# 0xPARC/plonky2-aes

Hardware: AMD Instinct MI355X
Metric: proofs/sec (AES-GCM 1 KiB circuit) (higher is better)
Workload: dtype u64 (Goldilocks field)

## Files before the change

### bindings/plonky2-hip/src/ffi.rs

```rust
#![allow(non_camel_case_types, dead_code)]
use std::os::raw::{c_char, c_int, c_long, c_void};

#[repr(C)] pub struct P2Builder { _private: [u8; 0] }
#[repr(C)] pub struct P2Circuit { _private: [u8; 0] }
#[repr(C)] pub struct P2Assignment { pub targets: *const u64, pub values: *const u64, pub count: usize }
#[repr(C)] #[derive(Default, Clone, Copy)]
pub struct P2CircuitInfo {
    pub degree_bits: u32, pub num_wires: u32, pub num_routed_wires: u32, pub num_constants_cols: u32, pub num_zs_cols: u32,
    pub num_quotient_cols: u32, pub num_luts: u32, pub num_ops: u32, pub num_levels: u32, pub num_slots: u32,
    pub num_virtual_targets: u32, pub num_fri_rounds: u32, pub proof_bytes: u64, pub zero_knowledge: u32, pub num_gate_kinds: u32,
    pub num_public_inputs: u32, pub hasher: u32,
}
#[repr(C)] pub struct P2KernelTime { pub name: [c_char; 48], pub ms: f32, pub count: u32 }
#[repr(C)] #[derive(Default, Clone, Copy, Debug)]
pub struct P2WitnessFault { pub kind: i32, pub op_kind: i32, pub input_index: i64, pub target: u64, pub gate_row: u32, pub computed: u64, pub found: u64 }

pub const P2_OK: c_int = 0;
pub const P2_PROOF_OK: c_int = 0;
pub const P2_VALUE_UNSET: u64 = u64::MAX;
pub const P2_FAULT_KINDS: [&str; 6] = ["NONE", "INPUT_NOT_CANONICAL", "INPUT_CONFLICT", "LOOKUP_MISS", "GENERATOR_CONFLICT", "NOT_SET"];
pub const P2_HASHER_POSEIDON: c_int = 0;
pub const P2_HASHER_KECCAK: c_int = 1;
pub const P2_POINT_WORDS: usize = 10;
pub const P2_SCALAR_LIMBS: usize = 5;
// ... 52 lines not shown
    pub fn p2_gcm_inc32(a0: *mut P2Builder, block: *const u64, out: *mut u64);
    pub fn p2_gcm_gf_2_128_mul(a0: *mut P2Builder, xor_lut: usize, shift_lut: usize, bitref_lut: usize, x: *const u64, y: *const u64, out: *mut u64);
    pub fn p2_gcm_ghash(a0: *mut P2Builder, xor_lut: usize, shift_lut: usize, bitref_lut: usize, h: *const u64, x: *const u64, len: usize, out: *mut u64) -> c_int;
    pub fn p2_gcm_gf_2_128_mul_tables(a0: *mut P2Builder, xor_lut: usize, clmul_lo_lut: usize, clmul_hi_lut: usize, x: *const u64, y: *const u64, out: *mut u64) -> c_int;
    pub fn p2_gcm_ghash_tables(a0: *mut P2Builder, xor_lut: usize, clmul_lo_lut: usize, clmul_hi_lut: usize, h: *const u64, x: *const u64, len: usize, out: *mut u64, lanes: c_int) -> c_int;
    pub fn p2_builder_set_ghash_tables(a0: *mut P2Builder, lanes: c_int) -> c_int;
    pub fn p2_aes_gcm_build(a0: *mut P2Builder, nk: c_int, nr: c_int, L: usize, with_tag: c_int, key: *mut u64, nonce: *mut u64, pt: *mut u64, ct: *mut u64, tag: *mut u64) -> c_int;
    pub fn p2_aes_gcm_build_aad(a0: *mut P2Builder, nk: c_int, nr: c_int, L: usize, with_tag: c_int, aad_len: usize, key: *mut u64, nonce: *mut u64, pt: *mut u64, ct: *mut u64, tag: *mut u64, aad: *mut u64) -> c_int;
    pub fn p2_builder_hash_n_to_m_no_pad(a0: *mut P2Builder, inputs: *const u64, n: usize, outputs: *mut u64, m: usize) -> c_int;
    pub fn p2_builder_permute_swapped(a0: *mut P2Builder, inputs: *const u64, swap: u64, out: *mut u64) -> c_int;
    pub fn p2_builder_hash_or_noop(a0: *mut P2Builder, inputs: *const u64, n: usize, out: *mut u64) -> c_int;
    pub fn p2_builder_add_virtual_hash(a0: *mut P2Builder, out: *mut u64) -> c_int;
    pub fn p2_builder_add_virtual_cap(a0: *mut P2Builder, cap_height: c_int, out: *mut u64) -> c_int;
    pub fn p2_builder_connect_hashes(a0: *mut P2Builder, x: *const u64, y: *const u64) -> c_int;
    pub fn p2_builder_verify_merkle_proof_to_cap(a0: *mut P2Builder, leaf: *const u64, leaf_len: usize, index_bits: *const u64, n_bits: usize, cap: *const u64, cap_height: c_int, siblings: *const u64, n_siblings: usize) -> c_int;
    pub fn p2_builder_verify_merkle_proof(a0: *mut P2Builder, leaf: *const u64, leaf_len: usize, index_bits: *const u64, n_bits: usize, root: *const u64, siblings: *const u64, n_siblings: usize) -> c_int;
    pub fn p2_builder_merkle_update_to_cap(a0: *mut P2Builder, old_leaf: *const u64, new_leaf: *const u64, leaf_len: usize, index_bits: *const u64, n_bits: usize, old_cap: *const u64, cap_height: c_int, siblings: *const u64, n_siblings: usize, new_cap: *mut u64) -> c_int;
    pub fn p2_builder_merkle_update(a0: *mut P2Builder, old_leaf: *const u64, new_leaf: *const u64, leaf_len: usize, index_bits: *const u64, n_bits: usize, old_root: *const u64, siblings: *const u64, n_siblings: usize, new_root: *mut u64) -> c_int;
    pub fn p2_native_merkle_cap(leaves: *const u64, num_leaves: usize, leaf_len: usize, cap_height: c_int, cap: *mut u64) -> c_int;
    pub fn p2_native_merkle_prove(leaves: *const u64, num_leaves: usize, leaf_len: usize, cap_height: c_int, index: usize, siblings: *mut u64) -> c_int;
    pub fn p2_native_merkle_verify(leaf: *const u64, leaf_len: usize, index: usize, siblings: *const u64, depth: usize, cap: *const u64, cap_height: c_int, status: *mut c_int) -> c_int;
    pub fn p2_native_merkle_update(leaves: *mut u64, num_leaves: usize, leaf_len: usize, cap_height: c_int, indices: *const u64, new_leaves: *const u64, k: usize, siblings: *mut u64, root_after: *mut u64) -> c_int;
    pub fn p2_builder_merkle_map_lookup_to_cap(a0: *mut P2Builder, key_bits: *const u64, n_bits: usize, value: *const u64, value_len: usize, present: u64, cap: *const u64, cap_height: c_int, siblings: *const u64, n_siblings: usize) -> c_int;
    pub fn p2_builder_merkle_map_lookup(a0: *mut P2Builder, key_bits: *const u64, n_bits: usize, value: *const u64, value_len: usize, present: u64, root: *const u64, siblings: *const u64, n_siblings: usize) -> c_int;
    pub fn p2_builder_merkle_map_update_to_cap(a0: *mut P2Builder, key_bits: *const u64, n_bits: usize, old_present: u64, old_value: *const u64, new_present: u64, new_value: *const u64, value_len: usize, old_cap: *const u64, cap_height: c_int, siblings: *const u64, n_siblings: usize, new_cap: *mut u64) -> c_int;
    pub fn p2_builder_merkle_map_update(a0: *mut P2Builder, key_bits: *const u64, n_bits: usize, old_present: u64, old_value: *const u64, new_present: u64, new_value: *const u64, value_len: usize, old_root: *const u64, siblings: *const u64, n_siblings: usize, new_root: *mut u64) -> c_int;
    pub fn p2_builder_merkle_map_insert_to_cap(a0: *mut P2Builder, key_bits: *const u64, n_bits: usize, value: *const u64, value_len: usize, old_cap: *const u64, cap_height: c_int, siblings: *const u64, n_siblings: usize, new_cap: *mut u64) -> c_int;
    pub fn p2_builder_merkle_map_insert(a0: *mut P2Builder, key_bits: *const u64, n_bits: usize, value: *const u64, value_len: usize, old_root: *const u64, siblings: *const u64, n_siblings: usize, new_root: *mut u64) -> c_int;
    pub fn p2_builder_merkle_map_remove_to_cap(a0: *mut P2Builder, key_bits: *const u64, n_bits: usize, value: *const u64, value_len: usize, old_cap: *const u64, cap_height: c_int, siblings: *const u64, n_siblings: usize, new_cap: *mut u64) -> c_int;
    pub fn p2_builder_merkle_map_remove(a0: *mut P2Builder, key_bits: *const u64, n_bits: usize, value: *const u64, value_len: usize, old_root: *const u64, siblings: *const u64, n_siblings: usize, new_root: *mut u64) -> c_int;
    pub fn p2_native_merkle_map_cap(keys: *const u64, values: *const u64, n: usize, value_len: usize, key_bits: c_int, cap_height: c_int, cap: *mut u64) -> c_int;
    pub fn p2_native_merkle_map_get(keys: *const u64, values: *const u64, n: usize, value_len: usize, key_bits: c_int, cap_height: c_int, key: u64, present: *mut c_int, value: *mut u64, siblings: *mut u64) -> c_int;
    pub fn p2_native_merkle_map_verify(key: u64, key_bits: c_int, present: u64, value: *const u64, value_len: usize, siblings: *const u64, cap: *const u64, cap_height: c_int, status: *mut c_int) -> c_int;
    pub fn p2_poseidon_cipher_build(a0: *mut P2Builder, L: usize, ks: *mut u64, m: *mut u64, nonce: *mut u64, ct: *mut u64) -> c_int;
    pub fn p2_builder_poseidon_encrypt(a0: *mut P2Builder, ks: *const u64, nonce: *const u64, m: *const u64, L: usize, ct: *mut u64) -> c_int;
    pub fn p2_builder_poseidon_decrypt(a0: *mut P2Builder, ks: *const u64, nonce: *const u64, ct: *const u64, L: usize, m: *mut u64) -> c_int;
    pub fn p2_native_hash_n_to_m_no_pad(in: *const u64, n: usize, out: *mut u64, m: usize);
    pub fn p2_native_poseidon_encrypt(ks10: *const u64, msg: *const u64, n_msg: usize, nonce2: *const u64, ct: *mut u64);
    pub fn p2_native_poseidon_decrypt(ks10: *const u64, ct: *const u64, n_ct: usize, nonce2: *const u64, l: usize, msg: *mut u64) -> c_int;
    pub fn p2_ecgfp5_group_order(out: *mut u64);
    pub fn p2_ecgfp5_generator(out: *mut u64);
    pub fn p2_ecgfp5_mul(k: *const u64, p: *const u64, out: *mut u64);
    pub fn p2_ecgfp5_add(p: *const u64, q: *const u64, out: *mut u64);
    pub fn p2_ecgfp5_neg(p: *const u64, out: *mut u64);
    pub fn p2_ecgfp5_is_in_subgroup(p: *const u64) -> c_int;
    pub fn p2_ecgfp5_compress(p: *const u64, w: *mut u64);
    pub fn p2_ecgfp5_decompress(w: *const u64, out: *mut u64) -> c_int;
    pub fn p2_ecgfp5_random_scalar(out: *mut u64) -> c_int;
    pub fn p2_ecgfp5_random_point(out: *mut u64) -> c_int;
    pub fn p2_ecgfp5_encode_binary(limbs: *const u32, out: *mut u64) -> c_int;
    pub fn p2_ecgfp5_random_scalar_seeded(seed: u64, out: *mut u64);
    pub fn p2_ecgfp5_random_point_seeded(seed: u64, out: *mut u64);
    pub fn p2_ecgfp5_encode_binary_seeded(limbs: *const u32, seed: u64, out: *mut u64);
    pub fn p2_ecgfp5_decode_binary(p: *const u64, limbs: *mut u32);
    pub fn p2_elgamal_encrypt(pk: *const u64, nonce: *const u64, msg: *const u64, c0: *mut u64, c1: *mut u64) -> c_int;
    pub fn p2_elgamal_decrypt(sk: *const u64, c0: *const u64, c1: *const u64, msg: *mut u64) -> c_int;
    pub fn p2_hashed_elgamal_encrypt(pk: *const u64, nonce: *const u64, msg: *const u64, c0: *mut u64, ct: *mut u64) -> c_int;
    pub fn p2_hashed_elgamal_decrypt(sk: *const u64, c0: *const u64, ct: *const u64, msg: *mut u64) -> c_int;
    pub fn p2_builder_add_virtual_point_target(a0: *mut P2Builder, out: *mut u64);
    pub fn p2_builder_constant_point(a0: *mut P2Builder, p: *const u64, out: *mut u64);
    pub fn p2_builder_add_virtual_biguint320_target(a0: *mut P2Builder, bits: *mut u64);
    pub fn p2_builder_multiply_point(a0: *mut P2Builder, bits: *const u64, p: *const u64, out: *mut u64) -> c_int;
    pub fn p2_builder_add_point(a0: *mut P2Builder, p: *const u64, q: *const u64, out: *mut u64);
    pub fn p2_builder_set_ec_gate(a0: *mut P2Builder, on: c_int) -> c_int;
    pub fn p2_builder_ec_step(a0: *mut P2Builder, acc: *const u64, q: *const u64, bit: u64, hinted: c_int, mid: *mut u64, out: *mut u64) -> c_int;
    pub fn p2_builder_public_key(a0: *mut P2Builder, sk_bits: *const u64, pk: *mut u64) -> c_int;
    pub fn p2_builder_elgamal_encrypt(a0: *mut P2Builder, pk: *const u64, nonce_bits: *const u64, msg: *const u64, c0: *mut u64, c1: *mut u64) -> c_int;
    pub fn p2_builder_hashed_elgamal_encrypt(a0: *mut P2Builder, pk: *const u64, nonce_bits: *const u64, msg: *const u64, c0: *mut u64, ct: *mut u64) -> c_int;
    pub fn p2_ecgfp5_encode_binary_padded(limbs: *const u32, pad: *const u32, attempts: usize, out: *mut u64, used: *mut u32) -> c_int;
    pub fn p2_builder_neg_point(a0: *mut P2Builder, p: *const u64, out: *mut u64) -> c_int;
    pub fn p2_builder_elgamal_decrypt(a0: *mut P2Builder, sk_bits: *const u64, c0: *const u64, c1: *const u64, msg: *mut u64) -> c_int;
    pub fn p2_builder_hashed_elgamal_decrypt(a0: *mut P2Builder, sk_bits: *const u64, c0: *const u64, ct: *const u64, msg: *mut u64) -> c_int;
    pub fn p2_ecgfp5_scalar_muladd(a: *const u64, b: *const u64, c: *const u64, out: *mut u64);
    pub fn p2_schnorr_challenge(r: *const u64, pk: *const u64, msg: *const u64, msg_len: usize, e: *mut u64) -> c_int;
    pub fn p2_schnorr_sign(sk: *const u64, nonce: *const u64, msg: *const u64, msg_len: usize, sig: *mut u64, pk: *mut u64, status: *mut c_int) -> c_int;
    pub fn p2_schnorr_verify(pk: *const u64, msg: *const u64, msg_len: usize, sig: *const u64, status: *mut c_int) -> c_int;
    pub fn p2_builder_add_virtual_schnorr_signature(a0: *mut P2Builder, s_bits: *mut u64, e: *mut u64) -> c_int;
    pub fn p2_builder_verify_schnorr_signature(a0: *mut P2Builder, pk: *const u64, msg: *const u64, msg_len: usize, s_bits: *const u64, e: *const u64, r: *mut u64) -> c_int;
    pub fn p2_selftest_host(seed: u64, n_reductions: usize, n_permutations: usize) -> c_int;
    pub fn p2_selftest_device(seed: u64, threads: usize, device: c_int) -> c_int;
    pub fn p2_selftest_lazy_device(seed: u64, threads: usize, device: c_int) -> c_int;
    pub fn p2_selftest_ntt_device(seed: u64, threads: usize, device: c_int) -> c_int;
    pub fn p2_host_poseidon_known(states: *mut u64, n_perm: usize, kind: c_int, rows: u32, parts: c_int) -> c_int;
    pub fn p2_host_pcipher_hash_state(in: *const u64, last: c_int, out: *mut u64) -> c_int;
    pub fn p2_host_partial_rounds(states: *mut u64, count: usize) -> c_int;
    pub fn p2_host_merged_middle(states: *mut u64, count: usize) -> c_int;
    pub fn p2_host_ecstep_constraints(wires: *const u64, count: usize, out: *mut u64) -> c_int;
    pub fn p2_host_ecstep_constraints_ext(wires: *const u64, count: usize, out: *mut u64) -> c_int;
    pub fn p2_host_hash_leaves(data: *const u64, cols: usize, active_cols: usize, num_leaves: usize, digests: *mut u64) -> c_int;
    pub fn p2_native_gf_2_8_mul(a: u8, b: u8) -> u8;
    pub fn p2_native_aes_key_expansion(key: *const u8, nk: c_int, nr: c_int, out: *mut u8);
    pub fn p2_native_aes_encrypt_block(key: *const u8, nk: c_int, nr: c_int, in16: *const u8, out16: *mut u8);
    pub fn p2_native_gf_2_128_mul(x16: *const u8, y16: *const u8, out16: *mut u8);
    pub fn p2_native_ghash(h16: *const u8, x: *const u8, len: usize, out16: *mut u8);
    pub fn p2_native_gctr(key: *const u8, nk: c_int, nr: c_int, icb16: *const u8, x: *const u8, len: usize, y: *mut u8);
    pub fn p2_native_aes_gcm_encrypt_aad(key: *const u8, nk: c_int, nr: c_int, nonce12: *const u8, aad: *const u8, aad_len: usize, pt: *const u8, len: usize, ct: *mut u8, tag16: *mut u8);
    pub fn p2_native_aes_gcm_decrypt(key: *const u8, nk: c_int, nr: c_int, nonce12: *const u8, aad: *const u8, aad_len: usize, ct: *const u8, len: usize, tag16: *const u8, pt: *mut u8) -> c_int;
    pub fn p2_native_aes_gcm_encrypt(key: *const u8, nk: c_int, nr: c_int, nonce12: *const u8, pt: *const u8, len: usize, ct: *mut u8, tag16: *mut u8);
    pub fn p2_native_keccak_hash_no_pad(in: *const u64, n: usize, out4: *mut u64);
    pub fn p2_native_keccak_two_to_one(l4: *const u64, r4: *const u64, out4: *mut u64);
    pub fn p2_native_keccak256(data: *const u8, len: usize, out32: *mut u8);
    pub fn p2_blob_info(blob: *const u8, len: usize, out: *mut P2CircuitInfo) -> c_int;
    pub fn p2_witness_schedule_check(blob: *const u8, len: usize, fuse: u32, out: *mut u32) -> c_int;
    pub fn p2_verify(blob: *const u8, blob_len: usize, verifier_data: *const u64, verifier_data_len: usize, proof: *const u8, proof_len: usize) -> c_int;
    pub fn p2_vanishing_terms(blob: *const u8, blob_len: usize, openings: *const u8, len: usize, challenges: *const u64, pi_hash: *const u64, terms: *mut u64, cap: usize, n_terms: *mut usize, sides: *mut u64, verdict: *mut c_int) -> c_int;
    pub fn p2_proof_compress(blob: *const u8, blob_len: usize, verifier_data: *const u64, verifier_data_len: usize, proof: *const u8, proof_len: usize, out: *mut u8, cap: usize, n_written: *mut usize) -> c_int;
    pub fn p2_proof_decompress(blob: *const u8, blob_len: usize, verifier_data: *const u64, verifier_data_len: usize, cproof: *const u8, cproof_len: usize, out: *mut u8, cap: usize, n_written: *mut usize) -> c_int;
    pub fn p2_verify_compressed(blob: *const u8, blob_len: usize, verifier_data: *const u64, verifier_data_len: usize, cproof: *const u8, cproof_len: usize) -> c_int;
    pub fn p2_proof_public_inputs(blob: *const u8, blob_len: usize, proof: *const u8, proof_len: usize, out: *mut u64, cap: usize, n_written: *mut usize) -> c_int;
    pub fn p2_circuit_load(blob: *const u8, len: usize, device: c_int) -> *mut P2Circuit;
    pub fn p2_circuit_free(a0: *mut P2Circuit);
    pub fn p2_circuit_verifier_data(a0: *const P2Circuit, out: *mut u64, cap: usize, n_written: *mut usize) -> c_int;
    pub fn p2_circuit_chunk_proofs(a0: *mut P2Circuit) -> usize;
    pub fn p2_circuit_set_zk_key(a0: *mut P2Circuit, key: *const u64) -> c_int;
    pub fn p2_circuit_set_zk_seed(a0: *mut P2Circuit, seed: u64) -> c_int;
    pub fn p2_circuit_proof_bytes(a0: *const P2Circuit) -> usize;
    pub fn p2_circuit_num_public_inputs(a0: *const P2Circuit) -> usize;
    pub fn p2_circuit_public_inputs(a0: *const P2Circuit, proof: *const u8, proof_len: usize, out: *mut u64, cap: usize, n_written: *mut usize) -> c_int;
    pub fn p2_prove_batch(a0: *mut P2Circuit, batch: usize, inputs: *const P2Assignment, proofs: *mut u8, status: *mut c_int) -> c_int;
    pub fn p2_prove_batch_multi(handles: *const *mut P2Circuit, n_handles: usize, batch: usize, inputs: *const P2Assignment, proofs: *mut u8, status: *mut c_int) -> c_int;
    pub fn p2_prove_batch_device(a0: *mut P2Circuit, batch: usize, targets: *const u64, n_targets: usize, d_values: *const u64, d_proofs: *mut u8, d_status: *mut c_int, stream: *mut c_void) -> c_int;
    pub fn p2_circuit_synchronize(a0: *mut P2Circuit) -> c_int;
    pub fn p2_prove_batch_outputs_device(a0: *mut P2Circuit, batch: usize, targets: *const u64, n_targets: usize, d_values: *const u64, out_targets: *const u64, n_out: usize, d_out: *mut u64, d_proofs: *mut u8, d_status: *mut c_int, stream: *mut c_void) -> c_int;
    pub fn p2_prove_batch_outputs(a0: *mut P2Circuit, batch: usize, inputs: *const P2Assignment, out_targets: *const u64, n_out: usize, out_values: *mut u64, proofs: *mut u8, status: *mut c_int) -> c_int;
    pub fn p2_witness_batch_device(a0: *mut P2Circuit, batch: usize, targets: *const u64, n_targets: usize, d_values: *const u64, out_targets: *const u64, n_out: usize, d_out: *mut u64, d_status: *mut c_int, stream: *mut c_void) -> c_int;
    pub fn p2_witness_batch(a0: *mut P2Circuit, batch: usize, inputs: *const P2Assignment, out_targets: *const u64, n_out: usize, out_values: *mut u64, status: *mut c_int) -> c_int;
    pub fn p2_witness_explain(a0: *mut P2Circuit, input: *const P2Assignment, status: *mut c_int, out: *mut c_void) -> c_int;
    pub fn p2_host_witness(blob: *const u8, len: usize, input: *const P2Assignment, out_targets: *const u64, n_out: usize, out_values: *mut u64, status: *mut c_int, fault: *mut c_void) -> c_int;
    pub fn p2_verify_batch(a0: *mut P2Circuit, batch: usize, proofs: *const u8, verifier_data: *const u64, vd_len: usize, status: *mut c_int) -> c_int;
    pub fn p2_verify_batch_device(a0: *mut P2Circuit, batch: usize, d_proofs: *const u8, verifier_data: *const u64, vd_len: usize, d_status: *mut c_int, stream: *mut c_void) -> c_int;
    pub fn p2_gpu_vanishing_flags(a0: *mut P2Circuit, batch: usize, buffers: *const u8, challenges: *const u64, pi_hashes: *const u64, flags: *mut u32) -> c_int;
    pub fn p2_compress_batch(a0: *mut P2Circuit, batch: usize, proofs: *const u8, verifier_data: *const u64, vd_len: usize, out: *mut u8, lengths: *mut u32, status: *mut c_int) -> c_int;
    pub fn p2_decompress_batch(a0: *mut P2Circuit, batch: usize, cproofs: *const u8, lengths: *const u32, verifier_data: *const u64, vd_len: usize, out: *mut u8, status: *mut c_int) -> c_int;
    pub fn p2_verify_compressed_batch(a0: *mut P2Circuit, batch: usize, cproofs: *const u8, lengths: *const u32, verifier_data: *const u64, vd_len: usize, status: *mut c_int) -> c_int;
    pub fn p2_compress_batch_device(a0: *mut P2Circuit, batch: usize, d_proofs: *const u8, verifier_data: *const u64, vd_len: usize, d_out: *mut u8, d_lengths: *mut u32, d_status: *mut c_int, stream: *mut c_void) -> c_int;
    pub fn p2_decompress_batch_device(a0: *mut P2Circuit, batch: usize, d_cproofs: *const u8, d_lengths: *const u32, verifier_data: *const u64, vd_len: usize, d_out: *mut u8, d_status: *mut c_int, stream: *mut c_void) -> c_int;
    pub fn p2_verify_compressed_batch_device(a0: *mut P2Circuit, batch: usize, d_cproofs: *const u8, d_lengths: *const u32, verifier_data: *const u64, vd_len: usize, d_status: *mut c_int, stream: *mut c_void) -> c_int;
    pub fn p2_circuit_set_option(a0: *mut P2Circuit, name: *const c_char, value: c_long) -> c_int;
    pub fn p2_circuit_set_timing(a0: *mut P2Circuit, enable: c_int) -> c_int;
    pub fn p2_circuit_get_timing(a0: *mut P2Circuit, out: *mut P2KernelTime, cap: usize) -> usize;
    pub fn p2_merkle_tree_new(leaves: *const u64, num_leaves: usize, leaf_len: usize, cap_height: c_int, device: c_int, tree: *mut *mut c_void) -> c_int;
    pub fn p2_merkle_tree_new_device(d_leaves: *const u64, num_leaves: usize, leaf_len: usize, cap_height: c_int, device: c_int, stream: *mut c_void, tree: *mut *mut c_void) -> c_int;
    pub fn p2_merkle_tree_free(tree: *mut c_void);
    pub fn p2_merkle_tree_cap(tree: *mut c_void, cap: *mut u64, cap_words: usize) -> c_int;
    pub fn p2_merkle_tree_prove_batch(tree: *mut c_void, indices: *const u64, n: usize, siblings: *mut u64) -> c_int;
    pub fn p2_merkle_tree_prove_batch_device(tree: *mut c_void, d_indices: *const u64, n: usize, d_out: *mut u64, out_stride_words: usize, d_status: *mut c_int, stream: *mut c_void) -> c_int;
    pub fn p2_merkle_tree_update(tree: *mut c_void, indices: *const u64, leaves: *const u64, k: usize, siblings: *mut u64, root_after: *mut u64) -> c_int;
    pub fn p2_merkle_tree_update_device(tree: *mut c_void, d_indices: *const u64, d_leaves: *const u64, k: usize, d_siblings: *mut u64, sib_stride_words: usize, d_root_after: *mut u64, root_stride_words: usize, d_status: *mut c_int, stream: *mut c_void) -> c_int;
    pub fn p2_merkle_tree_last_update_hashes(tree: *mut c_void, hashes: *mut u64) -> c_int;
    pub fn p2_merkle_verify_batch(leaves: *const u64, leaf_len: usize, indices: *const u64, siblings: *const u64, depth: usize, cap: *const u64, cap_height: c_int, n: usize, status: *mut c_int, device: c_int) -> c_int;
    pub fn p2_merkle_verify_batch_device(d_leaves: *const u64, leaf_len: usize, d_indices: *const u64, d_siblings: *const u64, depth: usize, d_cap: *const u64, cap_height: c_int, n: usize, d_status: *mut c_int, device: c_int, stream: *mut c_void) -> c_int;
    pub fn p2_gpu_merkle_build_device(d_leaves: *const u64, num_leaves: usize, leaf_len: usize, cap_height: c_int, with_transpose: c_int, d_scratch: *mut u64, d_dig: *mut u64, device: c_int, stream: *mut c_void) -> c_int;
    pub fn p2_merkle_map_new(keys: *const u64, values: *const u64, n: usize, value_len: usize, key_bits: c_int, cap_height: c_int, device: c_int, map: *mut *mut c_void) -> c_int;
    pub fn p2_merkle_map_new_device(d_keys: *const u64, d_values: *const u64, n: usize, value_len: usize, key_bits: c_int, cap_height: c_int, device: c_int, stream: *mut c_void, map: *mut *mut c_void) -> c_int;
    pub fn p2_merkle_map_free(map: *mut c_void);
    pub fn p2_merkle_map_cap(map: *mut c_void, cap: *mut u64, cap_words: usize) -> c_int;
    pub fn p2_merkle_map_len(map: *mut c_void, n: *mut usize) -> c_int;
    pub fn p2_merkle_map_hashes(map: *mut c_void, hashes: *mut u64) -> c_int;
    pub fn p2_merkle_map_get_batch(map: *mut c_void, keys: *const u64, n: usize, present: *mut u64, values: *mut u64, siblings: *mut u64) -> c_int;
    pub fn p2_merkle_map_get_batch_device(map: *mut c_void, d_keys: *const u64, n: usize, d_out: *mut u64, out_stride_words: usize, present_off: usize, value_off: usize, siblings_off: usize, d_status: *mut c_int, stream: *mut c_void) -> c_int;
    pub fn p2_merkle_map_verify_batch(keys: *const u64, key_bits: c_int, present: *const u64, values: *const u64, value_len: usize, siblings: *const u64, cap: *const u64, cap_height: c_int, n: usize, status: *mut c_int, device: c_int) -> c_int;
    pub fn p2_merkle_map_verify_batch_device(d_keys: *const u64, key_bits: c_int, d_present: *const u64, d_values: *const u64, value_len: usize, d_siblings: *const u64, d_cap: *const u64, cap_height: c_int, n: usize, d_status: *mut c_int, device: c_int, stream: *mut c_void) -> c_int;
    pub fn p2_ecgfp5_mul_batch(k: *const u64, p: *const u64, count: usize, out: *mut u64, status: *mut c_int, device: c_int) -> c_int;
    pub fn p2_ecgfp5_mul_batch_device(d_k: *const u64, d_p: *const u64, count: usize, d_out: *mut u64, d_status: *mut c_int, device: c_int, stream: *mut c_void) -> c_int;
    pub fn p2_schnorr_sign_batch(sk: *const u64, nonce: *const u64, msg: *const u64, msg_len: usize, count: usize, sig: *mut u64, pk: *mut u64, status: *mut c_int, device: c_int) -> c_int;
    pub fn p2_schnorr_sign_batch_device(d_sk: *const u64, d_nonce: *const u64, d_msg: *const u64, msg_len: usize, count: usize, d_sig: *mut u64, d_pk: *mut u64, d_status: *mut c_int, device: c_int, stream: *mut c_void) -> c_int;
    pub fn p2_schnorr_verify_batch(pk: *const u64, msg: *const u64, msg_len: usize, sig: *const u64, count: usize, status: *mut c_int, device: c_int) -> c_int;
    pub fn p2_schnorr_verify_batch_device(d_pk: *const u64, d_msg: *const u64, msg_len: usize, d_sig: *const u64, count: usize, d_status: *mut c_int, device: c_int, stream: *mut c_void) -> c_int;
    pub fn p2_gpu_ecgfp5_scalar_muladd(a: *const u64, b: *const u64, c: *const u64, count: usize, out: *mut u64, device: c_int) -> c_int;
    pub fn p2_ecgfp5_decompress_batch(w: *const u64, count: usize, out: *mut u64, status: *mut c_int, device: c_int) -> c_int;
    pub fn p2_ecgfp5_decompress_batch_device(d_w: *const u64, count: usize, d_out: *mut u64, d_status: *mut c_int, device: c_int, stream: *mut c_void) -> c_int;
    pub fn p2_ecgfp5_encode_binary_batch(limbs: *const u32, pad: *const u32, attempts: usize, count: usize, out: *mut u64, used: *mut u32, status: *mut c_int, device: c_int) -> c_int;
    pub fn p2_ecgfp5_encode_binary_batch_device(d_limbs: *const u32, d_pad: *const u32, attempts: usize, count: usize, d_out: *mut u64, d_used: *mut u32, d_status: *mut c_int, device: c_int, stream: *mut c_void) -> c_int;
    pub fn p2_elgamal_encrypt_batch(pk: *const u64, nonce: *const u64, msg: *const u64, count: usize, c0: *mut u64, c1: *mut u64, status: *mut c_int, device: c_int) -> c_int;
    pub fn p2_elgamal_encrypt_batch_device(d_pk: *const u64, d_nonce: *const u64, d_msg: *const u64, count: usize, d_c0: *mut u64, d_c1: *mut u64, d_status: *mut c_int, device: c_int, stream: *mut c_void) -> c_int;
    pub fn p2_elgamal_decrypt_batch(sk: *const u64, c0: *const u64, c1: *const u64, count: usize, msg: *mut u64, status: *mut c_int, device: c_int) -> c_int;
    pub fn p2_elgamal_decrypt_batch_device(d_sk: *const u64, d_c0: *const u64, d_c1: *const u64, count: usize, d_msg: *mut u64, d_status: *mut c_int, device: c_int, stream: *mut c_void) -> c_int;
    pub fn p2_hashed_elgamal_encrypt_batch(pk: *const u64, nonce: *const u64, msg: *const u64, count: usize, c0: *mut u64, ct: *mut u64, status: *mut c_int, device: c_int) -> c_int;
    pub fn p2_hashed_elgamal_encrypt_batch_device(d_pk: *const u64, d_nonce: *const u64, d_msg: *const u64, count: usize, d_c0: *mut u64, d_ct: *mut u64, d_status: *mut c_int, device: c_int, stream: *mut c_void) -> c_int;
    pub fn p2_hashed_elgamal_decrypt_batch(sk: *const u64, c0: *const u64, ct: *const u64, count: usize, msg: *mut u64, status: *mut c_int, device: c_int) -> c_int;
    pub fn p2_hashed_elgamal_decrypt_batch_device(d_sk: *const u64, d_c0: *const u64, d_ct: *const u64, count: usize, d_msg: *mut u64, d_status: *mut c_int, device: c_int, stream: *mut c_void) -> c_int;
    pub fn p2_ecgfp5_scalar_bits_device(d_k: *const u64, count: usize, d_out: *mut u64, stride: usize, device: c_int, stream: *mut c_void) -> c_int;
    pub fn p2_poseidon_encrypt_batch(ks: *const u64, nonce: *const u64, msg: *const u64, l: usize, count: usize, ct: *mut u64, status: *mut c_int, device: c_int) -> c_int;
    pub fn p2_poseidon_encrypt_batch_device(d_ks: *const u64, d_nonce: *const u64, d_msg: *const u64, l: usize, count: usize, d_ct: *mut u64, d_status: *mut c_int, device: c_int, stream: *mut c_void) -> c_int;
    pub fn p2_poseidon_decrypt_batch(ks: *const u64, nonce: *const u64, ct: *const u64, l: usize, count: usize, msg: *mut u64, status: *mut c_int, device: c_int) -> c_int;
    pub fn p2_poseidon_decrypt_batch_device(d_ks: *const u64, d_nonce: *const u64, d_ct: *const u64, l: usize, count: usize, d_msg: *mut u64, d_status: *mut c_int, device: c_int, stream: *mut c_void) -> c_int;
    pub fn p2_aes_gcm_batch_workspace(nk: c_int, len: usize, aad_len: usize, count: usize) -> usize;
    pub fn p2_aes_gcm_encrypt_batch(key: *const u8, nk: c_int, nonce: *const u8, aad: *const u8, aad_len: usize, pt: *const u8, len: usize, count: usize, ct: *mut u8, tag: *mut u8, status: *mut c_int, device: c_int) -> c_int;
    pub fn p2_aes_gcm_decrypt_batch(key: *const u8, nk: c_int, nonce: *const u8, aad: *const u8, aad_len: usize, ct: *const u8, tag: *const u8, len: usize, count: usize, pt: *mut u8, status: *mut c_int, device: c_int) -> c_int;
    pub fn p2_aes_gcm_encrypt_batch_device(d_key: *const u8, nk: c_int, d_nonce: *const u8, d_aad: *const u8, aad_len: usize, d_pt: *const u8, len: usize, row_stride: usize, count: usize, d_ct: *mut u8, d_tag: *mut u8, d_status: *mut c_int, d_work: *mut c_void, device: c_int, stream: *mut c_void) -> c_int;
    pub fn p2_aes_gcm_decrypt_batch_device(d_key: *const u8, nk: c_int, d_nonce: *const u8, d_aad: *const u8, aad_len: usize, d_ct: *const u8, d_tag: *const u8, len: usize, row_stride: usize, count: usize, d_pt: *mut u8, d_status: *mut c_int, d_work: *mut c_void, device: c_int, stream: *mut c_void) -> c_int;
    pub fn p2_bytes_to_words_device(d_bytes: *const u8, row_bytes: usize, byte_stride: usize, count: usize, d_out: *mut u64, stride_words: usize, device: c_int, stream: *mut c_void) -> c_int;
    pub fn p2_gpu_gcm_ghash(h: *const u8, x: *const u8, blocks: usize, count: usize, lanes: c_int, out: *mut u8, device: c_int) -> c_int;
    pub fn p2_gpu_aes_encrypt_blocks(key: *const u8, nk: c_int, in: *const u8, count: usize, out: *mut u8, device: c_int) -> c_int;
    pub fn p2_gpu_gcm_kernel_times(nk: c_int, len: usize, aad_len: usize, count: usize, lanes: c_int, repeats: usize, ns: *mut u64, device: c_int) -> c_int;
    pub fn p2_gpu_device_count() -> c_int;
    pub fn p2_gpu_poseidon(states: *mut u64, n_perm: usize, device: c_int) -> c_int;
    pub fn p2_gpu_lde(coeffs: *const u64, cols: usize, degree_bits: c_int, rate_bits: c_int, lde: *mut u64, device: c_int) -> c_int;
    pub fn p2_gpu_intt(values: *const u64, cols: usize, degree_bits: c_int, coeffs: *mut u64, device: c_int) -> c_int;
    pub fn p2_gpu_lde_round(coeffs: *const u64, cols: usize, degree_bits: c_int, arities: *const u32, n_rounds: usize, round: usize, batch: usize, in_batch_stride: usize, out: *mut u64, out_batch_stride: usize, device: c_int) -> c_int;
    pub fn p2_gpu_quotient_chunks(qvals: *const u64, chunks: usize, degree_bits: c_int, batch: usize, out: *mut u64, device: c_int) -> c_int;
    pub fn p2_gpu_merkle_cap(cols_major: *const u64, cols: usize, num_leaves: usize, cap_height: c_int, cap: *mut u64, device: c_int) -> c_int;
    pub fn p2_gpu_merkle_cap_hasher(cols_major: *const u64, cols: usize, num_leaves: usize, cap_height: c_int, hasher: c_int, cap: *mut u64, device: c_int) -> c_int;
    pub fn p2_gpu_hash_leaves(data: *const u64, cols: usize, active_cols: usize, num_leaves: usize, batch: usize, digests: *mut u64, device: c_int) -> c_int;
    pub fn p2_gpu_partial_rounds(states: *mut u64, count: usize, device: c_int) -> c_int;
    pub fn p2_gpu_merged_middle(states: *mut u64, count: usize, device: c_int) -> c_int;
    pub fn p2_gpu_ecstep_constraints(wires: *const u64, count: usize, out: *mut u64, device: c_int) -> c_int;
    pub fn p2_gpu_merkle_level(child: *const u64, num_parents: usize, batch: usize, parent: *mut u64, device: c_int) -> c_int;
    pub fn p2_gpu_hash_fri_leaves(vals: *const u64, len: usize, arity: c_int, batch: usize, digests: *mut u64, device: c_int) -> c_int;
    pub fn p2_gpu_zeta_pows(z: *const u64, n: usize, pows: *mut u64, device: c_int) -> c_int;
    pub fn p2_circuit_debug_read(a0: *mut P2Circuit, name: *const c_char, index: usize, out: *mut u64, cap: usize, n_written: *mut usize) -> c_int;
    pub fn p2_debug_live_resources() -> usize;
}
```

### include/p2aes.h

```cpp
#ifndef P2AES_H
#define P2AES_H
#include <stddef.h>
#include <stdint.h>

#ifdef __cplusplus
extern "C" {
#endif

enum {
    P2_OK = 0,
    P2_ERR_INVALID = 1,
    P2_ERR_NO_DEVICE = 2,
    P2_ERR_HIP = 3,
    P2_ERR_VERIFY = 4
};
enum {
    P2_PROOF_OK = 0,
    P2_PROOF_WITNESS_CONFLICT = 1,
    P2_PROOF_MISSING_INPUT = 2,
    P2_PROOF_ZETA_IN_SUBGROUP = 3,
    P2_PROOF_POW_NOT_FOUND = 4
};
enum {
    P2_VERIFY_OK = 0,
// ... 101 lines not shown
                            size_t k, uint64_t* siblings, uint64_t* root_after);
int p2_builder_merkle_map_lookup_to_cap(p2_builder*, const p2_target* key_bits, size_t n_bits, const p2_target* value, size_t value_len, p2_target present,
                                        const p2_target* cap, int cap_height, const p2_target* siblings, size_t n_siblings);
int p2_builder_merkle_map_lookup(p2_builder*, const p2_target* key_bits, size_t n_bits, const p2_target* value, size_t value_len, p2_target present,
                                 const p2_target root[4], const p2_target* siblings, size_t n_siblings);
int p2_builder_merkle_map_update_to_cap(p2_builder*, const p2_target* key_bits, size_t n_bits, p2_target old_present, const p2_target* old_value,
                                        p2_target new_present, const p2_target* new_value, size_t value_len, const p2_target* old_cap, int cap_height,
                                        const p2_target* siblings, size_t n_siblings, p2_target* new_cap);
int p2_builder_merkle_map_update(p2_builder*, const p2_target* key_bits, size_t n_bits, p2_target old_present, const p2_target* old_value, p2_target new_present,
                                 const p2_target* new_value, size_t value_len, const p2_target old_root[4], const p2_target* siblings, size_t n_siblings,
                                 p2_target new_root[4]);
int p2_builder_merkle_map_insert_to_cap(p2_builder*, const p2_target* key_bits, size_t n_bits, const p2_target* value, size_t value_len, const p2_target* old_cap,
                                        int cap_height, const p2_target* siblings, size_t n_siblings, p2_target* new_cap);
int p2_builder_merkle_map_insert(p2_builder*, const p2_target* key_bits, size_t n_bits, const p2_target* value, size_t value_len, const p2_target old_root[4],
                                 const p2_target* siblings, size_t n_siblings, p2_target new_root[4]);
int p2_builder_merkle_map_remove_to_cap(p2_builder*, const p2_target* key_bits, size_t n_bits, const p2_target* value, size_t value_len, const p2_target* old_cap,
                                        int cap_height, const p2_target* siblings, size_t n_siblings, p2_target* new_cap);
int p2_builder_merkle_map_remove(p2_builder*, const p2_target* key_bits, size_t n_bits, const p2_target* value, size_t value_len, const p2_target old_root[4],
                                 const p2_target* siblings, size_t n_siblings, p2_target new_root[4]);
int p2_native_merkle_map_cap(const uint64_t* keys, const uint64_t* values, size_t n, size_t value_len, int key_bits, int cap_height, uint64_t* cap);
int p2_native_merkle_map_get(const uint64_t* keys, const uint64_t* values, size_t n, size_t value_len, int key_bits, int cap_height, uint64_t key, int* present,
                             uint64_t* value, uint64_t* siblings);
int p2_native_merkle_map_verify(uint64_t key, int key_bits, uint64_t present, const uint64_t* value, size_t value_len, const uint64_t* siblings,
                                const uint64_t* cap, int cap_height, int* status);
int p2_poseidon_cipher_build(p2_builder*, size_t L, p2_target* ks, p2_target* m, p2_target* nonce, p2_target* ct);
int p2_builder_poseidon_encrypt(p2_builder*, const p2_target ks[10], const p2_target nonce[2], const p2_target* m, size_t L, p2_target* ct);
int p2_builder_poseidon_decrypt(p2_builder*, const p2_target ks[10], const p2_target nonce[2], const p2_target* ct, size_t L, p2_target* m);
void p2_native_hash_n_to_m_no_pad(const uint64_t* in, size_t n, uint64_t* out, size_t m);
void p2_native_poseidon_encrypt(const uint64_t* ks10, const uint64_t* msg, size_t n_msg, const uint64_t* nonce2, uint64_t* ct);
int p2_native_poseidon_decrypt(const uint64_t* ks10, const uint64_t* ct, size_t n_ct, const uint64_t* nonce2, size_t l, uint64_t* msg);

#define P2_POINT_WORDS 10
#define P2_SCALAR_LIMBS 5
#define P2_SCALAR_BITS 320
void p2_ecgfp5_group_order(uint64_t out[5]);
void p2_ecgfp5_generator(uint64_t out[10]);
void p2_ecgfp5_mul(const uint64_t k[5], const uint64_t p[10], uint64_t out[10]);
void p2_ecgfp5_add(const uint64_t p[10], const uint64_t q[10], uint64_t out[10]);
void p2_ecgfp5_neg(const uint64_t p[10], uint64_t out[10]);
int p2_ecgfp5_is_in_subgroup(const uint64_t p[10]);
void p2_ecgfp5_compress(const uint64_t p[10], uint64_t w[5]);
int p2_ecgfp5_decompress(const uint64_t w[5], uint64_t out[10]);
int p2_ecgfp5_random_scalar(uint64_t out[5]);
int p2_ecgfp5_random_point(uint64_t out[10]);
int p2_ecgfp5_encode_binary(const uint32_t limbs[5], uint64_t out[10]);
void p2_ecgfp5_random_scalar_seeded(uint64_t seed, uint64_t out[5]);
void p2_ecgfp5_random_point_seeded(uint64_t seed, uint64_t out[10]);
void p2_ecgfp5_encode_binary_seeded(const uint32_t limbs[5], uint64_t seed, uint64_t out[10]);
void p2_ecgfp5_decode_binary(const uint64_t p[10], uint32_t limbs[5]);
int p2_elgamal_encrypt(const uint64_t pk[10], const uint64_t nonce[5], const uint64_t msg[10], uint64_t c0[10], uint64_t c1[10]);
int p2_elgamal_decrypt(const uint64_t sk[5], const uint64_t c0[10], const uint64_t c1[10], uint64_t msg[10]);
int p2_hashed_elgamal_encrypt(const uint64_t pk[10], const uint64_t nonce[5], const uint64_t msg[5], uint64_t c0[10], uint64_t ct[5]);
int p2_hashed_elgamal_decrypt(const uint64_t sk[5], const uint64_t c0[10], const uint64_t ct[5], uint64_t msg[5]);
void p2_builder_add_virtual_point_target(p2_builder*, p2_target out[10]);
void p2_builder_constant_point(p2_builder*, const uint64_t p[10], p2_target out[10]);
void p2_builder_add_virtual_biguint320_target(p2_builder*, p2_target bits[320]);
int p2_builder_multiply_point(p2_builder*, const p2_target bits[320], const p2_target p[10], p2_target out[10]);
void p2_builder_add_point(p2_builder*, const p2_target p[10], const p2_target q[10], p2_target out[10]);
int p2_builder_set_ec_gate(p2_builder*, int on);
int p2_builder_ec_step(p2_builder*, const p2_target acc[20], const p2_target q[10], p2_target bit, int hinted, p2_target mid[20], p2_target out[20]);
int p2_builder_public_key(p2_builder*, const p2_target sk_bits[320], p2_target pk[10]);
int p2_builder_elgamal_encrypt(p2_builder*, const p2_target pk[10], const p2_target nonce_bits[320], const p2_target msg[10],
                               p2_target c0[10], p2_target c1[10]);
int p2_builder_hashed_elgamal_encrypt(p2_builder*, const p2_target pk[10], const p2_target nonce_bits[320], const p2_target msg[5],
                                      p2_target c0[10], p2_target ct[5]);
int p2_ecgfp5_encode_binary_padded(const uint32_t limbs[5], const uint32_t* pad, size_t attempts, uint64_t out[10], uint32_t* used);
int p2_builder_neg_point(p2_builder*, const p2_target p[10], p2_target out[10]);
int p2_builder_elgamal_decrypt(p2_builder*, const p2_target sk_bits[320], const p2_target c0[10], const p2_target c1[10], p2_target msg[10]);
int p2_builder_hashed_elgamal_decrypt(p2_builder*, const p2_target sk_bits[320], const p2_target c0[10], const p2_target ct[5], p2_target msg[5]);

void p2_ecgfp5_scalar_muladd(const uint64_t a[5], const uint64_t b[5], const uint64_t c[5], uint64_t out[5]);
int p2_schnorr_challenge(const uint64_t r[10], const uint64_t pk[10], const uint64_t* msg, size_t msg_len, uint64_t e[4]);
int p2_schnorr_sign(const uint64_t sk[5], const uint64_t nonce[5], const uint64_t* msg, size_t msg_len, uint64_t sig[9], uint64_t pk[10], int* status);
int p2_schnorr_verify(const uint64_t pk[10], const uint64_t* msg, size_t msg_len, const uint64_t sig[9], int* status);
int p2_builder_add_virtual_schnorr_signature(p2_builder*, p2_target s_bits[320], p2_target e[4]);
int p2_builder_verify_schnorr_signature(p2_builder*, const p2_target pk[10], const p2_target* msg, size_t msg_len, const p2_target s_bits[320],
                                        const p2_target e[4], p2_target r[10]);

int p2_selftest_host(uint64_t seed, size_t n_reductions, size_t n_permutations);
int p2_selftest_device(uint64_t seed, size_t threads, int device);
int p2_selftest_lazy_device(uint64_t seed, size_t threads, int device);
int p2_selftest_ntt_device(uint64_t seed, size_t threads, int device);
int p2_host_poseidon_known(uint64_t* states, size_t n_perm, int kind, uint32_t rows, int parts);
int p2_host_pcipher_hash_state(const uint64_t in[20], int last, uint64_t out[20]);
int p2_host_partial_rounds(uint64_t* states, size_t count);
int p2_host_merged_middle(uint64_t* states, size_t count);
int p2_host_ecstep_constraints(const uint64_t* wires, size_t count, uint64_t* out);
int p2_host_ecstep_constraints_ext(const uint64_t* wires, size_t count, uint64_t* out);
int p2_host_hash_leaves(const uint64_t* data, size_t cols, size_t active_cols, size_t num_leaves, uint64_t* digests);

uint8_t p2_native_gf_2_8_mul(uint8_t a, uint8_t b);
void p2_native_aes_key_expansion(const uint8_t* key, int nk, int nr, uint8_t* out );
void p2_native_aes_encrypt_block(const uint8_t* key, int nk, int nr, const uint8_t* in16, uint8_t* out16);
void p2_native_gf_2_128_mul(const uint8_t* x16, const uint8_t* y16, uint8_t* out16);
void p2_native_ghash(const uint8_t* h16, const uint8_t* x, size_t len, uint8_t* out16);
void p2_native_gctr(const uint8_t* key, int nk, int nr, const uint8_t* icb16, const uint8_t* x, size_t len, uint8_t* y);
void p2_native_aes_gcm_encrypt_aad(const uint8_t* key, int nk, int nr, const uint8_t* nonce12, const uint8_t* aad, size_t aad_len, const uint8_t* pt,
                                   size_t len, uint8_t* ct, uint8_t* tag16);
int p2_native_aes_gcm_decrypt(const uint8_t* key, int nk, int nr, const uint8_t* nonce12, const uint8_t* aad, size_t aad_len, const uint8_t* ct, size_t len,
                              const uint8_t* tag16, uint8_t* pt);
void p2_native_aes_gcm_encrypt(const uint8_t* key, int nk, int nr, const uint8_t* nonce12, const uint8_t* pt, size_t len,
                               uint8_t* ct, uint8_t* tag16);

void p2_native_keccak_hash_no_pad(const uint64_t* in, size_t n, uint64_t out4[4]);
void p2_native_keccak_two_to_one(const uint64_t l4[4], const uint64_t r4[4], uint64_t out4[4]);
void p2_native_keccak256(const uint8_t* data, size_t len, uint8_t out32[32]);

typedef struct {
    uint32_t degree_bits, num_wires, num_routed_wires, num_constants_cols, num_zs_cols, num_quotient_cols, num_luts,
        num_ops, num_levels, num_slots, num_virtual_targets, num_fri_rounds;
    uint64_t proof_bytes;
    uint32_t zero_knowledge, num_gate_kinds;
    uint32_t num_public_inputs;
    uint32_t hasher;
} p2_circuit_info;
int p2_blob_info(const uint8_t* blob, size_t len, p2_circuit_info* out);
int p2_witness_schedule_check(const uint8_t* blob, size_t len, uint32_t fuse, uint32_t out[4]);
int p2_verify(const uint8_t* blob, size_t blob_len, const uint64_t* verifier_data, size_t verifier_data_len,
              const uint8_t* proof, size_t proof_len);
int p2_vanishing_terms(const uint8_t* blob, size_t blob_len, const uint8_t* openings, size_t len, const uint64_t challenges[16],
                       const uint64_t pi_hash[4], uint64_t* terms, size_t cap, size_t* n_terms, uint64_t sides[8], int* verdict);
int p2_proof_compress(const uint8_t* blob, size_t blob_len, const uint64_t* verifier_data, size_t verifier_data_len, const uint8_t* proof,
                      size_t proof_len, uint8_t* out, size_t cap, size_t* n_written);
int p2_proof_decompress(const uint8_t* blob, size_t blob_len, const uint64_t* verifier_data, size_t verifier_data_len, const uint8_t* cproof,
                        size_t cproof_len, uint8_t* out, size_t cap, size_t* n_written);
int p2_verify_compressed(const uint8_t* blob, size_t blob_len, const uint64_t* verifier_data, size_t verifier_data_len,
                         const uint8_t* cproof, size_t cproof_len);
int p2_proof_public_inputs(const uint8_t* blob, size_t blob_len, const uint8_t* proof, size_t proof_len, uint64_t* out, size_t cap,
                           size_t* n_written);

typedef struct p2_circuit p2_circuit;
p2_circuit* p2_circuit_load(const uint8_t* blob, size_t len, int device);
void p2_circuit_free(p2_circuit*);
int p2_circuit_verifier_data(const p2_circuit*, uint64_t* out, size_t cap, size_t* n_written);
size_t p2_circuit_chunk_proofs(p2_circuit*);
int p2_circuit_set_zk_key(p2_circuit*, const uint64_t key[4]);
int p2_circuit_set_zk_seed(p2_circuit*, uint64_t seed);
size_t p2_circuit_proof_bytes(const p2_circuit*);
size_t p2_circuit_num_public_inputs(const p2_circuit*);
int p2_circuit_public_inputs(const p2_circuit*, const uint8_t* proof, size_t proof_len, uint64_t* out, size_t cap, size_t* n_written);
typedef struct {
    const p2_target* targets;
    const uint64_t* values;
    size_t count;
} p2_assignment;
int p2_prove_batch(p2_circuit*, size_t batch, const p2_assignment* inputs, uint8_t* proofs, int* status);
int p2_prove_batch_multi(p2_circuit* const* handles, size_t n_handles, size_t batch, const p2_assignment* inputs,
                         uint8_t* proofs, int* status);
int p2_prove_batch_device(p2_circuit*, size_t batch, const p2_target* targets, size_t n_targets, const uint64_t* d_values,
                          uint8_t* d_proofs, int* d_status, void* stream);
int p2_circuit_synchronize(p2_circuit*);

#define P2_VALUE_UNSET UINT64_MAX
int p2_prove_batch_outputs_device(p2_circuit*, size_t batch, const p2_target* targets, size_t n_targets, const uint64_t* d_values,
                                  const p2_target* out_targets, size_t n_out, uint64_t* d_out, uint8_t* d_proofs, int* d_status, void* stream);
int p2_prove_batch_outputs(p2_circuit*, size_t batch, const p2_assignment* inputs, const p2_target* out_targets, size_t n_out,
                           uint64_t* out_values, uint8_t* proofs, int* status);
int p2_witness_batch_device(p2_circuit*, size_t batch, const p2_target* targets, size_t n_targets, const uint64_t* d_values,
                            const p2_target* out_targets, size_t n_out, uint64_t* d_out, int* d_status, void* stream);
int p2_witness_batch(p2_circuit*, size_t batch, const p2_assignment* inputs, const p2_target* out_targets, size_t n_out,
                     uint64_t* out_values, int* status);
typedef struct {
    int32_t kind;
    int32_t op_kind;
    int64_t input_index;
    p2_target target;
// ... 60 lines not shown
int p2_merkle_map_new_device(const uint64_t* d_keys, const uint64_t* d_values, size_t n, size_t value_len, int key_bits, int cap_height, int device, void* stream,
                             void** map);
void p2_merkle_map_free(void* map);
int p2_merkle_map_cap(void* map, uint64_t* cap, size_t cap_words);
int p2_merkle_map_len(void* map, size_t* n);
int p2_merkle_map_hashes(void* map, uint64_t* hashes);
int p2_merkle_map_get_batch(void* map, const uint64_t* keys, size_t n, uint64_t* present, uint64_t* values, uint64_t* siblings);
int p2_merkle_map_get_batch_device(void* map, const uint64_t* d_keys, size_t n, uint64_t* d_out, size_t out_stride_words, size_t present_off, size_t value_off,
                                   size_t siblings_off, int* d_status, void* stream);
int p2_merkle_map_verify_batch(const uint64_t* keys, int key_bits, const uint64_t* present, const uint64_t* values, size_t value_len, const uint64_t* siblings,
                               const uint64_t* cap, int cap_height, size_t n, int* status, int device);
int p2_merkle_map_verify_batch_device(const uint64_t* d_keys, int key_bits, const uint64_t* d_present, const uint64_t* d_values, size_t value_len,
                                      const uint64_t* d_siblings, const uint64_t* d_cap, int cap_height, size_t n, int* d_status, int device, void* stream);

int p2_ecgfp5_mul_batch(const uint64_t* k, const uint64_t* p, size_t count, uint64_t* out, int* status, int device);
int p2_ecgfp5_mul_batch_device(const uint64_t* d_k, const uint64_t* d_p, size_t count, uint64_t* d_out, int* d_status, int device, void* stream);
int p2_schnorr_sign_batch(const uint64_t* sk, const uint64_t* nonce, const uint64_t* msg, size_t msg_len, size_t count, uint64_t* sig, uint64_t* pk,
                          int* status, int device);
int p2_schnorr_sign_batch_device(const uint64_t* d_sk, const uint64_t* d_nonce, const uint64_t* d_msg, size_t msg_len, size_t count, uint64_t* d_sig,
                                 uint64_t* d_pk, int* d_status, int device, void* stream);
int p2_schnorr_verify_batch(const uint64_t* pk, const uint64_t* msg, size_t msg_len, const uint64_t* sig, size_t count, int* status, int device);
int p2_schnorr_verify_batch_device(const uint64_t* d_pk, const uint64_t* d_msg, size_t msg_len, const uint64_t* d_sig, size_t count, int* d_status,
                                   int device, void* stream);
int p2_gpu_ecgfp5_scalar_muladd(const uint64_t* a, const uint64_t* b, const uint64_t* c, size_t count, uint64_t* out, int device);

int p2_ecgfp5_decompress_batch(const uint64_t* w, size_t count, uint64_t* out, int* status, int device);
int p2_ecgfp5_decompress_batch_device(const uint64_t* d_w, size_t count, uint64_t* d_out, int* d_status, int device, void* stream);
int p2_ecgfp5_encode_binary_batch(const uint32_t* limbs, const uint32_t* pad, size_t attempts, size_t count, uint64_t* out, uint32_t* used, int* status,
                                  int device);
int p2_ecgfp5_encode_binary_batch_device(const uint32_t* d_limbs, const uint32_t* d_pad, size_t attempts, size_t count, uint64_t* d_out, uint32_t* d_used,
                                         int* d_status, int device, void* stream);
int p2_elgamal_encrypt_batch(const uint64_t* pk, const uint64_t* nonce, const uint64_t* msg, size_t count, uint64_t* c0, uint64_t* c1, int* status,
                             int device);
int p2_elgamal_encrypt_batch_device(const uint64_t* d_pk, const uint64_t* d_nonce, const uint64_t* d_msg, size_t count, uint64_t* d_c0, uint64_t* d_c1,
                                    int* d_status, int device, void* stream);
int p2_elgamal_decrypt_batch(const uint64_t* sk, const uint64_t* c0, const uint64_t* c1, size_t count, uint64_t* msg, int* status, int device);
int p2_elgamal_decrypt_batch_device(const uint64_t* d_sk, const uint64_t* d_c0, const uint64_t* d_c1, size_t count, uint64_t* d_msg, int* d_status,
                                    int device, void* stream);
int p2_hashed_elgamal_encrypt_batch(const uint64_t* pk, const uint64_t* nonce, const uint64_t* msg, size_t count, uint64_t* c0, uint64_t* ct, int* status,
                                    int device);
int p2_hashed_elgamal_encrypt_batch_device(const uint64_t* d_pk, const uint64_t* d_nonce, const uint64_t* d_msg, size_t count, uint64_t* d_c0,
                                           uint64_t* d_ct, int* d_status, int device, void* stream);
int p2_hashed_elgamal_decrypt_batch(const uint64_t* sk, const uint64_t* c0, const uint64_t* ct, size_t count, uint64_t* msg, int* status, int device);
int p2_hashed_elgamal_decrypt_batch_device(const uint64_t* d_sk, const uint64_t* d_c0, const uint64_t* d_ct, size_t count, uint64_t* d_msg,
                                           int* d_status, int device, void* stream);
int p2_ecgfp5_scalar_bits_device(const uint64_t* d_k, size_t count, uint64_t* d_out, size_t stride, int device, void* stream);

int p2_poseidon_encrypt_batch(const uint64_t* ks, const uint64_t* nonce, const uint64_t* msg, size_t l, size_t count, uint64_t* ct, int* status, int device);
int p2_poseidon_encrypt_batch_device(const uint64_t* d_ks, const uint64_t* d_nonce, const uint64_t* d_msg, size_t l, size_t count, uint64_t* d_ct, int* d_status,
                                     int device, void* stream);
int p2_poseidon_decrypt_batch(const uint64_t* ks, const uint64_t* nonce, const uint64_t* ct, size_t l, size_t count, uint64_t* msg, int* status, int device);
int p2_poseidon_decrypt_batch_device(const uint64_t* d_ks, const uint64_t* d_nonce, const uint64_t* d_ct, size_t l, size_t count, uint64_t* d_msg, int* d_status,
                                     int device, void* stream);

size_t p2_aes_gcm_batch_workspace(int nk, size_t len, size_t aad_len, size_t count);
int p2_aes_gcm_encrypt_batch(const uint8_t* key, int nk, const uint8_t* nonce, const uint8_t* aad, size_t aad_len, const uint8_t* pt, size_t len, size_t count,
                             uint8_t* ct, uint8_t* tag, int* status, int device);
int p2_aes_gcm_decrypt_batch(const uint8_t* key, int nk, const uint8_t* nonce, const uint8_t* aad, size_t aad_len, const uint8_t* ct, const uint8_t* tag,
                             size_t len, size_t count, uint8_t* pt, int* status, int device);
int p2_aes_gcm_encrypt_batch_device(const uint8_t* d_key, int nk, const uint8_t* d_nonce, const uint8_t* d_aad, size_t aad_len, const uint8_t* d_pt, size_t len,
                                    size_t row_stride, size_t count, uint8_t* d_ct, uint8_t* d_tag, int* d_status, void* d_work, int device, void* stream);
int p2_aes_gcm_decrypt_batch_device(const uint8_t* d_key, int nk, const uint8_t* d_nonce, const uint8_t* d_aad, size_t aad_len, const uint8_t* d_ct,
                                    const uint8_t* d_tag, size_t len, size_t row_stride, size_t count, uint8_t* d_pt, int* d_status, void* d_work,
                                    int device, void* stream);
int p2_bytes_to_words_device(const uint8_t* d_bytes, size_t row_bytes, size_t byte_stride, size_t count, uint64_t* d_out, size_t stride_words, int device,
                             void* stream);
int p2_gpu_gcm_ghash(const uint8_t* h, const uint8_t* x, size_t blocks, size_t count, int lanes, uint8_t* out, int device);
int p2_gpu_aes_encrypt_blocks(const uint8_t* key, int nk, const uint8_t* in, size_t count, uint8_t* out, int device);
int p2_gpu_gcm_kernel_times(int nk, size_t len, size_t aad_len, size_t count, int lanes, size_t repeats, uint64_t* ns, int device);

int p2_gpu_device_count(void);
int p2_gpu_poseidon(uint64_t* states, size_t n_perm, int device);
int p2_gpu_lde(const uint64_t* coeffs, size_t cols, int degree_bits, int rate_bits, uint64_t* lde, int device);
int p2_gpu_intt(const uint64_t* values, size_t cols, int degree_bits, uint64_t* coeffs, int device);
int p2_gpu_lde_round(const uint64_t* coeffs, size_t cols, int degree_bits, const uint32_t* arities, size_t n_rounds, size_t round, size_t batch,
                     size_t in_batch_stride, uint64_t* out, size_t out_batch_stride, int device);
int p2_gpu_quotient_chunks(const uint64_t* qvals, size_t chunks, int degree_bits, size_t batch, uint64_t* out, int device);
int p2_gpu_merkle_cap(const uint64_t* cols_major, size_t cols, size_t num_leaves, int cap_height, uint64_t* cap, int device);
int p2_gpu_merkle_cap_hasher(const uint64_t* cols_major, size_t cols, size_t num_leaves, int cap_height, int hasher, uint64_t* cap, int device);
int p2_gpu_hash_leaves(const uint64_t* data, size_t cols, size_t active_cols, size_t num_leaves, size_t batch, uint64_t* digests, int device);
int p2_gpu_partial_rounds(uint64_t* states, size_t count, int device);
int p2_gpu_merged_middle(uint64_t* states, size_t count, int device);
int p2_gpu_ecstep_constraints(const uint64_t* wires, size_t count, uint64_t* out, int device);
int p2_gpu_merkle_level(const uint64_t* child, size_t num_parents, size_t batch, uint64_t* parent, int device);
int p2_gpu_hash_fri_leaves(const uint64_t* vals, size_t len, int arity, size_t batch, uint64_t* digests, int device);
int p2_gpu_zeta_pows(const uint64_t* z, size_t n, uint64_t* pows, int device);
int p2_circuit_debug_read(p2_circuit*, const char* name, size_t index, uint64_t* out, size_t cap, size_t* n_written);
size_t p2_debug_live_resources(void);

#ifdef __cplusplus
}
#endif
#endif
```

### plonky2-aes_amd/api.py

```python
import ctypes as C
import os
import struct

P = 0xFFFFFFFF00000001


class P2Error(RuntimeError):
    pass


class ProveError(P2Error):

    def __init__(self, status):
        self.status = status
        super().__init__({1: "witness conflict or lookup input not in table", 2: "a generator never ran (missing input)",
                          3: "opening point is in the subgroup",
                          4: "no proof-of-work witness found"}.get(status, "prove failed (%d)" % status))


VERIFY_OK, VERIFY_SHAPE, VERIFY_NON_CANONICAL, VERIFY_POW, VERIFY_ZETA_IN_SUBGROUP, VERIFY_VANISHING = 0, 1, 2, 3, 4, 5
VERIFY_MERKLE_INITIAL, VERIFY_FRI_FOLD, VERIFY_MERKLE_FRI, VERIFY_FINAL_POLY = 6, 7, 8, 9
VERIFY_REASONS = {
    "": VERIFY_OK,
    "proof truncated": VERIFY_SHAPE,
# ... 151 lines not shown
        "p2_aes_gf_2_8_mul": (u64, [vp, sz, u64, u64]), "p2_aes_gf_2_8_add": (u64, [vp, sz, u64, u64]),
        "p2_aes_key_expansion": (None, [vp, C.c_int, C.c_int, sz, sz, u64p, u64p]),
        "p2_aes_encrypt_block": (None, [vp, C.c_int, sz, sz, sz, u64p, u64p, u64p]),
        "p2_gcm_gctr": (None, [vp, C.c_int, sz, sz, sz, u64p, u64p, u64p, sz, u64p]),
        "p2_gcm_right_shift_one": (None, [vp, sz, u64p, u64p]), "p2_gcm_inc32": (None, [vp, u64p, u64p]),
        "p2_gcm_gf_2_128_mul": (None, [vp, sz, sz, sz, u64p, u64p, u64p]),
        "p2_gcm_ghash": (C.c_int, [vp, sz, sz, sz, u64p, u64p, sz, u64p]),
        "p2_gcm_clmul_lo_lut": (sz, [vp]), "p2_gcm_clmul_hi_lut": (sz, [vp]),
        "p2_gcm_gf_2_128_mul_tables": (C.c_int, [vp, sz, sz, sz, u64p, u64p, u64p]),
        "p2_gcm_ghash_tables": (C.c_int, [vp, sz, sz, sz, u64p, u64p, sz, u64p, C.c_int]),
        "p2_builder_set_ghash_tables": (C.c_int, [vp, C.c_int]),
        "p2_aes_gcm_build": (C.c_int, [vp, C.c_int, C.c_int, sz, C.c_int, u64p, u64p, u64p, u64p, u64p]),
        "p2_builder_hash_n_to_m_no_pad": (C.c_int, [vp, u64p, sz, u64p, sz]),
        "p2_poseidon_cipher_build": (C.c_int, [vp, sz, u64p, u64p, u64p, u64p]),
        "p2_native_hash_n_to_m_no_pad": (None, [u64p, sz, u64p, sz]),
        "p2_native_poseidon_encrypt": (None, [u64p, u64p, sz, u64p, u64p]),
        "p2_native_poseidon_decrypt": (C.c_int, [u64p, u64p, sz, u64p, sz, u64p]),
        "p2_ecgfp5_group_order": (None, [u64p]), "p2_ecgfp5_generator": (None, [u64p]),
        "p2_ecgfp5_mul": (None, [u64p, u64p, u64p]), "p2_ecgfp5_add": (None, [u64p, u64p, u64p]), "p2_ecgfp5_neg": (None, [u64p, u64p]),
        "p2_ecgfp5_is_in_subgroup": (C.c_int, [u64p]),
        "p2_ecgfp5_compress": (None, [u64p, u64p]), "p2_ecgfp5_decompress": (C.c_int, [u64p, u64p]),
        "p2_ecgfp5_random_scalar": (C.c_int, [u64p]), "p2_ecgfp5_random_point": (C.c_int, [u64p]),
        "p2_ecgfp5_encode_binary": (C.c_int, [u32p, u64p]),
        "p2_ecgfp5_random_scalar_seeded": (None, [u64, u64p]), "p2_ecgfp5_random_point_seeded": (None, [u64, u64p]),
        "p2_ecgfp5_encode_binary_seeded": (None, [u32p, u64, u64p]), "p2_ecgfp5_decode_binary": (None, [u64p, u32p]),
        "p2_elgamal_encrypt": (C.c_int, [u64p, u64p, u64p, u64p, u64p]), "p2_elgamal_decrypt": (C.c_int, [u64p, u64p, u64p, u64p]),
        "p2_hashed_elgamal_encrypt": (C.c_int, [u64p, u64p, u64p, u64p, u64p]),
        "p2_hashed_elgamal_decrypt": (C.c_int, [u64p, u64p, u64p, u64p]),
        "p2_builder_add_virtual_point_target": (None, [vp, u64p]), "p2_builder_constant_point": (None, [vp, u64p, u64p]),
        "p2_builder_add_virtual_biguint320_target": (None, [vp, u64p]),
        "p2_builder_multiply_point": (C.c_int, [vp, u64p, u64p, u64p]), "p2_builder_add_point": (None, [vp, u64p, u64p, u64p]),
        "p2_builder_public_key": (C.c_int, [vp, u64p, u64p]),
        "p2_builder_set_ec_gate": (C.c_int, [vp, C.c_int]), "p2_builder_ec_step": (C.c_int, [vp, u64p, u64p, u64, C.c_int, u64p, u64p]),
        "p2_builder_elgamal_encrypt": (C.c_int, [vp, u64p, u64p, u64p, u64p, u64p]),
        "p2_builder_hashed_elgamal_encrypt": (C.c_int, [vp, u64p, u64p, u64p, u64p, u64p]),
        "p2_selftest_host": (C.c_int, [u64, sz, sz]), "p2_selftest_device": (C.c_int, [u64, sz, C.c_int]),
        "p2_selftest_lazy_device": (C.c_int, [u64, sz, C.c_int]),
        "p2_selftest_ntt_device": (C.c_int, [u64, sz, C.c_int]),
        "p2_native_gf_2_8_mul": (C.c_uint8, [C.c_uint8, C.c_uint8]),
        "p2_native_aes_key_expansion": (None, [C.c_char_p, C.c_int, C.c_int, C.c_char_p]),
        "p2_native_aes_encrypt_block": (None, [C.c_char_p, C.c_int, C.c_int, C.c_char_p, C.c_char_p]),
        "p2_native_gf_2_128_mul": (None, [C.c_char_p, C.c_char_p, C.c_char_p]),
        "p2_native_ghash": (None, [C.c_char_p, C.c_char_p, sz, C.c_char_p]),
        "p2_native_gctr": (None, [C.c_char_p, C.c_int, C.c_int, C.c_char_p, C.c_char_p, sz, C.c_char_p]),
        "p2_native_aes_gcm_encrypt": (None, [C.c_char_p, C.c_int, C.c_int, C.c_char_p, C.c_char_p, sz, C.c_char_p, C.c_char_p]),
        "p2_native_aes_gcm_encrypt_aad": (None, [C.c_char_p, C.c_int, C.c_int, C.c_char_p, C.c_char_p, sz, C.c_char_p, sz, C.c_char_p, C.c_char_p]),
        "p2_native_aes_gcm_decrypt": (C.c_int, [C.c_char_p, C.c_int, C.c_int, C.c_char_p, C.c_char_p, sz, C.c_char_p, sz, C.c_char_p, C.c_char_p]),
        "p2_aes_gcm_build_aad": (C.c_int, [vp, C.c_int, C.c_int, sz, C.c_int, sz, u64p, u64p, u64p, u64p, u64p, u64p]),
        "p2_blob_info": (C.c_int, [C.c_char_p, sz, C.POINTER(_Info)]),
        "p2_witness_schedule_check": (C.c_int, [C.c_char_p, sz, C.c_uint32, u32p]),
        "p2_verify": (C.c_int, [C.c_char_p, sz, u64p, sz, C.c_char_p, sz]),
        "p2_vanishing_terms": (C.c_int, [C.c_char_p, sz, C.c_char_p, sz, u64p, u64p, u64p, sz, C.POINTER(sz), u64p, C.POINTER(C.c_int)]),
        "p2_gpu_vanishing_flags": (C.c_int, [vp, sz, C.c_char_p, u64p, u64p, u32p]),
        "p2_proof_compress": (C.c_int, [C.c_char_p, sz, u64p, sz, C.c_char_p, sz, C.c_char_p, sz, C.POINTER(sz)]),
        "p2_proof_decompress": (C.c_int, [C.c_char_p, sz, u64p, sz, C.c_char_p, sz, C.c_char_p, sz, C.POINTER(sz)]),
        "p2_verify_compressed": (C.c_int, [C.c_char_p, sz, u64p, sz, C.c_char_p, sz]),
        "p2_circuit_load": (vp, [C.c_char_p, sz, C.c_int]), "p2_circuit_free": (None, [vp]),
        "p2_circuit_verifier_data": (C.c_int, [vp, u64p, sz, C.POINTER(sz)]),
        "p2_circuit_proof_bytes": (sz, [vp]),
        "p2_circuit_num_public_inputs": (sz, [vp]),
        "p2_circuit_public_inputs": (C.c_int, [vp, C.c_char_p, sz, u64p, sz, C.POINTER(sz)]),
        "p2_circuit_chunk_proofs": (sz, [vp]),
        "p2_prove_batch": (C.c_int, [vp, sz, C.POINTER(_Assignment), C.c_char_p, C.POINTER(C.c_int)]),
        "p2_prove_batch_device": (C.c_int, [vp, sz, u64p, sz, vp, vp, vp, vp]),
        "p2_circuit_synchronize": (C.c_int, [vp]),
        "p2_prove_batch_outputs": (C.c_int, [vp, sz, C.POINTER(_Assignment), u64p, sz, u64p, C.c_char_p, C.POINTER(C.c_int)]),
        "p2_prove_batch_outputs_device": (C.c_int, [vp, sz, u64p, sz, vp, u64p, sz, vp, vp, vp, vp]),
        "p2_witness_batch": (C.c_int, [vp, sz, C.POINTER(_Assignment), u64p, sz, u64p, C.POINTER(C.c_int)]),
        "p2_witness_batch_device": (C.c_int, [vp, sz, u64p, sz, vp, u64p, sz, vp, vp, vp]),
        "p2_witness_explain": (C.c_int, [vp, C.POINTER(_Assignment), C.POINTER(C.c_int), vp]),
        "p2_host_witness": (C.c_int, [C.c_char_p, sz, C.POINTER(_Assignment), u64p, sz, u64p, C.POINTER(C.c_int), vp]),
        "p2_verify_batch": (C.c_int, [vp, sz, C.c_char_p, u64p, sz, C.POINTER(C.c_int)]),
        "p2_verify_batch_device": (C.c_int, [vp, sz, vp, u64p, sz, vp, vp]),
        "p2_compress_batch": (C.c_int, [vp, sz, C.c_char_p, u64p, sz, C.c_char_p, u32p, C.POINTER(C.c_int)]),
        "p2_compress_batch_device": (C.c_int, [vp, sz, vp, u64p, sz, vp, vp, vp, vp]),
        "p2_decompress_batch": (C.c_int, [vp, sz, C.c_char_p, u32p, u64p, sz, C.c_char_p, C.POINTER(C.c_int)]),
        "p2_decompress_batch_device": (C.c_int, [vp, sz, vp, vp, u64p, sz, vp, vp, vp]),
        "p2_verify_compressed_batch": (C.c_int, [vp, sz, C.c_char_p, u32p, u64p, sz, C.POINTER(C.c_int)]),
        "p2_verify_compressed_batch_device": (C.c_int, [vp, sz, vp, vp, u64p, sz, vp, vp]),
        "p2_circuit_set_timing": (C.c_int, [vp, C.c_int]),
        "p2_circuit_get_timing": (sz, [vp, C.POINTER(_KernelTime), sz]),
        "p2_gpu_device_count": (C.c_int, []),
        "p2_gpu_poseidon": (C.c_int, [u64p, sz, C.c_int]),
        "p2_host_partial_rounds": (C.c_int, [u64p, sz]),
        "p2_gpu_partial_rounds": (C.c_int, [u64p, sz, C.c_int]),
        "p2_host_merged_middle": (C.c_int, [u64p, sz]),
        "p2_gpu_merged_middle": (C.c_int, [u64p, sz, C.c_int]),
        "p2_host_ecstep_constraints": (C.c_int, [u64p, sz, u64p]), "p2_host_ecstep_constraints_ext": (C.c_int, [u64p, sz, u64p]),
        "p2_gpu_ecstep_constraints": (C.c_int, [u64p, sz, u64p, C.c_int]),
        "p2_gpu_lde": (C.c_int, [u64p, sz, C.c_int, C.c_int, u64p, C.c_int]),
        "p2_gpu_intt": (C.c_int, [u64p, sz, C.c_int, u64p, C.c_int]),
        "p2_gpu_lde_round": (C.c_int, [u64p, sz, C.c_int, u32p, sz, sz, sz, sz, u64p, sz, C.c_int]),
        "p2_gpu_quotient_chunks": (C.c_int, [u64p, sz, C.c_int, sz, u64p, C.c_int]),
        "p2_gpu_merkle_cap": (C.c_int, [u64p, sz, sz, C.c_int, u64p, C.c_int]),
        "p2_gpu_zeta_pows": (C.c_int, [u64p, sz, u64p, C.c_int]),
        "p2_circuit_debug_read": (C.c_int, [vp, C.c_char_p, sz, u64p, sz, C.POINTER(sz)]),
        "p2_debug_live_resources": (sz, []),
        "p2_builder_permute_swapped": (C.c_int, [vp, u64p, u64, u64p]), "p2_builder_hash_or_noop": (C.c_int, [vp, u64p, sz, u64p]),
        "p2_builder_add_virtual_hash": (C.c_int, [vp, u64p]), "p2_builder_add_virtual_cap": (C.c_int, [vp, C.c_int, u64p]),
        "p2_builder_connect_hashes": (C.c_int, [vp, u64p, u64p]),
        "p2_builder_verify_merkle_proof_to_cap": (C.c_int, [vp, u64p, sz, u64p, sz, u64p, C.c_int, u64p, sz]),
        "p2_builder_verify_merkle_proof": (C.c_int, [vp, u64p, sz, u64p, sz, u64p, u64p, sz]),
        "p2_native_merkle_cap": (C.c_int, [u64p, sz, sz, C.c_int, u64p]),
        "p2_native_merkle_prove": (C.c_int, [u64p, sz, sz, C.c_int, sz, u64p]),
        "p2_native_merkle_verify": (C.c_int, [u64p, sz, sz, u64p, sz, u64p, C.c_int, C.POINTER(C.c_int)]),
        "p2_merkle_tree_new": (C.c_int, [u64p, sz, sz, C.c_int, C.c_int, C.POINTER(vp)]),
        "p2_merkle_tree_new_device": (C.c_int, [vp, sz, sz, C.c_int, C.c_int, vp, C.POINTER(vp)]),
        "p2_merkle_tree_free": (None, [vp]), "p2_merkle_tree_cap": (C.c_int, [vp, u64p, sz]),
        "p2_merkle_tree_prove_batch": (C.c_int, [vp, u64p, sz, u64p]),
        "p2_merkle_tree_prove_batch_device": (C.c_int, [vp, vp, sz, vp, sz, vp, vp]),
        "p2_merkle_verify_batch": (C.c_int, [u64p, sz, u64p, u64p, sz, u64p, C.c_int, sz, C.POINTER(C.c_int), C.c_int]),
        "p2_merkle_verify_batch_device": (C.c_int, [vp, sz, vp, vp, sz, vp, C.c_int, sz, vp, C.c_int, vp]),
        "p2_gpu_merkle_build_device": (C.c_int, [vp, sz, sz, C.c_int, C.c_int, vp, vp, C.c_int, vp]),
        "p2_native_merkle_update": (C.c_int, [u64p, sz, sz, C.c_int, u64p, u64p, sz, u64p, u64p]),
        "p2_merkle_tree_update": (C.c_int, [vp, u64p, u64p, sz, u64p, u64p]),
        "p2_merkle_tree_update_device": (C.c_int, [vp, vp, vp, sz, vp, sz, vp, sz, vp, vp]),
        "p2_merkle_tree_last_update_hashes": (C.c_int, [vp, u64p]),
        "p2_builder_merkle_update_to_cap": (C.c_int, [vp, u64p, u64p, sz, u64p, sz, u64p, C.c_int, u64p, sz, u64p]),
        "p2_builder_merkle_update": (C.c_int, [vp, u64p, u64p, sz, u64p, sz, u64p, u64p, sz, u64p]),
        "p2_builder_merkle_map_lookup_to_cap": (C.c_int, [vp, u64p, sz, u64p, sz, u64, u64p, C.c_int, u64p, sz]),
        "p2_builder_merkle_map_lookup": (C.c_int, [vp, u64p, sz, u64p, sz, u64, u64p, u64p, sz]),
        "p2_builder_merkle_map_update_to_cap": (C.c_int, [vp, u64p, sz, u64, u64p, u64, u64p, sz, u64p, C.c_int, u64p, sz, u64p]),
        "p2_builder_merkle_map_update": (C.c_int, [vp, u64p, sz, u64, u64p, u64, u64p, sz, u64p, u64p, sz, u64p]),
        "p2_builder_merkle_map_insert_to_cap": (C.c_int, [vp, u64p, sz, u64p, sz, u64p, C.c_int, u64p, sz, u64p]),
        "p2_builder_merkle_map_insert": (C.c_int, [vp, u64p, sz, u64p, sz, u64p, u64p, sz, u64p]),
        "p2_builder_merkle_map_remove_to_cap": (C.c_int, [vp, u64p, sz, u64p, sz, u64p, C.c_int, u64p, sz, u64p]),
        "p2_builder_merkle_map_remove": (C.c_int, [vp, u64p, sz, u64p, sz, u64p, u64p, sz, u64p]),
        "p2_native_merkle_map_cap": (C.c_int, [u64p, u64p, sz, sz, C.c_int, C.c_int, u64p]),
        "p2_native_merkle_map_get": (C.c_int, [u64p, u64p, sz, sz, C.c_int, C.c_int, u64, C.POINTER(C.c_int), u64p, u64p]),
        "p2_native_merkle_map_verify": (C.c_int, [u64, C.c_int, u64, u64p, sz, u64p, u64p, C.c_int, C.POINTER(C.c_int)]),
        "p2_merkle_map_new": (C.c_int, [u64p, u64p, sz, sz, C.c_int, C.c_int, C.c_int, C.POINTER(vp)]),
        "p2_merkle_map_new_device": (C.c_int, [vp, vp, sz, sz, C.c_int, C.c_int, C.c_int, vp, C.POINTER(vp)]),
        "p2_merkle_map_free": (None, [vp]), "p2_merkle_map_cap": (C.c_int, [vp, u64p, sz]),
        "p2_merkle_map_len": (C.c_int, [vp, C.POINTER(sz)]), "p2_merkle_map_hashes": (C.c_int, [vp, u64p]),
        "p2_merkle_map_get_batch": (C.c_int, [vp, u64p, sz, u64p, u64p, u64p]),
        "p2_merkle_map_get_batch_device": (C.c_int, [vp, vp, sz, vp, sz, sz, sz, sz, vp, vp]),
        "p2_merkle_map_verify_batch": (C.c_int, [u64p, C.c_int, u64p, u64p, sz, u64p, u64p, C.c_int, sz, C.POINTER(C.c_int), C.c_int]),
        "p2_merkle_map_verify_batch_device": (C.c_int, [vp, C.c_int, vp, vp, sz, vp, vp, C.c_int, sz, vp, C.c_int, vp]),
        "p2_ecgfp5_scalar_muladd": (None, [u64p, u64p, u64p, u64p]),
        "p2_gpu_ecgfp5_scalar_muladd": (C.c_int, [u64p, u64p, u64p, sz, u64p, C.c_int]),
        "p2_schnorr_challenge": (C.c_int, [u64p, u64p, u64p, sz, u64p]),
        "p2_schnorr_sign": (C.c_int, [u64p, u64p, u64p, sz, u64p, u64p, C.POINTER(C.c_int)]),
        "p2_schnorr_verify": (C.c_int, [u64p, u64p, sz, u64p, C.POINTER(C.c_int)]),
        "p2_builder_add_virtual_schnorr_signature": (C.c_int, [vp, u64p, u64p]),
        "p2_builder_verify_schnorr_signature": (C.c_int, [vp, u64p, u64p, sz, u64p, u64p, u64p]),
        "p2_ecgfp5_mul_batch": (C.c_int, [u64p, u64p, sz, u64p, C.POINTER(C.c_int), C.c_int]),
        "p2_ecgfp5_mul_batch_device": (C.c_int, [vp, vp, sz, vp, vp, C.c_int, vp]),
        "p2_schnorr_sign_batch": (C.c_int, [u64p, u64p, u64p, sz, sz, u64p, u64p, C.POINTER(C.c_int), C.c_int]),
        "p2_schnorr_sign_batch_device": (C.c_int, [vp, vp, vp, sz, sz, vp, vp, vp, C.c_int, vp]),
        "p2_schnorr_verify_batch": (C.c_int, [u64p, u64p, sz, u64p, sz, C.POINTER(C.c_int), C.c_int]),
        "p2_schnorr_verify_batch_device": (C.c_int, [vp, vp, sz, vp, sz, vp, C.c_int, vp]),
        "p2_ecgfp5_encode_binary_padded": (C.c_int, [u32p, u32p, sz, u64p, u32p]),
        "p2_builder_neg_point": (C.c_int, [vp, u64p, u64p]),
        "p2_builder_elgamal_decrypt": (C.c_int, [vp, u64p, u64p, u64p, u64p]),
        "p2_builder_hashed_elgamal_decrypt": (C.c_int, [vp, u64p, u64p, u64p, u64p]),
        "p2_ecgfp5_decompress_batch": (C.c_int, [u64p, sz, u64p, C.POINTER(C.c_int), C.c_int]),
        "p2_ecgfp5_decompress_batch_device": (C.c_int, [vp, sz, vp, vp, C.c_int, vp]),
        "p2_ecgfp5_encode_binary_batch": (C.c_int, [u32p, u32p, sz, sz, u64p, u32p, C.POINTER(C.c_int), C.c_int]),
        "p2_ecgfp5_encode_binary_batch_device": (C.c_int, [vp, vp, sz, sz, vp, vp, vp, C.c_int, vp]),
        "p2_elgamal_encrypt_batch": (C.c_int, [u64p, u64p, u64p, sz, u64p, u64p, C.POINTER(C.c_int), C.c_int]),
        "p2_elgamal_encrypt_batch_device": (C.c_int, [vp, vp, vp, sz, vp, vp, vp, C.c_int, vp]),
        "p2_elgamal_decrypt_batch": (C.c_int, [u64p, u64p, u64p, sz, u64p, C.POINTER(C.c_int), C.c_int]),
        "p2_elgamal_decrypt_batch_device": (C.c_int, [vp, vp, vp, sz, vp, vp, C.c_int, vp]),
        "p2_hashed_elgamal_encrypt_batch": (C.c_int, [u64p, u64p, u64p, sz, u64p, u64p, C.POINTER(C.c_int), C.c_int]),
        "p2_hashed_elgamal_encrypt_batch_device": (C.c_int, [vp, vp, vp, sz, vp, vp, vp, C.c_int, vp]),
        "p2_hashed_elgamal_decrypt_batch": (C.c_int, [u64p, u64p, u64p, sz, u64p, C.POINTER(C.c_int), C.c_int]),
# ... 1877 lines not shown
```

### plonky2-aes_amd/csrc/capi_host.cpp

```cpp
#include <stdlib.h>

#include "../../include/p2aes.h"
#include "aes_gadgets.h"
#include "capi_common.h"
#include "compress.h"
#include "ecgfp5.h"
#include "merkle_host.h"
#define P2_PCIPHER_SPONGE_ONLY
#include "kernels_pcipher.h"
#include "poseidon_cipher.h"
#include "poseidon_fast.h"
#include "schnorr.h"
#include "verifier.h"
#include "witness_check.h"
#include "witness_schedule.h"

using namespace p2;

namespace p2 {
thread_local std::string g_last_error;
}

struct p2_builder {
    CircuitBuilder b;
// ... 759 lines not shown
        if (!status || msg_len > schnorr::MAX_MSG_LEN || (msg_len && !msg)) throw std::runtime_error("msg_len is at most 1024 words, status not null");
        ecgfp5::Affine pub;
        *status = schnorr::sign(sc_at(sk), sc_at(nonce), msg, msg_len, sig, pk ? &pub : nullptr);
        if (pk) pt_put(pub, pk);
    });
}
int p2_schnorr_verify(const uint64_t pk[10], const uint64_t* msg, size_t msg_len, const uint64_t sig[9], int* status) {
    return guarded([&] {
        if (!status || msg_len > schnorr::MAX_MSG_LEN || (msg_len && !msg)) throw std::runtime_error("msg_len is at most 1024 words, status not null");
        *status = schnorr::verify(pt_at(pk), msg, msg_len, sig);
    });
}
int p2_builder_add_virtual_schnorr_signature(p2_builder* b, p2_target s_bits[320], p2_target e[4]) {
    return guarded([&] {
        const schnorr::SignatureTarget t = schnorr::add_virtual_signature_target(b->b);
        for (size_t i = 0; i < t.s_bits.size(); i++) s_bits[i] = t.s_bits[i].target;
        std::copy(t.e.begin(), t.e.end(), e);
    });
}
int p2_builder_verify_schnorr_signature(p2_builder* b, const p2_target pk[10], const p2_target* msg, size_t msg_len, const p2_target s_bits[320], const p2_target e[4],
                                        p2_target r[10]) {
    return guarded([&] {
        if (msg_len && !msg) throw std::runtime_error("null message");
        const schnorr::SignatureTarget t{bits_at(s_bits), hash_at(e)};
        const ecgfp5::PointTarget rp = schnorr::verify_signature_target(b->b, ptt_at(pk), std::vector<Target>(msg, msg + msg_len), t);
        if (r) ptt_put(rp, r);
    });
}

int p2_selftest_host(uint64_t seed, size_t n_reductions, size_t n_permutations) {
    u64 x = seed | 1;
    auto rnd = [&]() {
        x ^= x << 13;
        x ^= x >> 7;
        x ^= x << 17;
        return x;
    };
    size_t bad = 0;
    for (size_t i = 0; i < n_reductions; i++) {
        u64 hi = rnd(), lo = rnd();
        switch (i & 15) {
            case 0: hi &= gl::EPS; break;
            case 1: lo &= gl::EPS; break;
            case 2: hi |= ~gl::EPS; break;
            case 3: lo |= ~gl::EPS; break;
            case 4: hi = 0; break;
            case 5: lo = 0; break;
            case 6: hi = ~0ull; lo = ~0ull - (x & 3); break;
            case 7: hi &= ~gl::EPS; lo &= gl::EPS; break;
            default: break;
        }
        unsigned __int128 v = ((unsigned __int128)hi << 64) | lo;
        u64 want = (u64)(v % gl::P);
        if (glf::canon(glf::red128(hi, lo)) != want) bad++;
        if (gl::reduce128(hi, lo) != want) bad++;
        glf::Acc a;
        a.init();
        a.fma(hi, lo);
        a.fma(lo, lo);
        unsigned __int128 w = ((unsigned __int128)hi * lo) % gl::P + ((unsigned __int128)lo * lo) % gl::P;
        if (glf::canon(a.reduce()) != (u64)(w % gl::P)) bad++;
    }
    for (size_t i = 0; i < n_permutations; i++) {
        u64 s0[12], s1[12];
        for (int k = 0; k < 12; k++) s0[k] = s1[k] = (i & 3) == 3 ? rnd() : rnd() % gl::P;
        for (int k = 0; k < 12; k++) s0[k] %= gl::P;
        gl::poseidon(s0);
        glf::poseidon(s1);
        for (int k = 0; k < 12; k++) bad += s0[k] != s1[k];
    }
    return (int)std::min<size_t>(bad, 0x7FFFFFFF);
}

int p2_host_poseidon_known(uint64_t* states, size_t n_perm, int kind, uint32_t rows, int parts) {
    if (kind < 0 || kind > (int)glf::FR_ZERO_RATE || rows == 0 || rows > glf::ROWS_ALL) return set_error("kind must be 0..2 and rows a mask of words 0..11"), P2_ERR_INVALID;
    for (size_t i = 0; i < n_perm; i++) {
        u64* s = states + 12 * i;
        if (parts) {
            glf::first_round_any(s, (u32)kind);
            glf::middle(s);
            glf::last_round_any(s, rows);
        } else {
            glf::permute_known_any(s, (u32)kind, rows);
        }
    }
    return P2_OK;
}
int p2_host_pcipher_hash_state(const uint64_t in[20], int last, uint64_t out[20]) {
    if (!in || !out) return set_error("p2_host_pcipher_hash_state: null argument"), P2_ERR_INVALID;
    for (int i = 0; i < 20; i++)
        if (in[i] >= gl::P) return set_error("p2_host_pcipher_hash_state: non-canonical word"), P2_ERR_INVALID;
    u64 s[20];
    memcpy(s, in, sizeof s);
    p2k::pcipher_hash_state(s, last != 0);
    for (int i = 0; i < 20; i++) out[i] = (last && (i < 5 || i >= 10)) ? 0 : s[i];
    return P2_OK;
}
int p2_host_partial_rounds(uint64_t* states, size_t count) {
    for (size_t i = 0; i < count; i++) glf::partial_block(states + 12 * i);
    return P2_OK;
}
int p2_host_merged_middle(uint64_t* states, size_t count) {
    for (size_t i = 0; i < count; i++) glf::merged_middle(states + 12 * i);
    return P2_OK;
}
int p2_host_ecstep_constraints(const uint64_t* wires, size_t count, uint64_t* out) {
    if (count && (!wires || !out)) return set_error("p2_host_ecstep_constraints: null argument"), P2_ERR_INVALID;
    for (size_t i = 0; i < 80 * count; i++)
        if (wires[i] >= gl::P) return set_error("p2_host_ecstep_constraints: non-canonical wire"), P2_ERR_INVALID;
    for (size_t r = 0; r < count; r++)
        ecstep_gate_constraints<FBase>([&](u32 i) { return wires[80 * r + i]; }, [&](int k, u64 c) { out[40 * r + k] = c; });
    return P2_OK;
}
int p2_host_ecstep_constraints_ext(const uint64_t* wires, size_t count, uint64_t* out) {
    if (count && (!wires || !out)) return set_error("p2_host_ecstep_constraints_ext: null argument"), P2_ERR_INVALID;
    for (size_t i = 0; i < 160 * count; i++)
        if (wires[i] >= gl::P) return set_error("p2_host_ecstep_constraints_ext: non-canonical wire"), P2_ERR_INVALID;
    for (size_t r = 0; r < count; r++)
        ecstep_gate_constraints<FExt>([&](u32 i) { return gl::e2(wires[160 * r + 2 * i], wires[160 * r + 2 * i + 1]); },
                                      [&](int k, gl::E2 c) { out[80 * r + 2 * k] = c.a, out[80 * r + 2 * k + 1] = c.b; });
    return P2_OK;
}
int p2_host_hash_leaves(const uint64_t* data, size_t cols, size_t active_cols, size_t num_leaves, uint64_t* digests) {
    if (cols == 0 || cols > (1u << 20)) return set_error("cols out of range"), P2_ERR_INVALID;
    for (size_t leaf = 0; leaf < num_leaves; leaf++) {
        u64 st[12] = {0};
        u64* out = digests + 4 * leaf;
        if (cols <= 4) {
            for (size_t c = 0; c < 4; c++) out[c] = (c < cols && c < active_cols) ? data[c * num_leaves + leaf] : 0;
            continue;
        }
        for (size_t c0 = 0; c0 < cols; c0 += 8) {
            for (size_t k = 0; k < 8 && c0 + k < cols; k++) st[k] = c0 + k < active_cols ? data[(c0 + k) * num_leaves + leaf] : 0;
            glf::sponge_permute(st, (int)c0, (int)cols, (int)std::min(active_cols, cols));
        }
        for (int i = 0; i < 4; i++) out[i] = st[i];
    }
    return P2_OK;
}

uint8_t p2_native_gf_2_8_mul(uint8_t a, uint8_t b) { return aes::gf_2_8_mul(a, b); }
void p2_native_aes_key_expansion(const uint8_t* key, int nk, int nr, uint8_t* out) {
    (void)guarded([&] {
        auto w = aes::key_expansion(nk, nr, key);
        for (size_t i = 0; i < w.size(); i++) memcpy(out + 4 * i, w[i].data(), 4);
    });
}
void p2_native_aes_encrypt_block(const uint8_t* key, int nk, int nr, const uint8_t* in, uint8_t* out) {
    (void)guarded([&] {
        auto w = aes::key_expansion(nk, nr, key);
        auto s = aes::flatten_state(aes::encrypt_block(nr, in, w));
        memcpy(out, s.data(), 16);
    });
}
void p2_native_gf_2_128_mul(const uint8_t* x, const uint8_t* y, uint8_t* out) {
    (void)guarded([&] {
        auto r = aes::gf_2_128_mul(x, y);
        memcpy(out, r.data(), 16);
    });
}
void p2_native_ghash(const uint8_t* h, const uint8_t* x, size_t len, uint8_t* out) {
    (void)guarded([&] {
        auto r = aes::ghash(h, x, len);
        memcpy(out, r.data(), 16);
    });
}
// ... 342 lines not shown
```

### plonky2-aes_amd/csrc/kernels.h

```cpp
#pragma once
#include <hip/hip_runtime.h>

#include "circuit.h"
#include "witness_schedule.h"
#include "gl.h"
#include "poseidon_fast.h"
#include "poseidon_gate.h"
#include "ecstep_gate.h"
#include "zk_prf.h"

namespace p2k {
using gl::E2;
using gl::u32;
using gl::u64;

static const u64 UNSET = ~0ull;

#ifndef P2_HASH_WAVES_PER_EU
#define P2_HASH_WAVES_PER_EU 5
#endif
#define P2_HASH_WAVES __attribute__((amdgpu_waves_per_eu(P2_HASH_WAVES_PER_EU, P2_HASH_WAVES_PER_EU)))

__global__ __launch_bounds__(256) P2_HASH_WAVES void k_hash_leaves(const u64* __restrict__ data, int cols, int active_cols, size_t col_stride,
                                                      size_t batch_stride, size_t num_leaves, u64* __restrict__ digests,
// ... 1079 lines not shown
    u64* ch = a.chal + (size_t)p * CH_WORDS;
    if (a.stage == 0) {
        c.w = c.inb = c.outb = 0;
        c.in_len = c.out_len = 0;
        for (int i = 0; i < 4; i++) c.observe(a.digest[i]);
        for (int i = 0; i < 4; i++) c.observe(a.pi_hash ? a.pi_hash[(size_t)p * 4 + i] : 0);
    } else {
        c.load(a.st[p]);
    }
    const u64* ob = a.observe + (size_t)p * a.observe_stride;
    if (a.stage == 6) {
        c.observe(ch[CH_POW]);
        (void)c.challenge();
        for (u32 q = 0; q < a.aux; q++) {
            const u64 v = c.challenge() % a.mod;
            if (writer) ch[CH_QUERY + q] = v;
        }
        if (real) c.store(a.st[p]);
        return;
    }
    for (u32 i = 0; i < a.observe_len; i++) c.observe(ob[i]);
    if (a.stage == 0) {
        u64 bg[4], dl[4];
        for (int i = 0; i < 4; i++) bg[i] = c.challenge();
        if (a.aux)
            for (int i = 0; i < 4; i++) dl[i] = c.challenge();
        if (writer) {
            for (int i = 0; i < 2; i++) ch[CH_BETAS + i] = bg[i];
            for (int i = 0; i < 2; i++) ch[CH_GAMMAS + i] = bg[2 + i];
            if (a.aux) {
                for (int i = 0; i < 4; i++) ch[CH_DELTAS + i] = bg[i];
                for (int i = 0; i < 4; i++) ch[CH_DELTAS + 4 + i] = dl[i];
            }
        }
    } else if (a.stage == 1) {
        const u64 a0 = c.challenge(), a1 = c.challenge();
        if (writer) ch[CH_ALPHAS] = a0, ch[CH_ALPHAS + 1] = a1;
    } else if (a.stage == 2) {
        const u64 z0 = c.challenge(), z1 = c.challenge();
        if (writer) {
            ch[CH_ZETA] = z0;
            ch[CH_ZETA + 1] = z1;
            E2 zp = gl::exp_pow2(gl::e2(z0, z1), (int)a.aux);
            if (zp.a == 1 && zp.b == 0) atomicMax(&a.status[p], 3);
        }
    } else if (a.stage == 3) {
        const u64 f0 = c.challenge(), f1 = c.challenge();
        if (writer) ch[CH_FRI_ALPHA] = f0, ch[CH_FRI_ALPHA + 1] = f1;
    } else if (a.stage == 4) {
        const u64 b0 = c.challenge(), b1 = c.challenge();
        if (writer) ch[CH_FRI_BETAS + 2 * a.aux] = b0, ch[CH_FRI_BETAS + 2 * a.aux + 1] = b1;
    }
    if (real) c.store(a.st[p]);
}

__global__ __launch_bounds__(64) void k_pi_hash(const u64* __restrict__ values, u32 num_slots, const u32* __restrict__ pi_slots, u32 k, u32 batch,
                                                u64* __restrict__ pi_hash, uint8_t* __restrict__ proofs, size_t proof_bytes, size_t trailer_off) {
    const u32 t = blockIdx.x * blockDim.x + threadIdx.x;
    const bool real = (t >> 4) < batch;
    const u32 p = real ? (t >> 4) : batch - 1;
    const u32 i = t & 15;
    const u64* v = values + (size_t)p * num_slots;
    uint8_t* tr = proofs + (size_t)p * proof_bytes + trailer_off;
    if (real) {
        for (u32 j = i; j < k; j += 16) {
            const u64 x = v[pi_slots[j]];
#pragma unroll
            for (int b = 0; b < 8; b++) tr[8 + 8 * (size_t)j + b] = (uint8_t)(x >> (8 * b));
        }
        if (i == 0)
#pragma unroll
            for (int b = 0; b < 8; b++) tr[b] = (uint8_t)((u64)k >> (8 * b));
    }
    u64 w = 0;
    for (u32 off = 0; off < k; off += 8) {
        if (i < 8 && off + i < k) w = v[pi_slots[off + i]];
        w = glf::poseidon_coop(w, i);
    }
    if (real && i < 4) pi_hash[(size_t)p * 4 + i] = w;
}

static const u32 POW_PHASE_BLOCKS[3] = {1u << 8, 3u << 8, 7u << 10};
static const u32 POW_PHASE_SLOTS[3] = {0, 64, 8};
__global__ __launch_bounds__(256) void k_pow(const ChalState* st, u64* chal, int pow_bits, unsigned long long* best , u32 block0,
                                             const u32* list , const u32* count) {
    __shared__ u64 sh[12];
    __shared__ u32 sh_pos;
    __shared__ unsigned long long sh_cur;
    const u64 block_start = ((u64)block0 + blockIdx.y) * blockDim.x;
    const u32 n_items = list ? *count : gridDim.x;
    for (u32 item = blockIdx.x; item < n_items; item += gridDim.x) {
        const u32 p = list ? list[item] : item;
        __syncthreads();
        if (threadIdx.x == 0) sh_cur = atomicMin(&best[p], ~0ull);
        __syncthreads();
        if (sh_cur < block_start) continue;
        if (threadIdx.x < 12) {
            const ChalState* s = st + p;
            u32 i = threadIdx.x;
            sh[i] = (i < s->in_len) ? s->in[i] : s->state[i];
            if (i == 0) sh_pos = s->in_len;
        }
        __syncthreads();
        const u64 cand = block_start + threadIdx.x;
        const u32 pos = sh_pos;
        u64 r[12];
#pragma unroll
        for (int i = 0; i < 12; i++) r[i] = ((u32)i == pos) ? cand : sh[i];
        glf::poseidon<false>(r);
        if ((r[7] >> (64 - pow_bits)) == 0) atomicMin(&best[p], (unsigned long long)cand);
    }
}
__global__ void k_pow_compact(const unsigned long long* best, u32 batch, u32* list, u32* count) {
    __shared__ u32 n;
    if (threadIdx.x == 0) n = 0;
    __syncthreads();
    for (u32 p = threadIdx.x; p < batch; p += blockDim.x)
        if (best[p] == ~0ull) list[atomicAdd(&n, 1u)] = p;
    __syncthreads();
    if (threadIdx.x == 0) *count = n;
}
__global__ void k_pow_finish(u64* chal, const unsigned long long* best, u32 batch, int* status) {
    u32 p = blockIdx.x * blockDim.x + threadIdx.x;
    if (p >= batch) return;
    chal[(size_t)p * CH_WORDS + CH_POW] = best[p];
    if (best[p] == ~0ull) atomicMax(&status[p], 4);
}

template <bool MUL>
__device__ __forceinline__ u64 block_scan_inclusive(u64 v, u64* lds) {
    const u32 t = threadIdx.x;
    lds[t] = v;
    __syncthreads();
    for (u32 off = 1; off < blockDim.x; off <<= 1) {
        u64 x = lds[t];
        u64 y = t >= off ? lds[t - off] : (MUL ? 1 : 0);
        __syncthreads();
        lds[t] = MUL ? gl::mul(x, y) : gl::add(x, y);
        __syncthreads();
    }
    return lds[t];
}

static const u32 PERM_MAX_CHUNKS = 12;
__device__ __forceinline__ u64 perm_term(u64 beta, u64 f, u64 t) { return gl::mul_add_nc(beta, f, t); }
__device__ __forceinline__ u64 perm_step(u64 prod, u64 term) { return gl::mul_nc(prod, term); }
__global__ __launch_bounds__(256) void k_perm_chunks(const u64* __restrict__ wires, size_t wires_batch_stride, const u64* __restrict__ sigmas,
                                                     const u64* __restrict__ k_is, const u64* __restrict__ subgroup, const u64* __restrict__ chal,
                                                     u64* __restrict__ q, size_t q_batch_stride, u32 n, u32 num_routed, u32 chunk_size, u32 num_chunks,
                                                     u32 num_challenges) {
    const u32 row = blockIdx.x * blockDim.x + threadIdx.x;
    if (row >= n) return;
    const u64* cw = chal + (size_t)blockIdx.y * CH_WORDS;
    const u64* w = wires + (size_t)blockIdx.y * wires_batch_stride + row;
    const u64* sg = sigmas + row;
    const bool two = num_challenges > 1;
    const u64 b0 = cw[CH_BETAS], g0 = cw[CH_GAMMAS], b1 = two ? cw[CH_BETAS + 1] : 0, g1 = two ? cw[CH_GAMMAS + 1] : 0;
    const u64 x = subgroup[row], bx0 = gl::mul(b0, x), bx1 = gl::mul(b1, x);
    u64 num[2 * PERM_MAX_CHUNKS], den[2 * PERM_MAX_CHUNKS], pre[2 * PERM_MAX_CHUNKS];
    auto factors = [&](u32 j, u64& tn0, u64& td0, u64& tn1, u64& td1) {
        const u64 wv = w[(size_t)j * n], s = sg[(size_t)j * n], kj = k_is[j];
        const u64 t0 = gl::add(wv, g0);
        tn0 = perm_term(bx0, kj, t0);
        td0 = perm_term(b0, s, t0);
        if (two) {
            const u64 t1 = gl::add(wv, g1);
            tn1 = perm_term(bx1, kj, t1);
            td1 = perm_term(b1, s, t1);
        }
    };
#pragma unroll
    for (u32 c = 0; c < PERM_MAX_CHUNKS; c++) {
        u64 n0 = 1, d0 = 1, n1 = 1, d1 = 1;
        if (c < num_chunks) {
            const u32 j0 = c * chunk_size, j1 = min(num_routed, (c + 1) * chunk_size);
            for (u32 j = j0; j < j1; j++) {
                u64 tn0, td0, tn1 = 1, td1 = 1;
                factors(j, tn0, td0, tn1, td1);
                if (j == j0) {
                    n0 = tn0, d0 = td0, n1 = tn1, d1 = td1;
                } else {
                    n0 = perm_step(n0, tn0);
                    d0 = perm_step(d0, td0);
                    if (two) {
                        n1 = perm_step(n1, tn1);
                        d1 = perm_step(d1, td1);
                    }
                }
            }
        }
        num[c] = n0;
        den[c] = d0;
        num[PERM_MAX_CHUNKS + c] = n1;
// ... 191 lines not shown
```

### plonky2-aes_amd/csrc/poseidon_fast.h

```cpp
#pragma once
#include "gl.h"

namespace glf {
using gl::u32;
using gl::u64;

#if defined(__HIP_DEVICE_COMPILE__)
#define P2F_DECL __device__ __constant__ static
#else
#define P2F_DECL static
#endif
#include "poseidon_fast.inc"
P2F_DECL const unsigned long long PF_ZERO12[12] = {0, 0, 0, 0, 0, 0, 0, 0, 0, 0, 0, 0};

GL_HD void mul128(u64 a, u64 b, u64& hi, u64& lo) {
#if defined(__HIP_DEVICE_COMPILE__)
    u32 a0 = (u32)a, a1 = (u32)(a >> 32), b0 = (u32)b, b1 = (u32)(b >> 32);
    u64 p00 = (u64)a0 * b0;
    u64 mid = (u64)a0 * b1 + (p00 >> 32);
    u64 mid2 = (u64)a1 * b0 + (u32)mid;
    lo = (mid2 << 32) | (u32)p00;
    hi = (u64)a1 * b1 + (mid >> 32) + (mid2 >> 32);
#else
    unsigned __int128 m = (unsigned __int128)a * b;
// ... 289 lines not shown

GL_HD void full_round(u64* s, const unsigned long long* rc_next) {
#pragma unroll
    for (int i = 0; i < 12; i++) s[i] = sbox7(s[i]);
    mds_full(s, rc_next);
}

GL_HD u64 mulr_add(u64 a, u64 b, u64 c) {
#if defined(__HIP_DEVICE_COMPILE__)
    return gl::mulr_add_dev<true>(a, b, c);
#else
    unsigned __int128 m = (unsigned __int128)a * b + c;
    return red128((u64)(m >> 64), (u64)m);
#endif
}

GL_HD u64 mulr_add_k(u64 k, u64 b, u64 c) {
#if defined(__HIP_DEVICE_COMPILE__)
    return gl::mulr_add_dev<true, true>(k, b, c);
#else
    return mulr_add(k, b, c);
#endif
}

enum : u32 { FR_GENERAL = 0, FR_ZERO_CAP = 1, FR_ZERO_RATE = 2 };
enum : u32 { ROWS_ALL = 0xFFF, ROWS_DIGEST = 0x00F, ROWS_CAPACITY = 0xF00 };

GL_HD constexpr u32 rows_before_chunk(int m) { return m <= 0 ? 0x00Fu : m >= 8 ? 0xF00u : (0xFFFu & ~((1u << m) - 1u)); }

GL_HD constexpr u32 mds_coef(int r, int j) {
    constexpr u32 C[12] = {17, 15, 41, 16, 2, 28, 13, 13, 39, 18, 34, 20};
    return C[(j - r + 12) % 12] + ((r == 0 && j == 0) ? 8u : 0u);
}

#if defined(__HIP_DEVICE_COMPILE__)
#define P2_FR_T(n) "v_mad_u64_u32 %[al], %[d], %[l" #n "], %[k" #n "], %[al]\n\tv_mad_u64_u32 %[ah], %[d], %[h" #n "], %[k" #n "], %[ah]\n\t"
template <int R>
GL_D void mds_rate_terms(u64& al, u64& ah, const u32* l, const u32* h, u64 rl, u64 rh) {
    gl::sg dead;
    asm("v_mad_u64_u32 %[al], %[d], %[l0], %[k0], %[rl]\n\tv_mad_u64_u32 %[ah], %[d], %[h0], %[k0], %[rh]\n\t"
        P2_FR_T(1) P2_FR_T(2) P2_FR_T(3) P2_FR_T(4) P2_FR_T(5) P2_FR_T(6) "v_mad_u64_u32 %[al], %[d], %[l7], %[k7], %[al]\n\t"
        "v_mad_u64_u32 %[ah], %[d], %[h7], %[k7], %[ah]"
        : [al] "=&v"(al), [ah] "=&v"(ah), [d] "=&s"(dead)
        : [rl] "s"(rl), [rh] "s"(rh), [l0] "v"(l[0]), [h0] "v"(h[0]), [l1] "v"(l[1]), [h1] "v"(h[1]), [l2] "v"(l[2]), [h2] "v"(h[2]),
          [l3] "v"(l[3]), [h3] "v"(h[3]), [l4] "v"(l[4]), [h4] "v"(h[4]), [l5] "v"(l[5]), [h5] "v"(h[5]), [l6] "v"(l[6]), [h6] "v"(h[6]),
          [l7] "v"(l[7]), [h7] "v"(h[7]), [k0] "n"(mds_coef(R, 0)), [k1] "n"(mds_coef(R, 1)), [k2] "n"(mds_coef(R, 2)),
          [k3] "n"(mds_coef(R, 3)), [k4] "n"(mds_coef(R, 4)), [k5] "n"(mds_coef(R, 5)), [k6] "n"(mds_coef(R, 6)), [k7] "n"(mds_coef(R, 7)));
}
template <int R, bool ADDEND>
GL_D void mds_cap_terms(u64& al, u64& ah, const u32* l, const u32* h, u64 rl, u64 rh) {
    gl::sg dead;
#define P2_FR_CAP_IN                                                                                                                      \
    [l8] "v"(l[8]), [h8] "v"(h[8]), [l9] "v"(l[9]), [h9] "v"(h[9]), [l10] "v"(l[10]), [h10] "v"(h[10]), [l11] "v"(l[11]), [h11] "v"(h[11]), \
        [k8] "n"(mds_coef(R, 8)), [k9] "n"(mds_coef(R, 9)), [k10] "n"(mds_coef(R, 10)), [k11] "n"(mds_coef(R, 11))
    if (ADDEND)
        asm("v_mad_u64_u32 %[al], %[d], %[l8], %[k8], %[rl]\n\tv_mad_u64_u32 %[ah], %[d], %[h8], %[k8], %[rh]\n\t"
            P2_FR_T(9) P2_FR_T(10) "v_mad_u64_u32 %[al], %[d], %[l11], %[k11], %[al]\n\t"
            "v_mad_u64_u32 %[ah], %[d], %[h11], %[k11], %[ah]"
            : [al] "=&v"(al), [ah] "=&v"(ah), [d] "=&s"(dead)
            : [rl] "s"(rl), [rh] "s"(rh), P2_FR_CAP_IN);
    else
        asm(P2_FR_T(8) P2_FR_T(9) P2_FR_T(10) "v_mad_u64_u32 %[al], %[d], %[l11], %[k11], %[al]\n\t"
            "v_mad_u64_u32 %[ah], %[d], %[h11], %[k11], %[ah]"
            : [al] "+v"(al), [ah] "+v"(ah), [d] "=&s"(dead)
            : P2_FR_CAP_IN);
#undef P2_FR_CAP_IN
}
#undef P2_FR_T
template <int R>
GL_D u64 first_round_row(const u32 kind, const u32* l, const u32* h, const u64 add) {
    u64 al, ah;
    mds_rate_terms<R>(al, ah, l, h, (u64)(u32)add, add >> 32);
    if (kind != FR_ZERO_CAP) mds_cap_terms<R, false>(al, ah, l, h, 0, 0);
    return fold_al_ah(al, ah);
}
template <int R>
GL_D u64 zero_rate_row(const u32* l, const u32* h, const u64 add) {
    u64 al, ah;
    mds_cap_terms<R, true>(al, ah, l, h, (u64)(u32)add, add >> 32);
    return fold_al_ah(al, ah);
}
#endif

GL_HD void sbox_layer_known(u64* s, const u32 kind, const unsigned long long* pre) {
#if defined(__HIP_DEVICE_COMPILE__)
    if (kind == FR_ZERO_RATE) {
#pragma unroll
        for (int i = 8; i < 12; i++) s[i] = sbox7(pre ? add_wrap(s[i], pre[i]) : s[i]);
        return;
    }
    if (pre) {
#pragma unroll
        for (int i = 0; i < 8; i++) s[i] = add_wrap(s[i], pre[i]);
    }
#pragma unroll
    for (int i = 0; i < 8; i++) s[i] = sbox7(s[i]);
    if (kind != FR_ZERO_CAP) {
        if (pre) {
#pragma unroll
            for (int i = 8; i < 12; i++) s[i] = add_wrap(s[i], pre[i]);
        }
#pragma unroll
        for (int i = 8; i < 12; i++) s[i] = sbox7(s[i]);
    }
#else
    const int j0 = kind == FR_ZERO_RATE ? 8 : 0, j1 = kind == FR_ZERO_CAP ? 8 : 12;
    for (int j = j0; j < j1; j++) s[j] = sbox7(pre ? add_wrap(s[j], pre[j]) : s[j]);
#endif
}
GL_HD void linear_layer_known(u64* s, const u32 kind, const unsigned long long* add) {
#if defined(__HIP_DEVICE_COMPILE__)
    u32 l[12], h[12];
#pragma unroll
    for (int i = 0; i < 12; i++) {
        l[i] = (u32)s[i];
        h[i] = (u32)(s[i] >> 32);
    }
    if (kind == FR_ZERO_RATE) {
#define P2_FR_ROW(r) s[r] = zero_rate_row<r>(l, h, add[r]);
        P2_FR_ROW(0) P2_FR_ROW(1) P2_FR_ROW(2) P2_FR_ROW(3) P2_FR_ROW(4) P2_FR_ROW(5) P2_FR_ROW(6) P2_FR_ROW(7) P2_FR_ROW(8) P2_FR_ROW(9)
        P2_FR_ROW(10) P2_FR_ROW(11)
#undef P2_FR_ROW
        return;
    }
#define P2_FR_ROW(r) s[r] = first_round_row<r>(kind, l, h, add[r]);
    P2_FR_ROW(0) P2_FR_ROW(1) P2_FR_ROW(2) P2_FR_ROW(3) P2_FR_ROW(4) P2_FR_ROW(5) P2_FR_ROW(6) P2_FR_ROW(7) P2_FR_ROW(8) P2_FR_ROW(9)
    P2_FR_ROW(10) P2_FR_ROW(11)
#undef P2_FR_ROW
#else
    const int j0 = kind == FR_ZERO_RATE ? 8 : 0, j1 = kind == FR_ZERO_CAP ? 8 : 12;
    u64 out[12];
    for (int r = 0; r < 12; r++) {
        u64 al = (u32)add[r], ah = add[r] >> 32;
        for (int j = j0; j < j1; j++) {
            al += (s[j] & gl::EPS) * mds_coef(r, j);
            ah += (s[j] >> 32) * mds_coef(r, j);
        }
        out[r] = fold_al_ah(al, ah);
    }
    for (int i = 0; i < 12; i++) s[i] = out[i];
#endif
}
GL_HD void full_round_known(u64* s, const u32 kind, const unsigned long long* pre, const unsigned long long* add) {
    sbox_layer_known(s, kind, pre);
    linear_layer_known(s, kind, add);
}
GL_HD const unsigned long long* poseidon_rc() {
#if defined(__HIP_DEVICE_COMPILE__)
    return (const unsigned long long*)gl::D_POSEIDON_RC;
#else
    return (const unsigned long long*)gl::H_POSEIDON_RC;
#endif
}
GL_HD void first_round_any(u64* s, const u32 kind) {
    full_round_known(s, kind, poseidon_rc(), kind == FR_ZERO_CAP ? RC1_ZCAP : kind == FR_ZERO_RATE ? RC1_ZRATE : poseidon_rc() + 12);
}
template <u32 KIND>
GL_HD void first_round(u64* s) {
    static_assert(KIND <= FR_ZERO_RATE, "FR_GENERAL, FR_ZERO_CAP or FR_ZERO_RATE");
    first_round_any(s, KIND);
}

#if defined(__HIP_DEVICE_COMPILE__)
#define P2_PB_T(n) "v_mad_u64_u32 %[al], %[d], %[l" #n "], %[k" #n "], %[al]\n\tv_mad_u64_u32 %[ah], %[d], %[h" #n "], %[k" #n "], %[ah]\n\t"
#define P2_PB_LAST(n) "v_mad_u64_u32 %[al], %[d], %[l" #n "], %[k" #n "], %[al]\n\tv_mad_u64_u32 %[ah], %[d], %[h" #n "], %[k" #n "], %[ah]"
#define P2_PB_IN(n) [l##n] "v"(l[n]), [h##n] "v"(h[n]), [k##n] "s"(c[n])
GL_D u64 block_row0_d2(const u32* l, const u32* h, const u64 t1, const unsigned int* c, const u64 k) {
    const u64 rl = (u64)(u32)k, rh = k >> 32;
    u64 al, ah;
    gl::sg dead;
    asm("v_mad_u64_u32 %[al], %[d], %[lt], 25, %[rl]\n\tv_mad_u64_u32 %[ah], %[d], %[ht], 25, %[rh]\n\t"
        P2_PB_T(0) P2_PB_T(1) P2_PB_T(2) P2_PB_T(3) P2_PB_T(4) P2_PB_LAST(5)
        : [al] "=&v"(al), [ah] "=&v"(ah), [d] "=&s"(dead)
        : [rl] "s"(rl), [rh] "s"(rh), [lt] "v"((u32)t1), [ht] "v"((u32)(t1 >> 32)), P2_PB_IN(0), P2_PB_IN(1), P2_PB_IN(2), P2_PB_IN(3),
          P2_PB_IN(4), P2_PB_IN(5));
    asm(P2_PB_T(6) P2_PB_T(7) P2_PB_T(8) P2_PB_T(9) P2_PB_T(10) P2_PB_LAST(11)
        : [al] "+v"(al), [ah] "+v"(ah), [d] "=&s"(dead)
        : P2_PB_IN(6), P2_PB_IN(7), P2_PB_IN(8), P2_PB_IN(9), P2_PB_IN(10), P2_PB_IN(11));
    return fold_al_ah(al, ah);
}
template <int R>
GL_D u64 block_end_row(const u32* l, const u32* h, const u64 t1, const u64 t2, const unsigned int* e, const u64 k) {
    const u64 rl = (u64)(u32)k, rh = k >> 32;
    const unsigned int* c = e + 1;
    u64 al, ah;
    gl::sg dead;
    asm("v_mad_u64_u32 %[al], %[d], %[lu], %[ku], %[rl]\n\tv_mad_u64_u32 %[ah], %[d], %[hu], %[ku], %[rh]\n\t"
        P2_PB_T(t) P2_PB_T(0) P2_PB_T(1) P2_PB_T(2) P2_PB_T(3) P2_PB_T(4) P2_PB_LAST(5)
        : [al] "=&v"(al), [ah] "=&v"(ah), [d] "=&s"(dead)
        : [rl] "s"(rl), [rh] "s"(rh), [lu] "v"((u32)t2), [hu] "v"((u32)(t2 >> 32)), [ku] "n"(mds_coef(R, 0)), [lt] "v"((u32)t1),
          [ht] "v"((u32)(t1 >> 32)), [kt] "s"(e[0]), P2_PB_IN(0), P2_PB_IN(1), P2_PB_IN(2), P2_PB_IN(3), P2_PB_IN(4), P2_PB_IN(5));
    asm(P2_PB_T(6) P2_PB_T(7) P2_PB_T(8) P2_PB_T(9) P2_PB_T(10) P2_PB_LAST(11)
        : [al] "+v"(al), [ah] "+v"(ah), [d] "=&s"(dead)
        : P2_PB_IN(6), P2_PB_IN(7), P2_PB_IN(8), P2_PB_IN(9), P2_PB_IN(10), P2_PB_IN(11));
    return fold_al_ah(al, ah);
}
static_assert((PM_ALWAYS_ROW0 & 3) == 0, "mds_row0 and block_row0_d2 fold with the rare-carry branch");
GL_D u64 merged_row0_d3(const u32* l, const u32* h, const u64 t1, const u64 t2, const unsigned int* e, const u64 k) {
    const u64 rl = (u64)(u32)k, rh = k >> 32;
    const unsigned int* c = e + 1;
    u64 al, ah;
    gl::sg dead;
    asm("v_mad_u64_u32 %[al], %[d], %[lu], 25, %[rl]\n\tv_mad_u64_u32 %[ah], %[d], %[hu], 25, %[rh]\n\t"
        P2_PB_T(t) P2_PB_T(0) P2_PB_T(1) P2_PB_T(2) P2_PB_T(3) P2_PB_T(4) P2_PB_LAST(5)
        : [al] "=&v"(al), [ah] "=&v"(ah), [d] "=&s"(dead)
        : [rl] "s"(rl), [rh] "s"(rh), [lu] "v"((u32)t2), [hu] "v"((u32)(t2 >> 32)), [lt] "v"((u32)t1), [ht] "v"((u32)(t1 >> 32)),
          [kt] "s"(e[0]), P2_PB_IN(0), P2_PB_IN(1), P2_PB_IN(2), P2_PB_IN(3), P2_PB_IN(4), P2_PB_IN(5));
    asm(P2_PB_T(6) P2_PB_T(7) P2_PB_T(8) P2_PB_T(9) P2_PB_T(10) P2_PB_LAST(11)
        : [al] "+v"(al), [ah] "+v"(ah), [d] "=&s"(dead)
        : P2_PB_IN(6), P2_PB_IN(7), P2_PB_IN(8), P2_PB_IN(9), P2_PB_IN(10), P2_PB_IN(11));
    return fold_al_ah<((PM_ALWAYS_ROW0 >> 2) & 1) != 0>(al, ah);
}
template <int R>
GL_D u64 merged_end_row(const u32* l, const u32* h, const u64 t1, const u64 t2, const u64 t3, const unsigned int* e, const u64 k) {
    const u64 rl = (u64)(u32)k, rh = k >> 32;
    const unsigned int* c = e + 2;
    u64 al, ah;
    gl::sg dead;
    asm("v_mad_u64_u32 %[al], %[d], %[lu], %[ku], %[rl]\n\tv_mad_u64_u32 %[ah], %[d], %[hu], %[ku], %[rh]\n\t"
        P2_PB_T(t) P2_PB_T(v) P2_PB_T(0) P2_PB_T(1) P2_PB_T(2) P2_PB_T(3) P2_PB_LAST(4)
        : [al] "=&v"(al), [ah] "=&v"(ah), [d] "=&s"(dead)
        : [rl] "s"(rl), [rh] "s"(rh), [lu] "v"((u32)t3), [hu] "v"((u32)(t3 >> 32)), [ku] "n"(mds_coef(R, 0)), [lt] "v"((u32)t1),
          [ht] "v"((u32)(t1 >> 32)), [kt] "s"(e[0]), [lv] "v"((u32)t2), [hv] "v"((u32)(t2 >> 32)), [kv] "s"(e[1]), P2_PB_IN(0), P2_PB_IN(1),
          P2_PB_IN(2), P2_PB_IN(3), P2_PB_IN(4));
    asm(P2_PB_T(5) P2_PB_T(6) P2_PB_T(7) P2_PB_T(8) P2_PB_T(9) P2_PB_T(10) P2_PB_LAST(11)
        : [al] "+v"(al), [ah] "+v"(ah), [d] "=&s"(dead)
        : P2_PB_IN(5), P2_PB_IN(6), P2_PB_IN(7), P2_PB_IN(8), P2_PB_IN(9), P2_PB_IN(10), P2_PB_IN(11));
// ... 53 lines not shown
#if defined(__HIP_DEVICE_COMPILE__)
            u32 l[12], h[12];
#pragma unroll
            for (int i = 0; i < 12; i++) {
                l[i] = (u32)s[i];
                h[i] = (u32)(s[i] >> 32);
            }
            t2 = sbox7(block_row0_d2(l, h, t1, PB_ROW0_D2, K[1]));
#else
            t2 = sbox7(block_row(s, PB_ROW0_D2, t1, mds_coef(0, 0), 0, 0, K[1]));
#endif
        }
        block_end(s, t1, t2, PB_END + (three ? 0 : 12 * 13), K + 2);
    }
}

GL_HD void merged_end(u64* s, const u64 t1, const u64 t2, const u64 t3, const unsigned int* e, const unsigned long long* k) {
    u64 res[12];
#if defined(__HIP_DEVICE_COMPILE__)
    u32 l[12], h[12];
#pragma unroll
    for (int i = 0; i < 12; i++) {
        l[i] = (u32)s[i];
        h[i] = (u32)(s[i] >> 32);
    }
#define P2_PM_ROW(r) res[r] = merged_end_row<r>(l, h, t1, t2, t3, e + 14 * r, k[r]);
    P2_PM_ROW(0) P2_PM_ROW(1) P2_PM_ROW(2) P2_PM_ROW(3) P2_PM_ROW(4) P2_PM_ROW(5) P2_PM_ROW(6) P2_PM_ROW(7) P2_PM_ROW(8) P2_PM_ROW(9)
    P2_PM_ROW(10) P2_PM_ROW(11)
#undef P2_PM_ROW
#else
    for (int r = 0; r < 12; r++) res[r] = merged_row(s, e + 14 * r + 2, t1, e[14 * r], t2, e[14 * r + 1], t3, mds_coef(r, 0), k[r]);
#endif
#pragma unroll
    for (int i = 0; i < 12; i++) s[i] = res[i];
}
GL_HD void merged_middle(u64* s) {
#pragma nounroll
    for (int b = 0; b < 6; b++) {
        const unsigned long long* K = PM_K + 15 * b;
        const bool four = PM_DEPTH[b] == 4;
        if (b) s[0] = sbox7(s[0]);
        const u64 t1 = sbox7(mds_row0(s, K[0]));
        u64 t3 = 0;
#if defined(__HIP_DEVICE_COMPILE__)
        u32 l[12], h[12];
#pragma unroll
        for (int i = 0; i < 12; i++) {
            l[i] = (u32)s[i];
            h[i] = (u32)(s[i] >> 32);
        }
        const u64 t2 = sbox7(block_row0_d2(l, h, t1, PB_ROW0_D2, K[1]));
        if (four) t3 = sbox7(merged_row0_d3(l, h, t1, t2, PM_ROW0_D3, K[2]));
#else
        const u64 t2 = sbox7(block_row(s, PB_ROW0_D2, t1, mds_coef(0, 0), 0, 0, K[1]));
        if (four) t3 = sbox7(merged_row(s, PM_ROW0_D3 + 1, t1, PM_ROW0_D3[0], t2, mds_coef(0, 0), 0, 0, K[2]));
#endif
        merged_end(s, t1, t2, t3, PM_END + (four ? 0 : 12 * 14), K + 3);
    }
}
GL_HD void middle(u64* s) {
    const unsigned long long* RC = poseidon_rc();
    for (int r = 1; r < 3; r++) full_round(s, RC + 12 * (r + 1));
#pragma unroll
    for (int i = 0; i < 12; i++) s[i] = sbox7(s[i]);
    merged_middle(s);
    for (int r = 26; r < 29; r++) full_round(s, RC + 12 * (r + 1));
}

GL_HD void last_round_any(u64* s, const u32 rows) {
#pragma unroll
    for (int i = 0; i < 12; i++) s[i] = sbox7(s[i]);
    mds_full(s, PF_ZERO12, rows);
#pragma unroll
    for (int i = 0; i < 12; i++)
        if ((rows >> i) & 1) s[i] = canon(s[i]);
}
template <u32 ROWS>
GL_HD void last_round(u64* s) {
    static_assert(ROWS != 0 && ROWS <= ROWS_ALL, "a mask of output words 0..11");
    last_round_any(s, ROWS);
}

template <bool OWN_SBOX3 = false>
GL_HD void permute_known_any(u64* s, const u32 kind, const u32 rows) {
    const unsigned long long* RC = poseidon_rc();
    const unsigned long long* add0 = kind == FR_ZERO_CAP ? RC1_ZCAP : kind == FR_ZERO_RATE ? RC1_ZRATE : RC + 12;
    if (OWN_SBOX3) {
#pragma nounroll
        for (int r = 0; r < 3; r++) full_round_known(s, r == 0 ? kind : (u32)FR_GENERAL, r == 0 ? RC : nullptr, r == 0 ? add0 : RC + 12 * (r + 1));
#pragma unroll
        for (int i = 0; i < 12; i++) s[i] = sbox7(s[i]);
    } else {
#pragma nounroll
        for (int r = 0; r < 4; r++) {
            if (r) linear_layer_known(s, r == 1 ? kind : (u32)FR_GENERAL, r == 1 ? add0 : RC + 12 * r);
            sbox_layer_known(s, r == 0 ? kind : (u32)FR_GENERAL, r == 0 ? RC : nullptr);
        }
    }
    merged_middle(s);
#pragma nounroll
    for (int r = 26; r < 30; r++) {
#pragma unroll
        for (int i = 0; i < 12; i++) s[i] = sbox7(s[i]);
        mds_full(s, r < 29 ? RC + 12 * (r + 1) : PF_ZERO12, r < 29 ? (u32)ROWS_ALL : rows);
    }
#pragma unroll
    for (int i = 0; i < 12; i++)
        if ((rows >> i) & 1) s[i] = canon(s[i]);
}
template <u32 KIND, u32 ROWS>
GL_HD void permute_known(u64* s) {
    static_assert(KIND <= FR_ZERO_RATE && ROWS != 0 && ROWS <= ROWS_ALL, "FR_* and a mask of output words 0..11");
    permute_known_any(s, KIND, ROWS);
}

template <bool MERGED = true>
GL_HD void poseidon(u64* s) {
    const unsigned long long* RC = poseidon_rc();
#pragma unroll
    for (int i = 0; i < 12; i++) s[i] = add_wrap(s[i], RC[i]);
    if (MERGED) {
        for (int r = 0; r < 4; r++) {
#pragma unroll
            for (int i = 0; i < 12; i++) s[i] = sbox7(s[i]);
            if (r < 3) mds_full(s, RC + 12 * (r + 1));
        }
        merged_middle(s);
    } else {
        for (int r = 0; r < 4; r++) full_round(s, RC + 12 * (r + 1));
        partial_block(s);
    }
    for (int r = 26; r < 29; r++) full_round(s, RC + 12 * (r + 1));
    full_round(s, nullptr);
#pragma unroll
    for (int i = 0; i < 12; i++) s[i] = canon(s[i]);
}

GL_HD u64 mds_row0_terms(const u64* s, u64 rc) {
#if defined(__HIP_DEVICE_COMPILE__)
    {
        u64 al = gl::madk_s<17>((u32)s[0], (u64)(u32)rc), ah = gl::madk_s<17>((u32)(s[0] >> 32), rc >> 32);
#define P2_MDS_TERM(i, K)                       \
    al = gl::madk<K>((u32)s[i], al);            \
    ah = gl::madk<K>((u32)(s[i] >> 32), ah);
        P2_MDS_TERM(1, 15) P2_MDS_TERM(2, 41) P2_MDS_TERM(3, 16) P2_MDS_TERM(4, 2) P2_MDS_TERM(5, 28) P2_MDS_TERM(6, 13)
        P2_MDS_TERM(7, 13) P2_MDS_TERM(8, 39) P2_MDS_TERM(9, 18) P2_MDS_TERM(10, 34) P2_MDS_TERM(11, 20) P2_MDS_TERM(0, 8)
#undef P2_MDS_TERM
        return fold_al_ah(al, ah);
    }
#endif
    return mds_row0(s, rc);
}
GL_HD void partial_block_sparse(u64* s) {
    {
        u64 z[12];
#pragma unroll
        for (int i = 0; i < 12; i++) z[i] = sbox7(s[i]);
#pragma nounroll
        for (int r = 0; r < 11; r++) {
            Acc a;
            a.init();
#pragma unroll
            for (int c = 0; c < 12; c++) a.fma_k(PF_E[r * 12 + c], z[c]);
            s[1 + r] = a.reduce();
        }
        s[0] = mds_row0_terms(z, PF_A[0]);
    }
    for (int i = 0; i < 22; i++) {
        u64 s0 = sbox7(s[0]);
        Acc a;
        a.init();
        a.e01 = i < 21 ? PF_A[i + 1] : PF_RC26[0];
        a.fma_small(25, s0);
#pragma unroll
        for (int j = 0; j < 11; j++) a.fma_k(PF_WHAT[i * 11 + j], s[1 + j]);
#pragma unroll
        for (int j = 0; j < 11; j++) s[1 + j] = mulr_add_k(PF_V[i * 11 + j], s0, s[1 + j]);
        s[0] = a.reduce();
    }
#pragma unroll
    for (int j = 1; j < 12; j++) s[j] = add_wrap(s[j], PF_RC26[j]);
}
GL_HD void poseidon_sparse(u64* s) {
    const unsigned long long* RC = poseidon_rc();
#pragma unroll
    for (int i = 0; i < 12; i++) s[i] = add_wrap(s[i], RC[i]);
    for (int r = 0; r < 3; r++) full_round(s, RC + 12 * (r + 1));
    partial_block_sparse(s);
    for (int r = 26; r < 29; r++) full_round(s, RC + 12 * (r + 1));
    full_round(s, nullptr);
#pragma unroll
    for (int i = 0; i < 12; i++) s[i] = canon(s[i]);
}

GL_HD u32 sponge_first_kind(int c0, int width, int live) {
    return c0 == 0 ? (u32)FR_ZERO_CAP : (c0 >= live && c0 + 8 <= width) ? (u32)FR_ZERO_RATE : (u32)FR_GENERAL;
}
GL_HD void sponge_permute(u64* s, int c0, int width, int live) {
    permute_known_any<true>(s, sponge_first_kind(c0, width, live), rows_before_chunk(width - (c0 + 8)));
}
GL_HD void two_to_one_permute(u64* s) {
    permute_known<FR_ZERO_CAP, ROWS_DIGEST>(s);
}

#if defined(__HIPCC__)
__device__ __forceinline__ u64 shfl64(u64 v, int src_lane) { return (u64)__shfl((unsigned long long)v, src_lane, 64); }
__device__ inline u64 poseidon_coop(u64 w, const u32 i ) {
    const int lane = (int)(threadIdx.x & 63), gbase = lane & ~15;
    const bool live = i < 12;
    const u32 ii = live ? i : 0;
    const unsigned long long* RC = (const unsigned long long*)gl::D_POSEIDON_RC;
    auto mds = [&](u64 z, u64 rc) -> u64 {
        const u32 C[12] = {17, 15, 41, 16, 2, 28, 13, 13, 39, 18, 34, 20};
        u64 al = (u32)rc, ah = rc >> 32;
#pragma unroll
        for (int k = 0; k < 12; k++) {
            u32 src = i + k;
            src = src >= 12 ? src - 12 : src;
            const u64 x = shfl64(z, gbase + (int)(src & 15));
            const u32 c = C[k] + ((k == 0 && i == 0) ? 8u : 0u);
            al += (x & gl::EPS) * c;
            ah += (x >> 32) * c;
        }
        return fold_al_ah(al, ah);
    };
    w = live ? add_wrap(w, RC[ii]) : 0;
    for (int r = 0; r < 3; r++) w = mds(sbox7(w), live ? RC[12 * (r + 1) + ii] : 0);
    {
        const u64 z = sbox7(w);
        const u64 row0 = mds(z, i == 0 ? PF_A[0] : 0);
        const u32 er = (live && i >= 1) ? i - 1 : 0;
        Acc a;
        a.init();
#pragma unroll
        for (int c = 0; c < 12; c++) a.fma(PF_E[er * 12 + c], shfl64(z, gbase + c));
        const u64 rowe = a.reduce();
        w = i == 0 ? row0 : (live ? rowe : 0);
    }
    for (int pr = 0; pr < 22; pr++) {
        const u64 z0 = shfl64(sbox7(w), gbase);
        const u32 cj = (live && i >= 1) ? pr * 11 + (i - 1) : 0;
        const u64 coef = i == 0 ? 25 : (live ? PF_WHAT[cj] : 0);
        u64 term = canon(mulr(coef, i == 0 ? z0 : w));
#pragma unroll
        for (int d = 1; d < 16; d <<= 1) term = gl::add(term, shfl64(term, lane ^ d));
        const u64 s0n = gl::add(term, pr < 21 ? PF_A[pr + 1] : PF_RC26[0]);
        const u64 wj = mulr_add((live && i >= 1) ? PF_V[cj] : 0, z0, w);
        w = i == 0 ? s0n : wj;
    }
    if (live && i >= 1) w = add_wrap(w, PF_RC26[ii]);
    for (int r = 26; r < 29; r++) w = mds(sbox7(w), live ? RC[12 * (r + 1) + ii] : 0);
    w = mds(sbox7(w), 0);
    return live ? canon(w) : 0;
}
#endif

}
```

### plonky2-aes_amd/csrc/prover_gpu.hip

```cpp
#include <hip/hip_runtime.h>
#include <chrono>
#include <cstring>

#include <rocprim/device/device_radix_sort.hpp>

#include <algorithm>
#include <map>
#include <memory>
#include <mutex>
#include <random>
#include <string>
#include <thread>

#include "capi_common.h"
#include "hip_owners.h"
#include "os_random.h"
#include "kernels.h"
#include "kernels2.h"
#include "kernels_compress.h"
#include "kernels_keccak.h"
#include "kernels_merkle.h"
#include "kernels_merkle_update.h"
#include "kernels_merkle_map.h"
#include "kernels_elgamal.h"
// ... 53 lines not shown
    return 0;
}
template <class T>
static int upload(Allocs& mem, T** p, const T* host, size_t count) {
    if (dalloc(mem, p, count)) return P2_ERR_HIP;
    if (count) HIPCHECK(hipMemcpy(*p, host, count * sizeof(T), hipMemcpyHostToDevice));
    return 0;
}

struct Lane {
    hipStream_t stream = nullptr;
    Stream own;
    bool timing = false;
    std::vector<std::pair<std::string, std::pair<Event, Event>>> pending;
    hipError_t open(unsigned flags) { const hipError_t e = own.create(flags); return stream = own, e; }
};
#define LAUNCH(lane, name, kernel, grid, block, shmem, ...)                                  \
    do {                                                                                     \
        Lane& _l = (lane);                                                                   \
        Event _e0, _e1;                                                                      \
        if (_l.timing) {                                                                     \
            (void)_e0.create(hipEventDefault);                                               \
            (void)_e1.create(hipEventDefault);                                               \
            (void)hipEventRecord(_e0, _l.stream);                                            \
        }                                                                                    \
        hipLaunchKernelGGL(kernel, grid, block, shmem, _l.stream, __VA_ARGS__);              \
        if (_l.timing) {                                                                     \
            (void)hipEventRecord(_e1, _l.stream);                                            \
            _l.pending.emplace_back(name, std::make_pair(std::move(_e0), std::move(_e1)));   \
        }                                                                                    \
        HIPCHECK(hipGetLastError());                                                         \
    } while (0)

struct Domain {
    u32 logn = 0;
    std::vector<u32> arities;
    u64 *d_tw_fwd = nullptr, *d_tw_inv = nullptr;
    u64 *d_tw_fwd_full = nullptr, *d_tw_inv_full = nullptr;
    u64* d_tw_fwd_round[9] = {nullptr};
    u64* d_shift_pows[9] = {nullptr};
    u64* d_shift_tw = nullptr;
    std::map<const u64*, u64*> pass1_out_tw;
    u32 rate_bits = 3, cap_height = 0, hasher = HASHER_POSEIDON;
    size_t n() const { return (size_t)1 << logn; }
};

struct Oracle {
    u64* vals = nullptr;
    u64 *coef = nullptr, *lde = nullptr;
    Tree tree;
    u32 cols = 0;
    u32 tree_cols = 0;
    u32 salt = 0;
    size_t coef_stride = 0, lde_stride = 0;
    size_t dig_stride() const { return lde_stride ? tree.stride() : 0; }
};

struct Workspace {
    Allocs mem;
    Lane lane;
    Event done;
    u32* d_input_slots = nullptr;
    std::vector<u32> h_input_slots;
    u64* d_input_values = nullptr;
    u64* d_values = nullptr;
    u32* d_mult = nullptr;
    int* d_status = nullptr;
    u64* d_advice = nullptr;
    u64* d_pi_hash = nullptr;
    DevBuf<u32> d_out_slots;
    std::vector<u32> h_out_slots;
    Oracle wires, zs, quot;
    u64 *d_permq = nullptr, *d_perm_seg = nullptr, *d_fri_seg = nullptr, *d_lktmp = nullptr;
    u64 *d_qvals = nullptr, *d_qres = nullptr;
    ChalState* d_chal_state = nullptr;
    u64* d_chal = nullptr;
    u64 *d_pows = nullptr, *d_ev = nullptr, *d_obs = nullptr, *d_comp = nullptr, *d_apow = nullptr;
    u64 *d_ztab = nullptr, *d_fripow = nullptr;
    u64* d_fri_coef[9] = {nullptr};
    u64* d_fri_vals[9] = {nullptr};
    Tree fri_tree[9];
    unsigned long long* d_pow_best = nullptr;
    u32* d_pow_list = nullptr;
    uint8_t* d_proofs = nullptr;
    PolyRef* d_polyrefs = nullptr;
    EvalRef* d_evalrefs = nullptr;
    ~Workspace() { if (lane.stream) (void)hipStreamSynchronize(lane.stream); }
};

struct p2_circuit {
    Circuit c;
    int device = 0;
    Allocs allocs;
    Lane setup;
    Domain dom;
    size_t n = 0, N = 0;
    u32 lde_bits = 0, active_wires = 0;
    ProofLayout layout;
    size_t pbytes = 0;
    Op* d_ops = nullptr;
    WLevel* d_wlevels = nullptr;
    WChain* d_wchains = nullptr;
    u32 witness_levels = 0, witness_chains = 0;
    int32_t* d_wire_slot = nullptr;
    u32* d_pi_slots = nullptr;
    u64* d_lut_ent = nullptr;
    u32 *d_lut_pairs = nullptr, *d_lut_offsets = nullptr, *d_num_lookups = nullptr;
    LookupRows* d_lookup_rows = nullptr;
    int32_t* d_pos_index = nullptr;
    u32 *d_blind_rows = nullptr, *d_blind_zrows = nullptr;
    ZkKey zk_key{};
    u64 zk_counter = 0;
    size_t total_lut_entries = 0;
    u64 *d_sigmas = nullptr, *d_k_is = nullptr, *d_subgroup = nullptr;
    u64* d_shift_inv_pows = nullptr;
    u64 *d_xs = nullptr, *d_l0 = nullptr, *d_zh_inv = nullptr, *d_w8inv = nullptr, *d_qscale = nullptr;
    Oracle pre;
    u64* d_digest = nullptr;
    std::vector<u64> verifier_data;
    u32 n_b0 = 0, n_b1 = 0, n_evalrefs = 0;
    u32 *d_map_obs = nullptr, *d_map_ser = nullptr;
    u32 n_obs = 0, n_ser = 0, ev_count = 0;
    std::vector<std::unique_ptr<Workspace>> ws;
    Event ev_witness;
    bool witness_recorded = false;
    u32 ws_inputs = 0;
    size_t chunk = 0;
    size_t opt_chunk = 128, opt_streams = 2;
    u32 opt_witness_fuse = 1;
    bool opt_debug_timing = false;
    Pool<struct Staging, NoKey> staging;
    std::string vfy_error;
    VerifyArgs vfy_args{};
    Pool<struct VerifyWs> vfy;
    u32* d_cmp_wmap = nullptr;
    u32* d_kc_hash_idx = nullptr;
    u32 kc_cap_hashes = 0, kc_hashes = 0;
    u32* d_wired_slots = nullptr;
    u32 n_wired = 0;
    Pool<struct WitnessWs> wit{256};
    std::unique_ptr<struct ExplainTables> explain;
    std::mutex explain_mu;
    long fail_alloc_after = -1;
    bool timing_on = false;
    std::map<std::string, std::pair<float, u32>> times;
    std::mutex mu;
    p2_circuit();
    ~p2_circuit();
};

#define LAUNCH_ON(st, kernel, grid, block, ...)                          \
    do {                                                                 \
        hipLaunchKernelGGL(kernel, grid, block, 0, st, __VA_ARGS__);     \
        HIPCHECK(hipGetLastError());                                     \
    } while (0)

template <class Args>
static void fill_gate_table(const Circuit& c, Args& a) {
    for (u32 g = 0; g < c.gates.size(); g++) {
        a.gate_kind[g] = c.gates[g];
        a.gate_sel[g] = c.selector_index[g];
        a.group_lo[g] = c.groups[c.selector_index[g]].first;
        a.group_hi[g] = c.groups[c.selector_index[g]].second;
    }
}

// ... 427 lines not shown
    const OpeningSet& os = C->layout.set;
    const Oracle* oracle[OS_SLOTS] = {&C->pre, &W.wires, &W.zs, &W.zs, &W.quot};
    std::vector<PolyRef> v;
    for (OpenGroup k : OPEN_OBSERVED)
        for (u32 i = os.g[k].lo; i < os.g[k].hi; i++) {
            const Oracle& o = *oracle[os.g[k].slot];
            v.push_back({i < o.cols ? o.coef : nullptr, o.coef_stride, i, 0});
        }
    C->n_b0 = os.n_b0;
    C->n_b1 = os.n_b1;
    std::vector<EvalRef> e;
    for (u32 b = 0; b < OS_SLOTS; b++)
        for (u32 i = 0; i < oracle[b]->cols; i++) e.push_back({oracle[b]->coef, oracle[b]->coef_stride, i, b == OS_Z_NEXT, os.slot_base[b] + i, 0});
    C->n_evalrefs = (u32)e.size();
    if (upload(W.mem, &W.d_evalrefs, e.data(), e.size())) return P2_ERR_HIP;
    return upload(W.mem, &W.d_polyrefs, v.data(), v.size());
}
static int dalloc_ws(p2_circuit* C, Allocs& mem, size_t& counter, void** p, size_t bytes) {
    if (C->fail_alloc_after >= 0 && (long)counter++ == C->fail_alloc_after) {
        C->fail_alloc_after = -1;
        return set_error("hipMalloc: injected allocation failure (test hook)"), P2_ERR_HIP;
    }
    HIPCHECK_AS("hipMalloc(&q, std::max<size_t>(bytes, 8))", mem.alloc(p, std::max<size_t>(bytes, 8)));
    return 0;
}
static u32 fri_pow_count(const p2_circuit* C) { return std::max<u32>(std::max(C->layout.set.n_b0, C->layout.set.n_b1), 1); }
static int build_workspace(p2_circuit* C, Workspace* W, size_t chunk, u32 ws_inputs, size_t& counter) {
    const Circuit& c = C->c;
    const size_t n = C->n, N = C->N;
    const u32 NC = c.cfg.num_challenges;
    W->lane.timing = C->timing_on;
    if (W->lane.open(hipStreamNonBlocking) != hipSuccess) return set_error("hipStreamCreate failed"), P2_ERR_HIP;
    if (W->done.create(hipEventDisableTiming) != hipSuccess) return set_error("hipEventCreate failed"), P2_ERR_HIP;
#define WS_ALLOC(field, count)                                                                       \
    if (dalloc_ws(C, W->mem, counter, (void**)&(field), (size_t)(count) * sizeof(*(field)))) return P2_ERR_HIP
    WS_ALLOC(W->d_input_slots, ws_inputs);
    WS_ALLOC(W->d_input_values, chunk * ws_inputs);
    WS_ALLOC(W->d_values, chunk * c.num_slots);
    WS_ALLOC(W->d_mult, chunk * std::max<size_t>(C->total_lut_entries, 1));
    WS_ALLOC(W->d_status, chunk);
    WS_ALLOC(W->d_advice, chunk * std::max<size_t>(c.poseidon_rows.size(), 1) * 55);
    WS_ALLOC(W->d_pi_hash, chunk * 4);
    W->wires.cols = C->active_wires, W->wires.tree_cols = c.cfg.num_wires;
    W->zs.cols = W->zs.tree_cols = c.num_zs_cols();
    W->quot.cols = W->quot.tree_cols = c.num_quotient_cols();
    for (Oracle* o : {&W->wires, &W->zs, &W->quot}) {
        o->salt = c.salt();
        o->coef_stride = (size_t)o->cols * n;
        o->lde_stride = (size_t)(o->cols + o->salt) * N;
        o->tree.bits = C->lde_bits;
        if (o != &W->quot) WS_ALLOC(o->vals, chunk * o->coef_stride);
        WS_ALLOC(o->coef, chunk * o->coef_stride);
        WS_ALLOC(o->lde, chunk * o->lde_stride);
        WS_ALLOC(o->tree.dig, chunk * o->tree.stride());
    }
    WS_ALLOC(W->d_permq, chunk * NC * (c.num_partial_products() + 1) * n);
    WS_ALLOC(W->d_perm_seg, chunk * NC * PERM_MAX_SEGS);
    WS_ALLOC(W->d_fri_seg, chunk * 4 * FRI_MAX_SEGS);
    WS_ALLOC(W->d_lktmp, chunk * NC * (c.num_sldc_polys() + 1) * n);
    WS_ALLOC(W->d_qvals, chunk * NC * N);
    WS_ALLOC(W->d_qres, chunk * NC * N);
    WS_ALLOC(W->d_chal_state, chunk);
    WS_ALLOC(W->d_chal, chunk * CH_WORDS);
    WS_ALLOC(W->d_pows, chunk * 8 * n);
    WS_ALLOC(W->d_ev, chunk * 2 * C->ev_count);
    WS_ALLOC(W->d_obs, chunk * 2 * C->n_obs);
    WS_ALLOC(W->d_comp, chunk * 4 * n);
    WS_ALLOC(W->d_apow, chunk * 2 * APOW_STRIDE);
    WS_ALLOC(W->d_ztab, chunk * 4 * zeta_tab_words((u32)n));
    WS_ALLOC(W->d_fripow, chunk * 2 * fri_pow_count(C));
    u32 logn_r = C->dom.logn;
    for (u32 r = 0; r <= C->dom.arities.size(); r++) {
        size_t n_r = (size_t)1 << logn_r;
        WS_ALLOC(W->d_fri_coef[r], chunk * 2 * n_r);
        if (r < C->dom.arities.size()) {
            WS_ALLOC(W->d_fri_vals[r], chunk * 2 * 8 * n_r);
            W->fri_tree[r].bits = logn_r + c.cfg.rate_bits - C->dom.arities[r];
            WS_ALLOC(W->fri_tree[r].dig, chunk * W->fri_tree[r].stride());
            logn_r -= C->dom.arities[r];
        }
    }
    WS_ALLOC(W->d_pow_best, chunk);
    WS_ALLOC(W->d_pow_list, chunk + 1);
    WS_ALLOC(W->d_proofs, chunk * C->pbytes);
#undef WS_ALLOC
    return setup_polyrefs(C, *W);
}
static int alloc_workspace(p2_circuit* C, size_t chunk, u32 n_inputs, size_t nstreams) {
    if (C->chunk >= chunk && C->ws_inputs >= n_inputs && C->ws.size() >= nstreams) return 0;
    if (C->chunk != 0) {
        if (C->timing_on) collect_timing(C);
        chunk = std::max(chunk, C->chunk);
        n_inputs = std::max(n_inputs, C->ws_inputs);
        nstreams = std::max(nstreams, C->ws.size());
        release_workspaces(C);
    }
    const u32 ws_inputs = std::max<u32>(n_inputs, 1);
    size_t counter = 0;
    for (size_t wi = 0; wi < nstreams; wi++) {
        C->ws.push_back(std::make_unique<Workspace>());
        if (build_workspace(C, C->ws.back().get(), chunk, ws_inputs, counter)) {
            std::string why = g_last_error;
            release_workspaces(C);
            set_error("workspace allocation failed (" + why + "); the handle holds no workspace now, a smaller batch may fit");
            return P2_ERR_HIP;
        }
    }
    C->chunk = chunk;
    C->ws_inputs = ws_inputs;
    return 0;
}

static int commit_oracle(p2_circuit* C, Workspace& W, Oracle& o, u32 stage, u32 aux, u64 proof_base, u32 B) {
    const size_t N = C->N;
    const u32 cap_h = C->dom.cap_height;
    if (o.vals && intt_cols(W.lane, C->dom, o.vals, o.coef, o.cols, o.coef_stride, B, o.lde, o.lde_stride)) return P2_ERR_HIP;
    if (lde_cols(W.lane, C->dom, o.coef, o.coef_stride, o.lde, o.lde_stride, o.cols, 0, B)) return P2_ERR_HIP;
    if (o.salt)
        LAUNCH(W.lane, "fill_salt", k_fill_salt, g1((size_t)o.salt * N / 8, 256, B), dim3(256), 0, o.lde + (size_t)o.cols * N, o.lde_stride, N, C->zk_key, proof_base,
               (u64)ZK_SALT + 1 + stage);
    if (merkle_build(W.lane, C->dom, o.lde, o.tree_cols + o.salt, o.cols + o.salt, N, o.lde_stride, o.tree, B)) return P2_ERR_HIP;
    return challenger(C, W, stage, o.tree.dig + cap_off(o.tree, cap_h), o.tree.stride(), 4u << cap_h, aux, 0, B);
}
static int prove_chunk(p2_circuit* C, Workspace& W, u32 B, u32 n_inputs, const u64* d_values, u32 n_out, u64* d_out, uint8_t* d_proofs, int* d_status_out,
                       u64 proof_base) {
    const Circuit& c = C->c;
    const size_t n = C->n, N = C->N;
    const u32 R = c.cfg.num_routed_wires, NC = c.cfg.num_challenges, npp = c.num_partial_products(), nlp = c.num_lookup_polys();
    const u32 qc = c.num_quotient_cols(), act = C->active_wires, ncc = c.num_constants_cols();
    const u32 cap_h = c.cfg.cap_height, cap_words = 4u << cap_h, nsldc = c.num_sldc_polys();
    const size_t ws = W.wires.coef_stride, wls = W.wires.lde_stride, zs_s = W.zs.coef_stride, zl_s = W.zs.lde_stride;
    hipStream_t st = W.lane.stream;
    HIPCHECK(hipMemsetAsync(W.d_mult, 0, (size_t)B * std::max<size_t>(C->total_lut_entries, 1) * 4, st));
    {
        WitnessArgs a{};
        a.ops = C->d_ops;
        a.levels = C->d_wlevels;
        a.chains = C->d_wchains;
        a.num_levels = C->witness_levels;
        a.num_slots = c.num_slots;
        a.n_inputs = n_inputs;
        a.input_slots = W.d_input_slots;
        a.input_values = d_values;
        a.values = W.d_values;
        a.lut_ent = C->d_lut_ent;
        a.mult = W.d_mult;
        a.total_lut_entries = C->total_lut_entries;
        a.status = W.d_status;
        a.wire_slot = C->d_wire_slot;
        a.advice = W.d_advice;
        a.n = (u32)n;
        a.num_poseidon_rows = (u32)c.poseidon_rows.size();
        const u32 WITNESS_THREADS = 512;
        if (C->witness_recorded) HIPCHECK(hipStreamWaitEvent(W.lane.stream, C->ev_witness, 0));
        if (ecstep_gate_index(c) >= 0) {
            const bool pos = !c.poseidon_rows.empty();
            if (!pos && C->witness_chains) LAUNCH(W.lane, "witness", (k_ecwitness<false, true>), dim3(B), dim3(WITNESS_THREADS), 0, a);
            if (!pos && !C->witness_chains) LAUNCH(W.lane, "witness", (k_ecwitness<false, false>), dim3(B), dim3(WITNESS_THREADS), 0, a);
            if (pos && C->witness_chains) LAUNCH(W.lane, "witness", (k_ecwitness<true, true>), dim3(B), dim3(WITNESS_THREADS), 0, a);
            if (pos && !C->witness_chains) LAUNCH(W.lane, "witness", (k_ecwitness<true, false>), dim3(B), dim3(WITNESS_THREADS), 0, a);
        } else if (c.poseidon_rows.empty()) {
            if (C->witness_chains)
                LAUNCH(W.lane, "witness", (k_witness<false, true>), dim3(B), dim3(WITNESS_THREADS), 0, a);
            else
                LAUNCH(W.lane, "witness", (k_witness<false, false>), dim3(B), dim3(WITNESS_THREADS), 0, a);
        } else {
            if (C->witness_chains)
                LAUNCH(W.lane, "witness", (k_witness<true, true>), dim3(B), dim3(WITNESS_THREADS), 0, a);
            else
// ... 84 lines not shown
        a.nsel = c.num_selectors();
        a.nls = c.num_lookup_selectors;
        a.NC = NC;
        a.npp = npp;
        a.qdf = c.cfg.quotient_degree_factor;
        a.num_luts = (u32)c.luts.size();
        a.nsldc = nsldc;
        a.lut_deg = nlp ? c.lut_degree() : 0;
        a.nlp = nlp;
        a.num_gates = (u32)c.gates.size();
        a.num_gate_constraints = c.num_gate_constraints;
        fill_gate_table(c, a);
        for (u32 l = 0; l < c.luts.size(); l++) a.lut_last_row[l] = c.lookup_rows[l].last_lut;
        a.zs_values = W.zs.vals;
        a.zs_values_batch_stride = zs_s;
        a.pi_hash = c.pi_slots.empty() ? nullptr : W.d_pi_hash;
        a.apow = W.d_apow;
        {
            u32 nlk = nlp ? 4 + (u32)c.luts.size() + 2 * nsldc : 0;
            u32 nterms = NC + NC * (npp + 1) + NC * nlk + c.num_gate_constraints;
            if (nterms > APOW_STRIDE) return set_error("internal: too many vanishing terms for the alpha-power table"), P2_ERR_INVALID;
            LAUNCH(W.lane, "alpha_pows", k_alpha_pows, g1(2 * B, 64), dim3(64), 0, W.d_chal, W.d_apow, B, nterms);
        }
        if (c.poseidon_rows.empty())
            LAUNCH(W.lane, "quotient", (k_quotient<false, true>), g1(N, 256, B), dim3(256), 0, a);
        else
            LAUNCH(W.lane, "quotient", k_quotient<true>, g1(N, 256, B), dim3(256), 0, a);
        const int eg = ecstep_gate_index(c);
        if (eg >= 0) {
            EcQuotientArgs e{};
            e.pre_lde = a.pre_lde, e.wires_lde = a.wires_lde, e.wires_batch_stride = a.wires_batch_stride, e.zh_inv = a.zh_inv, e.apow = a.apow;
            e.out = a.out, e.out_batch_stride = a.out_batch_stride;
            e.n = a.n, e.logn = a.logn, e.rate_bits = a.rate_bits, e.nsel = a.nsel;
            e.idx_gate = NC + NC * (npp + 1) + NC * (nlp ? 4 + (u32)c.luts.size() + 2 * nsldc : 0);
            e.gate = (u32)eg, e.gate_sel = a.gate_sel[eg], e.group_lo = a.group_lo[eg], e.group_hi = a.group_hi[eg];
            LAUNCH(W.lane, "quotient", k_ecstep_post, g1(N, 256, B), dim3(256), 0, e);
        }
        if (quotient_chunks(W.lane, C->dom, W.d_qvals, W.d_qres, W.quot.coef, NC, (size_t)qc * n, B, C->d_shift_inv_pows, C->d_w8inv, C->d_qscale)) return P2_ERR_HIP;
    }
    if (commit_oracle(C, W, W.quot, 2, c.degree_bits, proof_base, B)) return P2_ERR_HIP;
    LAUNCH(W.lane, "zeta_pows", k_zeta_tabs, g1(ZT_LO + zeta_tab_hi((u32)n), 256, B, 4), dim3(256), 0, W.d_chal, W.d_ztab, (u32)n, gl::root_of_unity((int)C->dom.logn));
    LAUNCH(W.lane, "zeta_pows", k_zeta_pows, g1(n, 256, B, 4), dim3(256), 0, W.d_ztab, W.d_pows, (size_t)8 * n, (u32)n);
    HIPCHECK(hipMemsetAsync(W.d_ev, 0, (size_t)B * 2 * C->ev_count * 8, st));
    {
        const size_t evs = 2 * (size_t)C->ev_count;
        u64* ev = W.d_ev;
        LAUNCH(W.lane, "eval_polys", k_eval_polys_refs, dim3(C->n_evalrefs, B), dim3(256), 0, W.d_evalrefs, W.d_pows, (size_t)8 * n, (u32)n, ev, evs);
        LAUNCH(W.lane, "gather_ext", k_gather_ext, g1(C->n_obs, 256, B), dim3(256), 0, W.d_ev, evs, C->d_map_obs, C->n_obs, W.d_obs, (size_t)2 * C->n_obs);
    }
    if (challenger(C, W, 3, W.d_obs, (size_t)2 * C->n_obs, 2 * C->n_obs, 0, 0, B)) return P2_ERR_HIP;
    {
        const u32 npow = fri_pow_count(C);
        LAUNCH(W.lane, "fri_compose", k_fri_alpha_pows, g1(npow, 64, B), dim3(64), 0, W.d_chal, W.d_fripow, npow);
        LAUNCH(W.lane, "fri_compose", k_fri_compose, g1(n, 256, B), dim3(256), 0, W.d_polyrefs, C->n_b0, C->n_b1, W.d_fripow, npow, (u32)n, W.d_comp, (size_t)4 * n);
    }
    {
        const u32 segs = (u32)std::min<size_t>(std::max<size_t>(n >> 14, 1), FRI_MAX_SEGS);
        if (segs > 1)
            LAUNCH(W.lane, "fri_divide", k_fri_seg_sums, dim3(B, segs), dim3(1024), 0, W.d_comp, (size_t)4 * n, W.d_pows, (size_t)8 * n, (u32)n, W.d_fri_seg);
        LAUNCH(W.lane, "fri_divide", k_fri_divide, dim3(B, segs), dim3(1024), 0, W.d_comp, (size_t)4 * n, W.d_pows, (size_t)8 * n, W.d_chal, (u32)n, C->n_b1,
               W.d_fri_coef[0], (size_t)2 * n, segs > 1 ? W.d_fri_seg : nullptr);
    }
    {
        u32 logn_r = C->dom.logn;
        for (u32 r = 0; r < C->dom.arities.size(); r++) {
            size_t n_r = (size_t)1 << logn_r, len = 8 * n_r;
            u32 arity = 1u << C->dom.arities[r];
            if (lde_cols(W.lane, C->dom, W.d_fri_coef[r], 2 * n_r, W.d_fri_vals[r], 2 * len, 2, r, B)) return P2_ERR_HIP;
            Tree& t = W.fri_tree[r];
            size_t leaves = len / arity;
            LAUNCH(W.lane, "hash_fri_leaves", tree_kernels(C->dom.hasher).fri_leaves, g1(leaves, 256, B), dim3(256), 0, W.d_fri_vals[r], len, 2 * len, (int)arity, t.dig,
                   t.stride());
            if (merkle_levels(W.lane, C->dom, t, B)) return P2_ERR_HIP;
            if (challenger(C, W, 4, t.dig + cap_off(t, cap_h), t.stride(), cap_words, r, 0, B)) return P2_ERR_HIP;
            size_t n_next = n_r >> C->dom.arities[r];
            LAUNCH(W.lane, "fri_fold", k_fri_fold, g1(n_next, 256, B), dim3(256), 0, W.d_fri_coef[r], n_r, 2 * n_r, W.d_fri_coef[r + 1], n_next, 2 * n_next, W.d_chal, r,
                   arity);
            logn_r -= C->dom.arities[r];
        }
        size_t fl = (size_t)1 << logn_r;
        u32 R_ = (u32)C->dom.arities.size();
        LAUNCH(W.lane, "interleave", k_interleave_ext, g1(fl, 256, B), dim3(256), 0, W.d_fri_coef[R_], fl, 2 * fl, W.d_obs, (size_t)2 * C->n_obs);
        if (challenger(C, W, 5, W.d_obs, (size_t)2 * C->n_obs, (u32)(2 * fl), 0, 0, B)) return P2_ERR_HIP;
        HIPCHECK(hipMemsetAsync(W.d_pow_best, 0xFF, (size_t)B * 8, st));
        {
            u32 block0 = 0;
            for (int ph = 0; ph < 3; ph++) {
                u32* list = ph ? W.d_pow_list : nullptr;
                if (ph) LAUNCH(W.lane, "pow", k_pow_compact, dim3(1), dim3(256), 0, W.d_pow_best, B, W.d_pow_list, W.d_pow_list + C->chunk);
                const u32 slots = ph ? std::min<u32>(B, POW_PHASE_SLOTS[ph]) : B;
                LAUNCH(W.lane, "pow", k_pow, dim3(slots, POW_PHASE_BLOCKS[ph]), dim3(256), 0, W.d_chal_state, W.d_chal, (int)c.cfg.pow_bits, W.d_pow_best,
                       block0, (const u32*)list, (const u32*)(list ? list + C->chunk : nullptr));
                block0 += POW_PHASE_BLOCKS[ph];
            }
        }
        LAUNCH(W.lane, "pow_finish", k_pow_finish, g1(B, 64), dim3(64), 0, W.d_chal, W.d_pow_best, B, W.d_status);
        if (challenger(C, W, 6, W.d_obs, 0, 0, c.cfg.num_query_rounds, (u64)N, B)) return P2_ERR_HIP;
        const ProofLayout& L = C->layout;
        ProofSegs segs{};
        u32 nseg = 0;
        segs.proofs = d_proofs;
        segs.proof_bytes = L.bytes;
        const Oracle* oracles[4] = {&C->pre, &W.wires, &W.zs, &W.quot};
        for (int o = 1; o < 4; o++) {
            const Tree& t = oracles[o]->tree;
            segs.s[nseg++] = ProofSeg{t.dig + cap_off(t, cap_h), nullptr, t.stride(), 0, L.caps_off[o - 1], cap_words, 0};
        }
        segs.s[nseg++] = ProofSeg{W.d_ev, C->d_map_ser, 2 * (size_t)C->ev_count, 0, L.open[0].off, C->n_ser, 2};
        if (R_ + 6 > 12) return set_error("internal: more FRI rounds than proof segments"), P2_ERR_INVALID;
        for (u32 r = 0; r < R_; r++) {
            Tree& t = W.fri_tree[r];
            segs.s[nseg++] = ProofSeg{t.dig + cap_off(t, cap_h), nullptr, t.stride(), 0, L.fri_caps_off + r * L.cap_bytes, cap_words, 0};
        }
        QueryArgs q{};
        for (int o = 0; o < 4; o++) {
            const Oracle& from = *oracles[o];
            q.oracles[o].lde = from.lde;
            q.oracles[o].lde_batch_stride = from.lde_stride;
            q.oracles[o].digests = from.tree.dig;
            q.oracles[o].dig_batch_stride = from.dig_stride();
            q.oracles[o].cols = from.tree_cols + from.salt;
            q.oracles[o].active_cols = from.cols + from.salt;
        }
        q.lde_bits = C->lde_bits;
        q.cap_height = cap_h;
        q.num_queries = c.cfg.num_query_rounds;
        q.num_rounds = R_;
        u32 lb = C->lde_bits;
        for (u32 r = 0; r < R_; r++) {
            q.arity_bits[r] = C->dom.arities[r];
            q.fri_vals[r] = W.d_fri_vals[r];
            q.fri_vals_batch_stride[r] = (size_t)2 << lb;
            q.fri_bits[r] = lb;
            q.fri_digests[r] = W.fri_tree[r].dig;
            q.fri_dig_batch_stride[r] = W.fri_tree[r].stride();
            lb -= C->dom.arities[r];
        }
        q.chal = W.d_chal;
        q.proofs = d_proofs;
        q.proof_bytes = L.bytes;
        q.queries_off = L.queries_off;
        q.query_bytes = L.query_bytes;
        LAUNCH(W.lane, "write_queries", k_write_queries, dim3(c.cfg.num_query_rounds, B), dim3(256), 0, q);
        segs.s[nseg++] = ProofSeg{W.d_fri_coef[R_], nullptr, 2 * fl, fl, L.final_off, (u32)fl, 1};
        segs.s[nseg++] = ProofSeg{W.d_chal + CH_POW, nullptr, (size_t)CH_WORDS, 0, L.pow_off, 1u, 0};
        LAUNCH(W.lane, "proof_segments", k_proof_segments, dim3(2, B, nseg), dim3(256), 0, segs);
    }
    LAUNCH(W.lane, "finish", k_finish, g1(C->pbytes, 256, B), dim3(256), 0, W.d_status, d_status_out, d_proofs, C->pbytes, B);
    return 0;
}

static void ws_drain(hipStream_t own, bool has_caller = false, void* caller = nullptr) {
    if (has_caller) (void)hipStreamSynchronize((hipStream_t)caller);
    if (own) (void)hipStreamSynchronize(own);
}
struct Staging {
    NoKey key;
    Staged<u64> vals, out;
    Staged<uint8_t> proofs;
    Staged<int> stat;
    Stream stream;
    void drain(bool has_caller, void* caller) { ws_drain(stream, has_caller, caller); }
    ~Staging() { ws_drain(stream); }
    bool fit(size_t vals_bytes, size_t proofs_bytes, size_t batch, size_t out_bytes) {
        return (stream || stream.create(hipStreamNonBlocking) == hipSuccess) && vals.grow(vals_bytes) && proofs.grow(proofs_bytes) &&
               stat.grow(batch * sizeof(int)) && out.grow(out_bytes);
    }
};

template <class F>
static int guarded_rc(F&& f) {
    try {
        return f();
    } catch (std::bad_alloc&) {
        return set_error("out of host memory"), P2_ERR_HIP;
    } catch (std::exception& e) {
        return set_error(e.what()), P2_ERR_INVALID;
    } catch (...) {
// ... 1356 lines not shown
        for (int k = 0; k < 16; k++) b += got[k] != want[k];
        {
            const int A = 1 + i % 3, half = 8 >> A, base = 16 - 2 * half, r = ((i >> 2) & 1) * 2 * half + (i % half);
            for (int k = 0; k < 16; k++) got[k] = want[k];
            if (!odd) {
                tw[base + r % half] = pw;
                got[r] = gl::add_ref(got[r + half], q);
            }
            for (int k = 0; k < 16; k++) want[k] = got[k];
            if (A == 1) ntt_r16_stage<1>(got, tw);
            if (A == 2) ntt_r16_stage<2>(got, tw);
            if (A == 3) ntt_r16_stage<3>(got, tw);
            ref_r16_stage(want, tw, A);
            for (int k = 0; k < 16; k++) b += got[k] != want[k];
        }
    }
    {
        const u64 one_nc = gl::P + 1 + (x & 0), w = (u64)1 << 33;
        if (gl::mul_nb(gl::sub(0, one_nc), w) == gl::mul_ref(gl::sub_ref(0, C(one_nc)), w)) b++;
    }
    if (b) atomicAdd(bad, b);
}
}

int p2_selftest_ntt_device(uint64_t seed, size_t threads, int device) {
    if (hipSetDevice(device) != hipSuccess) return set_error("no such HIP device"), -P2_ERR_HIP;
    if (threads == 0 || threads > ((size_t)1 << 30)) return set_error("thread count out of range"), -P2_ERR_INVALID;
    Allocs mem;
    unsigned long long* d = nullptr;
    if (dalloc(mem, &d, 1) || hipMemset(d, 0, 8) != hipSuccess) return set_error("hipMalloc failed"), -P2_ERR_HIP;
    hipLaunchKernelGGL(p2k::k_selftest_ntt, dim3((u32)((threads + 255) / 256)), dim3(256), 0, 0, d, (u64)seed, threads);
    unsigned long long h = 0;
    if (hipError_t e = hipMemcpy(&h, d, 8, hipMemcpyDeviceToHost)) return set_error(hipGetErrorString(e)), -P2_ERR_HIP;
    return (int)std::min<unsigned long long>(h, 0x7FFFFFFF);
}
int p2_gpu_zeta_pows(const uint64_t* z, size_t n, uint64_t* pows, int device) {
    if (n == 0 || n > ((size_t)1 << 22) || (n & (n - 1))) return set_error("n must be a power of two up to 2^22"), P2_ERR_INVALID;
    if (z[0] >= gl::P || z[1] >= gl::P) return set_error("z is not canonical"), P2_ERR_INVALID;
    if (int rc = pick_device(device)) return rc;
    int logn = 0;
    while (((size_t)1 << logn) < n) logn++;
    std::vector<u64> chal(CH_WORDS, 0);
    chal[CH_ZETA] = z[0];
    chal[CH_ZETA + 1] = z[1];
    Allocs mem;
    u64 *d_chal, *d_tab, *d_pows;
    if (upload(mem, &d_chal, chal.data(), chal.size()) || dalloc(mem, &d_tab, 4 * zeta_tab_words((u32)n)) || dalloc(mem, &d_pows, 8 * n)) return P2_ERR_HIP;
    hipLaunchKernelGGL(k_zeta_tabs, g1(ZT_LO + zeta_tab_hi((u32)n), 256, 1, 4), dim3(256), 0, 0, d_chal, d_tab, (u32)n, gl::root_of_unity(logn));
    HIPCHECK(hipGetLastError());
    hipLaunchKernelGGL(k_zeta_pows, g1(n, 256, 1, 4), dim3(256), 0, 0, d_tab, d_pows, (size_t)8 * n, (u32)n);
    HIPCHECK(hipGetLastError());
    HIPCHECK(hipMemcpy(pows, d_pows, 8 * n * 8, hipMemcpyDeviceToHost));
    return P2_OK;
}

static int states_in_place(void (*kernel)(u64*, size_t), const char* bad_shape, uint64_t* states, size_t count, int device) {
    return run_batch(bad_shape, count, on_host(device), {buf_inout(states, 12 * count)},
                     [&](const DevPtr* d, hipStream_t s) { hipLaunchKernelGGL(kernel, g1(count, 256), dim3(256), 0, s, d[0], count); });
}
static const char* states_count_shape(size_t count) { return count == 0 || count > (1u << 24) ? "count out of range" : nullptr; }
int p2_gpu_poseidon(uint64_t* states, size_t n_perm, int device) { return states_in_place(k_poseidon_states, nullptr, states, n_perm, device); }
int p2_gpu_partial_rounds(uint64_t* states, size_t count, int device) { return states_in_place(k_partial_rounds, states_count_shape(count), states, count, device); }
int p2_gpu_merged_middle(uint64_t* states, size_t count, int device) { return states_in_place(k_merged_middle, states_count_shape(count), states, count, device); }
int p2_gpu_hash_leaves(const uint64_t* data, size_t cols, size_t active_cols, size_t num_leaves, size_t batch, uint64_t* digests, int device) {
    if (cols == 0 || cols > (1u << 20) || num_leaves == 0 || batch == 0 || batch > 65535) return set_error("shape out of range"), P2_ERR_INVALID;
    if (int rc = pick_device(device)) return rc;
    const size_t stored = std::min(active_cols, cols), in_words = std::max<size_t>(stored, 1) * num_leaves;
    Allocs mem;
    u64 *d_in, *d_out;
    if (dalloc(mem, &d_in, batch * in_words) || dalloc(mem, &d_out, batch * num_leaves * 4)) return P2_ERR_HIP;
    HIPCHECK(hipMemcpy(d_in, data, batch * stored * num_leaves * 8, hipMemcpyHostToDevice));
    hipLaunchKernelGGL(k_hash_leaves, g1(num_leaves, 256, (u32)batch), dim3(256), 0, 0, d_in, (int)cols, (int)active_cols, num_leaves, stored * num_leaves, num_leaves,
                       d_out, num_leaves * 4);
    HIPCHECK(hipGetLastError());
    HIPCHECK(hipMemcpy(digests, d_out, batch * num_leaves * 32, hipMemcpyDeviceToHost));
    return P2_OK;
}
int p2_gpu_ecstep_constraints(const uint64_t* wires, size_t count, uint64_t* out, int device) {
    const char* bad = count == 0 || count > (1u << 20) || !wires || !out ? "count out of range" : nullptr;
    for (size_t i = 0; !bad && i < 80 * count; i++)
        if (wires[i] >= gl::P) bad = "p2_gpu_ecstep_constraints: non-canonical wire";
    return run_batch(bad, count, on_host(device), {buf_in(wires, 80 * count), buf_out(out, 40 * count)},
                     [&](const DevPtr* d, hipStream_t s) { hipLaunchKernelGGL(k_ecstep_selftest, g1(count, 256), dim3(256), 0, s, d[0], count, d[1]); });
}
int p2_gpu_merkle_level(const uint64_t* child, size_t num_parents, size_t batch, uint64_t* parent, int device) {
    if (num_parents == 0 || batch == 0 || batch > 65535) return set_error("shape out of range"), P2_ERR_INVALID;
    if (int rc = pick_device(device)) return rc;
    const size_t stride = 8 * num_parents;
    Allocs mem;
    u64 *d_in, *d_out;
    if (upload(mem, &d_in, (const u64*)child, batch * stride) || dalloc(mem, &d_out, batch * stride)) return P2_ERR_HIP;
    hipLaunchKernelGGL(k_merkle_level, g1(num_parents, 256, (u32)batch), dim3(256), 0, 0, d_in, d_out, num_parents, stride);
    HIPCHECK(hipGetLastError());
    for (size_t b = 0; b < batch; b++) HIPCHECK(hipMemcpy(parent + b * 4 * num_parents, d_out + b * stride, num_parents * 32, hipMemcpyDeviceToHost));
    return P2_OK;
}
int p2_gpu_hash_fri_leaves(const uint64_t* vals, size_t len, int arity, size_t batch, uint64_t* digests, int device) {
    const bool bad = arity < 1 || arity > 64 || len == 0 || len % (size_t)arity || batch == 0 || batch > 65535;
    const size_t leaves = bad ? 0 : len / (size_t)arity;
    return run_batch(bad ? "shape out of range" : nullptr, batch, on_host(device), {buf_in(vals, batch * 2 * len), buf_out(digests, batch * leaves * 4)},
                     [&](const DevPtr* d, hipStream_t s) {
                         hipLaunchKernelGGL(k_hash_fri_leaves, g1(leaves, 256, (u32)batch), dim3(256), 0, s, d[0], len, 2 * len, arity, d[1], leaves * 4);
                     });
}
struct PrimCtx {
    Allocs mem;
    Lane lane;
    Domain dom;
    u64* d_shift_inv_pows = nullptr;
    int init(int device, int degree_bits, const std::vector<u32>& arities = {}, bool with_quotient = false) {
        if (int rc = pick_device(device)) return rc;
        dom.logn = (u32)degree_bits;
        dom.arities = arities;
        HIPCHECK_AS("hipStreamCreate(&lane.stream)", lane.open(hipStreamDefault));
        HIPCHECK(raise_ntt_lds_limits());
        return build_transform_tables(lane, dom, mem, with_quotient ? &d_shift_inv_pows : nullptr);
    }
    ~PrimCtx() { if (lane.stream) (void)hipStreamSynchronize(lane.stream); }
};
int p2_gpu_intt(const uint64_t* values, size_t cols, int degree_bits, uint64_t* coeffs, int device) {
    if (degree_bits < 1 || degree_bits > 22) return set_error("degree_bits must be in 1..22"), P2_ERR_INVALID;
    PrimCtx ctx;
    if (int rc = ctx.init(device, degree_bits)) return rc;
    const size_t n = ctx.dom.n();
    u64 *d_in, *d_out, *d_scratch;
    if (upload(ctx.mem, &d_in, (const u64*)values, cols * n) || dalloc(ctx.mem, &d_out, cols * n) || dalloc(ctx.mem, &d_scratch, cols * n)) return P2_ERR_HIP;
    if (intt_cols(ctx.lane, ctx.dom, d_in, d_out, (u32)cols, 0, 1, d_scratch, 0)) return P2_ERR_HIP;
    HIPCHECK(hipStreamSynchronize(ctx.lane.stream));
    HIPCHECK(hipMemcpy(coeffs, d_out, cols * n * 8, hipMemcpyDeviceToHost));
    return P2_OK;
}
int p2_gpu_lde(const uint64_t* coeffs, size_t cols, int degree_bits, int rate_bits, uint64_t* lde, int device) {
    if (degree_bits < 1 || degree_bits > 22 || rate_bits != 3) return set_error("degree_bits must be in 1..22 and rate_bits 3"), P2_ERR_INVALID;
    PrimCtx ctx;
    if (int rc = ctx.init(device, degree_bits)) return rc;
    const size_t n = ctx.dom.n();
    u64 *d_in, *d_out;
    if (upload(ctx.mem, &d_in, (const u64*)coeffs, cols * n) || dalloc(ctx.mem, &d_out, cols * 8 * n)) return P2_ERR_HIP;
    if (lde_cols(ctx.lane, ctx.dom, d_in, 0, d_out, 0, (u32)cols, 0, 1)) return P2_ERR_HIP;
    HIPCHECK(hipStreamSynchronize(ctx.lane.stream));
    HIPCHECK(hipMemcpy(lde, d_out, cols * 8 * n * 8, hipMemcpyDeviceToHost));
    return P2_OK;
}
int p2_gpu_lde_round(const uint64_t* coeffs, size_t cols, int degree_bits, const uint32_t* arities, size_t n_rounds, size_t round, size_t batch,
                     size_t in_batch_stride, uint64_t* out, size_t out_batch_stride, int device) {
    if (degree_bits < 1 || degree_bits > 22 || cols == 0 || cols > 4096 || batch == 0 || batch > 65535 || n_rounds > 8 || (round && round >= n_rounds))
        return set_error("shape out of range"), P2_ERR_INVALID;
    u32 logn_r = (u32)degree_bits, left = (u32)degree_bits;
    std::vector<u32> ar(arities, arities + n_rounds);
    for (size_t r = 0; r < n_rounds; r++) {
        if (ar[r] == 0 || ar[r] >= left) return set_error("arities reduce the degree to nothing"), P2_ERR_INVALID;
        left -= ar[r];
        if (r < round) logn_r = left;
    }
    const size_t n_r = (size_t)1 << logn_r;
    if (in_batch_stride < cols * n_r || out_batch_stride < 8 * cols * n_r) return set_error("batch stride smaller than a proof's columns"), P2_ERR_INVALID;
    PrimCtx ctx;
    if (int rc = ctx.init(device, degree_bits, ar)) return rc;
    u64 *d_in, *d_out;
    if (upload(ctx.mem, &d_in, (const u64*)coeffs, batch * in_batch_stride) || upload(ctx.mem, &d_out, (const u64*)out, batch * out_batch_stride)) return P2_ERR_HIP;
    if (lde_cols(ctx.lane, ctx.dom, d_in, in_batch_stride, d_out, out_batch_stride, (u32)cols, (u32)round, (u32)batch)) return P2_ERR_HIP;
    HIPCHECK(hipStreamSynchronize(ctx.lane.stream));
    HIPCHECK(hipMemcpy(out, d_out, batch * out_batch_stride * 8, hipMemcpyDeviceToHost));
    return P2_OK;
}
int p2_gpu_quotient_chunks(const uint64_t* qvals, size_t chunks, int degree_bits, size_t batch, uint64_t* out, int device) {
// ... 890 lines not shown
```

Baseline: 786.5.

## Precompute Poseidon PoW midstate so grinding varies only one sbox input

Adds a per-proof midstate kernel that evaluates the first round for every fixed word and stores the canonical MDS output split into 32-bit halves, plus the MDS column for the witness position. Each grinding candidate then runs one sbox and a 12-term multiply-accumulate in place of the full first round, and the last round computes only row 7. Separately, sponge permutations gain a pre_mask/seam path that skips constant adds for known-zero words and defers the final canonicalisation into the next chunk. The aim is fewer field operations in the PoW search and the sponge hashing, at the cost of an extra launch, a midstate buffer and new host/GPU test entry points.

```diff
diff --git a/bindings/plonky2-hip/src/ffi.rs b/bindings/plonky2-hip/src/ffi.rs
--- a/bindings/plonky2-hip/src/ffi.rs
+++ b/bindings/plonky2-hip/src/ffi.rs
@@ -158,6 +158,8 @@
     pub fn p2_selftest_lazy_device(seed: u64, threads: usize, device: c_int) -> c_int;
     pub fn p2_selftest_ntt_device(seed: u64, threads: usize, device: c_int) -> c_int;
     pub fn p2_host_poseidon_known(states: *mut u64, n_perm: usize, kind: c_int, rows: u32, parts: c_int) -> c_int;
+    pub fn p2_host_poseidon_seam(states: *mut u64, n_perm: usize, kind: c_int, rows: u32, pre_mask: u32, seam: c_int) -> c_int;
+    pub fn p2_host_pow_search(state: *const u64, in: *const u64, in_len: *const u32, count: usize, pow_bits: c_int, witnesses: *mut u64, form: c_int) -> c_int;
     pub fn p2_host_pcipher_hash_state(in: *const u64, last: c_int, out: *mut u64) -> c_int;
     pub fn p2_host_partial_rounds(states: *mut u64, count: usize) -> c_int;
     pub fn p2_host_merged_middle(states: *mut u64, count: usize) -> c_int;
@@ -282,6 +284,7 @@
     pub fn p2_gpu_partial_rounds(states: *mut u64, count: usize, device: c_int) -> c_int;
     pub fn p2_gpu_merged_middle(states: *mut u64, count: usize, device: c_int) -> c_int;
     pub fn p2_gpu_ecstep_constraints(wires: *const u64, count: usize, out: *mut u64, device: c_int) -> c_int;
+    pub fn p2_gpu_pow_search(state: *const u64, in: *const u64, in_len: *const u32, count: usize, pow_bits: c_int, witnesses: *mut u64, device: c_int) -> c_int;
     pub fn p2_gpu_merkle_level(child: *const u64, num_parents: usize, batch: usize, parent: *mut u64, device: c_int) -> c_int;
     pub fn p2_gpu_hash_fri_leaves(vals: *const u64, len: usize, arity: c_int, batch: usize, digests: *mut u64, device: c_int) -> c_int;
     pub fn p2_gpu_zeta_pows(z: *const u64, n: usize, pows: *mut u64, device: c_int) -> c_int;
diff --git a/include/p2aes.h b/include/p2aes.h
--- a/include/p2aes.h
+++ b/include/p2aes.h
@@ -207,6 +207,8 @@
 int p2_selftest_lazy_device(uint64_t seed, size_t threads, int device);
 int p2_selftest_ntt_device(uint64_t seed, size_t threads, int device);
 int p2_host_poseidon_known(uint64_t* states, size_t n_perm, int kind, uint32_t rows, int parts);
+int p2_host_poseidon_seam(uint64_t* states, size_t n_perm, int kind, uint32_t rows, uint32_t pre_mask, int seam);
+int p2_host_pow_search(const uint64_t* state, const uint64_t* in, const uint32_t* in_len, size_t count, int pow_bits, uint64_t* witnesses, int form);
 int p2_host_pcipher_hash_state(const uint64_t in[20], int last, uint64_t out[20]);
 int p2_host_partial_rounds(uint64_t* states, size_t count);
 int p2_host_merged_middle(uint64_t* states, size_t count);
@@ -433,6 +435,7 @@
 int p2_gpu_partial_rounds(uint64_t* states, size_t count, int device);
 int p2_gpu_merged_middle(uint64_t* states, size_t count, int device);
 int p2_gpu_ecstep_constraints(const uint64_t* wires, size_t count, uint64_t* out, int device);
+int p2_gpu_pow_search(const uint64_t* state, const uint64_t* in, const uint32_t* in_len, size_t count, int pow_bits, uint64_t* witnesses, int device);
 int p2_gpu_merkle_level(const uint64_t* child, size_t num_parents, size_t batch, uint64_t* parent, int device);
 int p2_gpu_hash_fri_leaves(const uint64_t* vals, size_t len, int arity, size_t batch, uint64_t* digests, int device);
 int p2_gpu_zeta_pows(const uint64_t* z, size_t n, uint64_t* pows, int device);
diff --git a/plonky2-aes_amd/api.py b/plonky2-aes_amd/api.py
--- a/plonky2-aes_amd/api.py
+++ b/plonky2-aes_amd/api.py
@@ -257,6 +257,9 @@
         "p2_circuit_get_timing": (sz, [vp, C.POINTER(_KernelTime), sz]),
         "p2_gpu_device_count": (C.c_int, []),
         "p2_gpu_poseidon": (C.c_int, [u64p, sz, C.c_int]),
+        "p2_host_poseidon_seam": (C.c_int, [u64p, sz, C.c_int, C.c_uint32, C.c_uint32, C.c_int]),
+        "p2_host_pow_search": (C.c_int, [u64p, u64p, u32p, sz, C.c_int, u64p, C.c_int]),
+        "p2_gpu_pow_search": (C.c_int, [u64p, u64p, u32p, sz, C.c_int, u64p, C.c_int]),
         "p2_host_partial_rounds": (C.c_int, [u64p, sz]),
         "p2_gpu_partial_rounds": (C.c_int, [u64p, sz, C.c_int]),
         "p2_host_merged_middle": (C.c_int, [u64p, sz]),
diff --git a/plonky2-aes_amd/csrc/capi_host.cpp b/plonky2-aes_amd/csrc/capi_host.cpp
--- a/plonky2-aes_amd/csrc/capi_host.cpp
+++ b/plonky2-aes_amd/csrc/capi_host.cpp
@@ -865,6 +865,46 @@
             glf::last_round_any(s, rows);
         } else {
             glf::permute_known_any(s, (u32)kind, rows);
+        }
+    }
+    return P2_OK;
+}
+int p2_host_poseidon_seam(uint64_t* states, size_t n_perm, int kind, uint32_t rows, uint32_t pre_mask, int seam) {
+    if (kind < 0 || kind > (int)glf::FR_ZERO_RATE || rows == 0 || rows > glf::ROWS_ALL || pre_mask > 0xFFF)
+        return set_error("kind must be 0..2, rows and pre_mask masks of words 0..11"), P2_ERR_INVALID;
+    const uint32_t cap = pre_mask & 0xF00;
+    if (cap != 0 && cap != 0xF00) return set_error("the capacity words carry round 0's constants together or not at all"), P2_ERR_INVALID;
+    for (size_t i = 0; i < n_perm; i++) glf::permute_known_any<true>(states + 12 * i, (u32)kind, rows, pre_mask, seam != 0);
+    return P2_OK;
+}
+int p2_host_pow_search(const uint64_t* state, const uint64_t* in, const uint32_t* in_len, size_t count, int pow_bits, uint64_t* witnesses, int form) {
+    if (pow_bits < 1 || pow_bits > 32 || form < 0 || form > 1) return set_error("pow_bits must be in 1..32 and form 0 or 1"), P2_ERR_INVALID;
+    if (count && (!state || !in || !in_len || !witnesses)) return set_error("p2_host_pow_search: null argument"), P2_ERR_INVALID;
+    for (size_t p = 0; p < count; p++) {
+        const u32 pos = in_len[p];
+        if (pos >= 8) return set_error("in_len must be below 8"), P2_ERR_INVALID;
+        u64 base[12];
+        for (u32 i = 0; i < 12; i++) base[i] = i < pos ? in[8 * p + i] : state[12 * p + i];
+        for (u32 i = 0; i < 12; i++)
+            if (base[i] >= gl::P) return set_error("p2_host_pow_search: non-canonical word"), P2_ERR_INVALID;
+        glf::PowMidstate m;
+        if (form) glf::pow_midstate(base, pos, m);
+        witnesses[p] = ~0ull;
+        for (u64 w = 0; w < ((u64)1 << 21); w++) {
+            u64 r7;
+            if (form == 0) {
+                u64 s[12];
+                memcpy(s, base, sizeof s);
+                s[pos] = w;
+                glf::poseidon(s);
+                r7 = s[7];
+            } else {
+                r7 = glf::pow_response(m, w);
+            }
+            if ((r7 >> (64 - pow_bits)) == 0) {
+                witnesses[p] = w;
+                break;
+            }
         }
     }
     return P2_OK;
diff --git a/plonky2-aes_amd/csrc/kernels.h b/plonky2-aes_amd/csrc/kernels.h
--- a/plonky2-aes_amd/csrc/kernels.h
+++ b/plonky2-aes_amd/csrc/kernels.h
@@ -1185,10 +1185,22 @@
 
 static const u32 POW_PHASE_BLOCKS[3] = {1u << 8, 3u << 8, 7u << 10};
 static const u32 POW_PHASE_SLOTS[3] = {0, 64, 8};
-__global__ __launch_bounds__(256) void k_pow(const ChalState* st, u64* chal, int pow_bits, unsigned long long* best , u32 block0,
+__global__ void k_pow_midstate(const ChalState* st, u32 batch, glf::PowMidstate* mid) {
+    const u32 p = blockIdx.x * blockDim.x + threadIdx.x;
+    if (p >= batch) return;
+    const ChalState& s = st[p];
+    const u32 pos = s.in_len;
+    u64 in[12];
+#pragma unroll
+    for (int i = 0; i < 12; i++) in[i] = ((u32)i < pos) ? s.in[i & 7] : s.state[i];
+    glf::PowMidstate m;
+    glf::pow_midstate(in, pos, m);
+    mid[p] = m;
+}
+__global__ __launch_bounds__(256) void k_pow(const glf::PowMidstate* mid, u64* chal, int pow_bits, unsigned long long* best , u32 block0,
                                              const u32* list , const u32* count) {
-    __shared__ u64 sh[12];
-    __shared__ u32 sh_pos;
+    constexpr u32 MID_WORDS = sizeof(glf::PowMidstate) / 4;
+    __shared__ glf::PowMidstate sh;
     __shared__ unsigned long long sh_cur;
     const u64 block_start = ((u64)block0 + blockIdx.y) * blockDim.x;
     const u32 n_items = list ? *count : gridDim.x;
@@ -1198,20 +1210,11 @@
         if (threadIdx.x == 0) sh_cur = atomicMin(&best[p], ~0ull);
         __syncthreads();
         if (sh_cur < block_start) continue;
-        if (threadIdx.x < 12) {
-            const ChalState* s = st + p;
-            u32 i = threadIdx.x;
-            sh[i] = (i < s->in_len) ? s->in[i] : s->state[i];
-            if (i == 0) sh_pos = s->in_len;
-        }
+        if (threadIdx.x < MID_WORDS) ((u32*)&sh)[threadIdx.x] = ((const u32*)(mid + p))[threadIdx.x];
         __syncthreads();
         const u64 cand = block_start + threadIdx.x;
-        const u32 pos = sh_pos;
-        u64 r[12];
-#pragma unroll
-        for (int i = 0; i < 12; i++) r[i] = ((u32)i == pos) ? cand : sh[i];
-        glf::poseidon<false>(r);
-        if ((r[7] >> (64 - pow_bits)) == 0) atomicMin(&best[p], (unsigned long long)cand);
+        const u64 r7 = glf::pow_response(sh, cand);
+        if ((r7 >> (64 - pow_bits)) == 0) atomicMin(&best[p], (unsigned long long)cand);
     }
 }
 __global__ void k_pow_compact(const unsigned long long* best, u32 batch, u32* list, u32* count) {
diff --git a/plonky2-aes_amd/csrc/poseidon_fast.h b/plonky2-aes_amd/csrc/poseidon_fast.h
--- a/plonky2-aes_amd/csrc/poseidon_fast.h
+++ b/plonky2-aes_amd/csrc/poseidon_fast.h
@@ -395,21 +395,26 @@
 }
 #endif
 
-GL_HD void sbox_layer_known(u64* s, const u32 kind, const unsigned long long* pre) {
-#if defined(__HIP_DEVICE_COMPILE__)
+GL_HD void sbox_layer_known(u64* s, const u32 kind, const unsigned long long* pre, const u32 pre_mask = 0xFFF) {
+#if defined(__HIP_DEVICE_COMPILE__)
+    const bool pre_cap = pre && (pre_mask & 0xF00u);
     if (kind == FR_ZERO_RATE) {
-#pragma unroll
-        for (int i = 8; i < 12; i++) s[i] = sbox7(pre ? add_wrap(s[i], pre[i]) : s[i]);
+        if (pre_cap) {
+#pragma unroll
+            for (int i = 8; i < 12; i++) s[i] = add_wrap(s[i], pre[i]);
+        }
+#pragma unroll
+        for (int i = 8; i < 12; i++) s[i] = sbox7(s[i]);
         return;
     }
     if (pre) {
 #pragma unroll
-        for (int i = 0; i < 8; i++) s[i] = add_wrap(s[i], pre[i]);
+        for (int i = 0; i < 8; i++) s[i] = add_wrap(s[i], ((pre_mask >> i) & 1) ? pre[i] : 0ull);
     }
 #pragma unroll
     for (int i = 0; i < 8; i++) s[i] = sbox7(s[i]);
     if (kind != FR_ZERO_CAP) {
-        if (pre) {
+        if (pre_cap) {
 #pragma unroll
             for (int i = 8; i < 12; i++) s[i] = add_wrap(s[i], pre[i]);
         }
@@ -418,7 +423,8 @@
     }
 #else
     const int j0 = kind == FR_ZERO_RATE ? 8 : 0, j1 = kind == FR_ZERO_CAP ? 8 : 12;
-    for (int j = j0; j < j1; j++) s[j] = sbox7(pre ? add_wrap(s[j], pre[j]) : s[j]);
+    const u32 mask = pre ? (pre_mask & 0xF00u ? pre_mask | 0xF00u : pre_mask) : 0;
+    for (int j = j0; j < j1; j++) s[j] = sbox7((mask >> j) & 1 ? add_wrap(s[j], pre[j]) : s[j]);
 #endif
 }
 GL_HD void linear_layer_known(u64* s, const u32 kind, const unsigned long long* add) {
@@ -454,8 +460,8 @@
     for (int i = 0; i < 12; i++) s[i] = out[i];
 #endif
 }
-GL_HD void full_round_known(u64* s, const u32 kind, const unsigned long long* pre, const unsigned long long* add) {
-    sbox_layer_known(s, kind, pre);
+GL_HD void full_round_known(u64* s, const u32 kind, const unsigned long long* pre, const unsigned long long* add, const u32 pre_mask = 0xFFF) {
+    sbox_layer_known(s, kind, pre, pre_mask);
     linear_layer_known(s, kind, add);
 }
 GL_HD const unsigned long long* poseidon_rc() {
@@ -675,19 +681,21 @@
 }
 
 template <bool OWN_SBOX3 = false>
-GL_HD void permute_known_any(u64* s, const u32 kind, const u32 rows) {
+GL_HD void permute_known_any(u64* s, const u32 kind, const u32 rows, const u32 pre_mask = 0xFFF, const bool seam = false) {
     const unsigned long long* RC = poseidon_rc();
     const unsigned long long* add0 = kind == FR_ZERO_CAP ? RC1_ZCAP : kind == FR_ZERO_RATE ? RC1_ZRATE : RC + 12;
+    const unsigned long long* add29 = seam ? RC : PF_ZERO12;
     if (OWN_SBOX3) {
 #pragma nounroll
-        for (int r = 0; r < 3; r++) full_round_known(s, r == 0 ? kind : (u32)FR_GENERAL, r == 0 ? RC : nullptr, r == 0 ? add0 : RC + 12 * (r + 1));
+        for (int r = 0; r < 3; r++)
+            full_round_known(s, r == 0 ? kind : (u32)FR_GENERAL, r == 0 ? RC : nullptr, r == 0 ? add0 : RC + 12 * (r + 1), pre_mask);
 #pragma unroll
         for (int i = 0; i < 12; i++) s[i] = sbox7(s[i]);
     } else {
 #pragma nounroll
         for (int r = 0; r < 4; r++) {
             if (r) linear_layer_known(s, r == 1 ? kind : (u32)FR_GENERAL, r == 1 ? add0 : RC + 12 * r);
-            sbox_layer_known(s, r == 0 ? kind : (u32)FR_GENERAL, r == 0 ? RC : nullptr);
+            sbox_layer_known(s, r == 0 ? kind : (u32)FR_GENERAL, r == 0 ? RC : nullptr, pre_mask);
         }
     }
     merged_middle(s);
@@ -695,8 +703,9 @@
     for (int r = 26; r < 30; r++) {
 #pragma unroll
         for (int i = 0; i < 12; i++) s[i] = sbox7(s[i]);
-        mds_full(s, r < 29 ? RC + 12 * (r + 1) : PF_ZERO12, r < 29 ? (u32)ROWS_ALL : rows);
-    }
+        mds_full(s, r < 29 ? RC + 12 * (r + 1) : add29, r < 29 ? (u32)ROWS_ALL : rows);
+    }
+    if (seam) return;
 #pragma unroll
     for (int i = 0; i < 12; i++)
         if ((rows >> i) & 1) s[i] = canon(s[i]);
@@ -707,26 +716,63 @@
     permute_known_any(s, KIND, ROWS);
 }
 
-template <bool MERGED = true>
 GL_HD void poseidon(u64* s) {
     const unsigned long long* RC = poseidon_rc();
 #pragma unroll
     for (int i = 0; i < 12; i++) s[i] = add_wrap(s[i], RC[i]);
-    if (MERGED) {
-        for (int r = 0; r < 4; r++) {
-#pragma unroll
-            for (int i = 0; i < 12; i++) s[i] = sbox7(s[i]);
-            if (r < 3) mds_full(s, RC + 12 * (r + 1));
-        }
-        merged_middle(s);
-    } else {
-        for (int r = 0; r < 4; r++) full_round(s, RC + 12 * (r + 1));
-        partial_block(s);
-    }
+    for (int r = 0; r < 4; r++) {
+#pragma unroll
+        for (int i = 0; i < 12; i++) s[i] = sbox7(s[i]);
+        if (r < 3) mds_full(s, RC + 12 * (r + 1));
+    }
+    merged_middle(s);
     for (int r = 26; r < 29; r++) full_round(s, RC + 12 * (r + 1));
     full_round(s, nullptr);
 #pragma unroll
     for (int i = 0; i < 12; i++) s[i] = canon(s[i]);
+}
+
+struct PowMidstate {
+    unsigned long long alo[12], ahi[12];
+    unsigned int coef[12];
+    unsigned int pos;
+};
+GL_HD void pow_midstate(const u64* in, const u32 pos, PowMidstate& m) {
+    const unsigned long long* RC = poseidon_rc();
+    u64 z[12];
+#pragma unroll
+    for (int j = 0; j < 12; j++) z[j] = (u32)j == pos ? 0 : sbox7(add_wrap(in[j], RC[j]));
+    mds_full(z, RC + 12);
+#pragma unroll
+    for (int r = 0; r < 12; r++) {
+        const u64 a = canon(z[r]);
+        m.alo[r] = (u32)a;
+        m.ahi[r] = a >> 32;
+        u32 c = 0;
+#pragma unroll
+        for (int j = 0; j < 12; j++) c = (u32)j == pos ? mds_coef(r, j) : c;
+        m.coef[r] = c;
+    }
+    m.pos = pos;
+}
+GL_HD u64 pow_response(const PowMidstate& m, const u64 cand) {
+    const unsigned long long* RC = poseidon_rc();
+    const u64 t = sbox7(add_wrap(cand, RC[m.pos]));
+    const u64 tl = (u32)t, th = t >> 32;
+    u64 s[12];
+#pragma unroll
+    for (int r = 0; r < 12; r++) s[r] = fold_al_ah(m.alo[r] + tl * m.coef[r], m.ahi[r] + th * m.coef[r]);
+    for (int r = 1; r < 4; r++) {
+#pragma unroll
+        for (int i = 0; i < 12; i++) s[i] = sbox7(s[i]);
+        if (r < 3) mds_full(s, RC + 12 * (r + 1));
+    }
+    merged_middle(s);
+    for (int r = 26; r < 29; r++) full_round(s, RC + 12 * (r + 1));
+#pragma unroll
+    for (int i = 0; i < 12; i++) s[i] = sbox7(s[i]);
+    mds_full(s, nullptr, 1u << 7);
+    return canon(s[7]);
 }
 
 GL_HD u64 mds_row0_terms(const u64* s, u64 rc) {
@@ -789,8 +835,10 @@
 GL_HD u32 sponge_first_kind(int c0, int width, int live) {
     return c0 == 0 ? (u32)FR_ZERO_CAP : (c0 >= live && c0 + 8 <= width) ? (u32)FR_ZERO_RATE : (u32)FR_GENERAL;
 }
+GL_HD constexpr u32 sponge_pre_mask(int c0, int width) { return c0 == 0 ? 0xFFFu : 0xFFFu & ~rows_before_chunk(width - c0); }
 GL_HD void sponge_permute(u64* s, int c0, int width, int live) {
-    permute_known_any<true>(s, sponge_first_kind(c0, width, live), rows_before_chunk(width - (c0 + 8)));
+    const int m = width - (c0 + 8);
+    permute_known_any<true>(s, sponge_first_kind(c0, width, live), rows_before_chunk(m), sponge_pre_mask(c0, width), m > 0);
 }
 GL_HD void two_to_one_permute(u64* s) {
     permute_known<FR_ZERO_CAP, ROWS_DIGEST>(s);
diff --git a/plonky2-aes_amd/csrc/prover_gpu.hip b/plonky2-aes_amd/csrc/prover_gpu.hip
--- a/plonky2-aes_amd/csrc/prover_gpu.hip
+++ b/plonky2-aes_amd/csrc/prover_gpu.hip
@@ -159,6 +159,7 @@
     Tree fri_tree[9];
     unsigned long long* d_pow_best = nullptr;
     u32* d_pow_list = nullptr;
+    glf::PowMidstate* d_pow_mid = nullptr;
     uint8_t* d_proofs = nullptr;
     PolyRef* d_polyrefs = nullptr;
     EvalRef* d_evalrefs = nullptr;
@@ -752,9 +753,25 @@
     }
     WS_ALLOC(W->d_pow_best, chunk);
     WS_ALLOC(W->d_pow_list, chunk + 1);
+    WS_ALLOC(W->d_pow_mid, chunk);
     WS_ALLOC(W->d_proofs, chunk * C->pbytes);
 #undef WS_ALLOC
     return setup_polyrefs(C, *W);
+}
+static int pow_search(Lane& lane, const ChalState* d_state, glf::PowMidstate* d_mid, u64* d_chal, int pow_bits, unsigned long long* d_best, u32* d_list,
+                      u32 cap, u32 B) {
+    HIPCHECK(hipMemsetAsync(d_best, 0xFF, (size_t)B * 8, lane.stream));
+    LAUNCH(lane, "pow_midstate", k_pow_midstate, g1(B, 64), dim3(64), 0, d_state, B, d_mid);
+    u32 block0 = 0;
+    for (int ph = 0; ph < 3; ph++) {
+        u32* list = ph ? d_list : nullptr;
+        if (ph) LAUNCH(lane, "pow", k_pow_compact, dim3(1), dim3(256), 0, d_best, B, d_list, d_list + cap);
+        const u32 slots = ph ? std::min<u32>(B, POW_PHASE_SLOTS[ph]) : B;
+        LAUNCH(lane, "pow", k_pow, dim3(slots, POW_PHASE_BLOCKS[ph]), dim3(256), 0, d_mid, d_chal, pow_bits, d_best, block0, (const u32*)list,
+               (const u32*)(list ? list + cap : nullptr));
+        block0 += POW_PHASE_BLOCKS[ph];
+    }
+    return P2_OK;
 }
 static int alloc_workspace(p2_circuit* C, size_t chunk, u32 n_inputs, size_t nstreams) {
     if (C->chunk >= chunk && C->ws_inputs >= n_inputs && C->ws.size() >= nstreams) return 0;
@@ -1005,18 +1022,7 @@
         u32 R_ = (u32)C->dom.arities.size();
         LAUNCH(W.lane, "interleave", k_interleave_ext, g1(fl, 256, B), dim3(256), 0, W.d_fri_coef[R_], fl, 2 * fl, W.d_obs, (size_t)2 * C->n_obs);
         if (challenger(C, W, 5, W.d_obs, (size_t)2 * C->n_obs, (u32)(2 * fl), 0, 0, B)) return P2_ERR_HIP;
-        HIPCHECK(hipMemsetAsync(W.d_pow_best, 0xFF, (size_t)B * 8, st));
-        {
-            u32 block0 = 0;
-            for (int ph = 0; ph < 3; ph++) {
-                u32* list = ph ? W.d_pow_list : nullptr;
-                if (ph) LAUNCH(W.lane, "pow", k_pow_compact, dim3(1), dim3(256), 0, W.d_pow_best, B, W.d_pow_list, W.d_pow_list + C->chunk);
-                const u32 slots = ph ? std::min<u32>(B, POW_PHASE_SLOTS[ph]) : B;
-                LAUNCH(W.lane, "pow", k_pow, dim3(slots, POW_PHASE_BLOCKS[ph]), dim3(256), 0, W.d_chal_state, W.d_chal, (int)c.cfg.pow_bits, W.d_pow_best,
-                       block0, (const u32*)list, (const u32*)(list ? list + C->chunk : nullptr));
-                block0 += POW_PHASE_BLOCKS[ph];
-            }
-        }
+        if (int rc = pow_search(W.lane, W.d_chal_state, W.d_pow_mid, W.d_chal, (int)c.cfg.pow_bits, W.d_pow_best, W.d_pow_list, (u32)C->chunk, B)) return rc;
         LAUNCH(W.lane, "pow_finish", k_pow_finish, g1(B, 64), dim3(64), 0, W.d_chal, W.d_pow_best, B, W.d_status);
         if (challenger(C, W, 6, W.d_obs, 0, 0, c.cfg.num_query_rounds, (u64)N, B)) return P2_ERR_HIP;
         const ProofLayout& L = C->layout;
@@ -2539,6 +2545,28 @@
         if (wires[i] >= gl::P) bad = "p2_gpu_ecstep_constraints: non-canonical wire";
     return run_batch(bad, count, on_host(device), {buf_in(wires, 80 * count), buf_out(out, 40 * count)},
                      [&](const DevPtr* d, hipStream_t s) { hipLaunchKernelGGL(k_ecstep_selftest, g1(count, 256), dim3(256), 0, s, d[0], count, d[1]); });
+}
+int p2_gpu_pow_search(const uint64_t* state, const uint64_t* in, const uint32_t* in_len, size_t count, int pow_bits, uint64_t* witnesses, int device) {
+    const char* bad = count > 65535 || pow_bits < 1 || pow_bits > 32 ? "count or pow_bits out of range" : nullptr;
+    std::vector<ChalState> st(bad || !state || !in || !in_len ? 0 : count);
+    for (size_t p = 0; p < st.size(); p++) {
+        if (in_len[p] >= 8) bad = "in_len must be below 8";
+        for (int i = 0; i < 12; i++) bad = (st[p].state[i] = state[12 * p + i]) >= gl::P ? "non-canonical word" : bad;
+        for (int i = 0; i < 8; i++) bad = (st[p].in[i] = in[8 * p + i]) >= gl::P ? "non-canonical word" : bad;
+        for (int i = 0; i < 8; i++) st[p].out[i] = 0;
+        st[p].in_len = in_len[p], st[p].out_len = 0;
+    }
+    if (!bad && count && st.empty()) bad = "null argument";
+    int rc = P2_OK;
+    const int r = run_batch(bad, count, on_host(device),
+                            {buf_in(st.data(), st.size()), buf_out(witnesses, count), buf_scratch((glf::PowMidstate*)nullptr, count),
+                             buf_scratch((u32*)nullptr, count + 1)},
+                            [&](const DevPtr* d, hipStream_t s) {
+                                Lane lane;
+                                lane.stream = s;
+                                rc = pow_search(lane, d[0], d[2], nullptr, pow_bits, (unsigned long long*)d[1], d[3], (u32)count, (u32)count);
+                            });
+    return r ? r : rc;
 }
 int p2_gpu_merkle_level(const uint64_t* child, size_t num_parents, size_t batch, uint64_t* parent, int device) {
     if (num_parents == 0 || batch == 0 || batch > 65535) return set_error("shape out of range"), P2_ERR_INVALID;
```

After: 793.3, median of 6. No clear change (+0.9%).
